# pityka/lamp

Hardware: AMD Instinct MI355X
Metric: training-step samples/sec (higher is better)
Workload: dtype bf16; 1 GPU; example-cifar100 Cnn.resnet(100) training step (fwd+backprop+AdamW), synthetic CIFAR batch; per_gpu_batch=2048, global_batch=2048, parallelism=single, optimizer=AdamW lr 1e-3 wd 0 beta2 0.95 mixedPrecision

## Files before the change

### lamp_amd/csrc/core/switches.h

```cpp
#pragma once
#include <cstdint>

namespace lamp {

constexpr int64_t SW_NO_CLAMP = INT64_MIN;

#define LAMP_SWITCHES_ONCE(X)                                                                                                             \
                                                        \
  X(conv_sibling, "LAMP_CONV_SIBLING", BOOL, 1, 0, "a residual block's 3x3 and its sibling 1x1 of the same input as one forward launch") \
  X(fuse_bn_pair, "LAMP_FUSE_BN_PAIR", BOOL, 1, 0, "relu(bn(right) + bn(left)) at a block's end as one op (0: the chain)")                \
  X(fuse_pool_logsoftmax, "LAMP_FUSE_POOL_LOGSOFTMAX", BOOL, 1, 0, "average pool -> flatten -> log-softmax tail as one node")             \
  X(fuse_block_tail, "LAMP_FUSE_BLOCK_TAIL", BOOL, 1, 0, "the last residual block and the pooled log-softmax tail as one node")          \
  X(fuse_bn_conv, "LAMP_FUSE_BN_CONV", BOOL, 1, 0, "batch norm -> relu -> convolution: the convolution applies the norm while staging")  \
  X(fuse_loss_accumulate, "LAMP_FUSE_LOSS_ACCUMULATE", BOOL, 1, 0, "acc += n * loss inside the NLL loss kernel")                          \
  X(fuse_loss_backward, "LAMP_FUSE_LOSS_BACKWARD", BOOL, 1, 0, "the NLL loss backward goes straight to the pooled log-softmax node's input in one launch")                      \
  X(fuse_loss_tail, "LAMP_FUSE_LOSS_TAIL", BOOL, 1, 0, "the loss launch also writes the pooled log-softmax's input gradient per plane")  \
  X(conv_dgrad_accumulate, "LAMP_CONV_DGRAD_ACCUMULATE", BOOL, 1, 0, "a convolution's input gradient adds into the existing one in its epilogue") \
  X(conv_dgrad_pair, "LAMP_CONV_DGRAD_PAIR", BOOL, 1, 0, "input gradients of a block's 3x3 and sibling 1x1 from one launch")             \
  X(conv_wgrad_pair, "LAMP_CONV_WGRAD_PAIR", BOOL, 1, 0, "weight gradients of a block's 3x3 and sibling 1x1 from one launch")            \
  X(linear_bias_fused, "LAMP_LINEAR_BIAS_FUSED", BOOL, 1, 0, "a linear layer's bias in the GEMM epilogue (0: mm then add)")               \
  X(mult_add_fused, "LAMP_MULT_ADD_FUSED", BOOL, 1, 0, "x * scale + residual in one pass (0: mult then add)")                             \
  X(attention_as_written_for_cuda, "LAMP_ATTENTION_AS_WRITTEN_FOR_CUDA", BOOL, 0, 0, "multi-head attention as the reference's op chain instead of the fused kernels") \
  X(recurrent_fused, "LAMP_RECURRENT_FUSED", BOOL, 1, 0, "RNN / GRU / LSTM as one node per sequence with fused cell kernels (0: the fold over time steps)") \
  X(fuse_qkv, "LAMP_FUSE_QKV", BOOL, 1, 0, "self-attention's three projections as one product (0: three)")                                \
  X(host_stream_side, "LAMP_HOST_STREAM_SIDE", BOOL, 0, 0, "batch streams gather on a side stream instead of the consumer's")             \
                                                                           \
  X(pinned_cache_mb, "LAMP_PINNED_CACHE_MB", INT, 2048, 0, "upper bound of the cache of freed pinned host buffers, MiB")                  \
  X(pinned_gather_wgs, "LAMP_PINNED_GATHER_WGS", INT, 48, 1, "workgroups of a gather that reads pinned host memory")                      \
                                                                                                    \
  X(flash_attention, "LAMP_FLASH_ATTENTION", BOOL, 1, 0, "the flash attention kernels, forward and backward")                             \
  X(small_attention, "LAMP_SMALL_ATTENTION", BOOL, 1, 0, "the short-sequence attention kernels")                                          \
  X(knn_fused, "LAMP_KNN_FUSED", BOOL, 1, 0, "the fused distance + top-k nearest-neighbour kernel")                                       \
  X(knn_split, "LAMP_KNN_SPLIT", INT, -1, SW_NO_CLAMP, "f16-plane k-NN filter: 0 off, 1 where it pays, 2 forced; negative: the mode set through the API") \
  X(knn_split_planes, "LAMP_KNN_SPLIT_PLANES", INT, 0, SW_NO_CLAMP, "f16 planes per coordinate of that filter: 3, anything else 2")      \
  X(umap_pairs2, "LAMP_UMAP_PAIRS2", BOOL, 1, 0, "the UMAP loss's two-dimensional pair kernel")                                            \
                                                                                                             \
  X(gemm_shape_tags, "LAMP_GEMM_SHAPE_TAGS", BOOL, 0, 0, "profiling aid: one kernel-timer class per GEMM shape and layout")               \
  X(gemm_splitk, "LAMP_GEMM_SPLITK", BOOL, 1, 0, "split-K for products with few output tiles (bf16 and f32 / f64)")                       \
  X(gemm_tail_split, "LAMP_GEMM_TAIL_SPLIT", BOOL, 1, 0, "an almost empty last round of 256 x 256 tiles becomes a second, split-K product") \
  X(gemm_fp_split_wgs, "LAMP_GEMM_FP_SPLIT_WGS", INT, 512, 1, "workgroups an f32 / f64 split-K product aims at")                          \
                                                                                              \
  X(bn_fused_bwd, "LAMP_BN_FUSED_BWD", BOOL, 1, 0, "one-pass batch-norm backward (workgroups exchange their sums) where no mode is set through the API") \
  X(bn_fused_fp, "LAMP_BN_FUSED_FP", BOOL, 1, 0, "... its f32 / f64 form")                                                               \
  X(bn_fused_np_mask, "LAMP_BN_FUSED_NP_MASK", INT, 24, SW_NO_CLAMP, "bit mask of packets per thread (1 .. 16) at which the one-pass form runs") \
  X(bn_fused_per_cu, "LAMP_BN_FUSED_PER_CU", INT, 1, 1, "workgroups per CU the one-pass form aims at first")                              \
  X(bn_fused_small_bytes, "LAMP_BN_FUSED_SMALL_BYTES", INT, (4 << 20) + 1, SW_NO_CLAMP, "bf16 activations below this many bytes take the one-pass form whatever the mask") \
                          \
  X(conv_small2, "LAMP_CONV_SMALL2", BOOL, 1, 0, "the small-map direct convolution kernels (second generation)")                          \
  X(conv_small2_wgrad, "LAMP_CONV_SMALL2_WGRAD", BOOL, 1, 0, "... their weight gradient")                                                 \
  X(igemm_f32, "LAMP_IGEMM_F32", BOOL, 1, 0, "implicit-GEMM convolution for f32")                                                          \
  X(igemm_f64, "LAMP_IGEMM_F64", BOOL, 1, 0, "implicit-GEMM convolution for f64")                                                          \
  X(conv_bn_stats, "LAMP_CONV_BN_STATS", BOOL, 1, 0, "forward convolutions hand per-image batch-norm statistics of their output on")     \
  X(ncv_bn_stats, "LAMP_NCV_BN_STATS", BOOL, 1, 0, "... the narrow kernels' alone (needs LAMP_CONV_BN_STATS on as well)")                 \
  X(ncv_dgrad_parity, "LAMP_NCV_DGRAD_PARITY", BOOL, 1, 0, "narrow stride-2 pair input gradient: super-tiles by row parity (0: the plain form)") \
  X(ncv_pitch, "LAMP_NCV_PITCH", BOOL, 1, 0, "narrow kernels widen the LDS row pitch to a bank-conflict-free one")                        \
  X(ncv_two_shift, "LAMP_NCV_TWO_SHIFT", BOOL, 1, 0, "narrow kernels: two output phases per MFMA where the columns allow it")             \
  X(ncv_per_cu, "LAMP_NCV_PER_CU", INT, 4, 1, "narrow kernels: most workgroups per CU")                                                   \
  X(pack_cache, "LAMP_PACK_CACHE", BOOL, 1, 0, "packed filter images are cached per parameter and storage version")                       \
  X(pack_after_step, "LAMP_PACK_AFTER_STEP", BOOL, 1, 0, "the optimiser repacks every cached filter image in one launch (0: lazily at first use)") \
                                                    \
  X(ig_small_d, "LAMP_IG_SMALL_D", BOOL, 1, 0, "the eight-image kernel for at most 64 output channels too")                               \
  X(ig_w8, "LAMP_IG_W8", BOOL, 1, 0, "two-image 128-row kernel: eight waves per image pair at one workgroup per CU or fewer (0: four)")  \
  X(ig_one_image, "LAMP_IG_ONE_IMAGE", BOOL, 1, 0, "... one image per workgroup at one image per CU or fewer (0: pairs)")                 \
                                                                                                 \
  X(wgrad_group, "LAMP_WGRAD_GROUP", BOOL, 1, 0, "two layers' eight-wave weight gradients parked and launched as one (0: every layer at once)") \
  X(wgrad_min_ips, "LAMP_WGRAD_MIN_IPS", INT, 0, 2, "fewest images per weight-gradient workgroup; unset (0): 2 up to 512 images, 8 above") \
// ... 21 lines not shown
```

### lamp_amd/csrc/kernels/conv.hip

```cpp
#include "device_utils.h"
#include "../core/strided.h"
#include "conv_geom.h"

namespace lamp {

template <class T>
__global__ __launch_bounds__(256) void conv_fwd_direct_kernel(const T* __restrict__ x, const T* __restrict__ w, const T* __restrict__ bias,
                                                              T* __restrict__ y, ConvGeom g) {
  using A = acc_t<T>;
  const int64_t total = g.N * g.Cout * g.Ho * g.Wo;
  const int cin_g = (int)(g.Cin / g.groups), cout_g = (int)(g.Cout / g.groups);
  for (int64_t e = blockIdx.x * (int64_t)blockDim.x + threadIdx.x; e < total; e += (int64_t)gridDim.x * blockDim.x) {
    const int wo = (int)(e % g.Wo);
    const int ho = (int)((e / g.Wo) % g.Ho);
    const int co = (int)((e / (g.Wo * g.Ho)) % g.Cout);
    const int64_t n = e / (g.Wo * g.Ho * g.Cout);
    const int grp = co / cout_g;
    A acc = bias ? load_as<A>(bias[co]) : A(0);
    const T* wp = w + (int64_t)co * cin_g * g.kh * g.kw;
    for (int cl = 0; cl < cin_g; cl++) {
      const T* xp = x + ((n * g.Cin + grp * cin_g + cl) * g.H) * g.W;
      for (int r = 0; r < g.kh; r++) {
        const int h = ho * g.sh - g.ph + r * g.dh;
        if (h < 0 || h >= g.H) continue;
        for (int s = 0; s < g.kw; s++) {
          const int ww = wo * g.sw - g.pw + s * g.dw;
          if (ww < 0 || ww >= g.W) continue;
          acc += load_as<A>(xp[h * g.W + ww]) * load_as<A>(wp[(cl * g.kh + r) * g.kw + s]);
        }
      }
    }
    y[e] = store_as<T>(acc);
  }
}

template <class T>
__global__ __launch_bounds__(256) void conv_dgrad_direct_kernel(const T* __restrict__ dy, const T* __restrict__ w, const T* __restrict__ bias,
                                                                T* __restrict__ dx, ConvGeom g) {
  using A = acc_t<T>;
  const int64_t total = g.N * g.Cin * g.H * g.W;
  const int cin_g = (int)(g.Cin / g.groups), cout_g = (int)(g.Cout / g.groups);
  for (int64_t e = blockIdx.x * (int64_t)blockDim.x + threadIdx.x; e < total; e += (int64_t)gridDim.x * blockDim.x) {
    const int wi = (int)(e % g.W);
    const int hi = (int)((e / g.W) % g.H);
    const int ci = (int)((e / (g.W * g.H)) % g.Cin);
    const int64_t n = e / (g.W * g.H * g.Cin);
    const int grp = ci / cin_g, cl = ci - grp * cin_g;
    A acc = bias ? load_as<A>(bias[ci]) : A(0);
    for (int r = 0; r < g.kh; r++) {
      const int hn = hi + g.ph - r * g.dh;
      if (hn < 0 || hn % g.sh != 0) continue;
      const int ho = hn / g.sh;
      if (ho >= g.Ho) continue;
      for (int s = 0; s < g.kw; s++) {
        const int wn = wi + g.pw - s * g.dw;
// ... 159 lines not shown
  hipLaunchKernelGGL((conv_fwd_direct_kernel<T>), dim3(grid_for(total, 256, 16)), dim3(256), 0, st, x->ptr<T>(), w->ptr<T>(),
                     b ? b->ptr<T>() : (const T*)nullptr, y->ptr<T>(), g);
  LAMP_LAUNCH_CHECK();
}
template <class T> static void launch_dgrad(const Tensor* dy, const Tensor* w, const Tensor* b, Tensor* dx, const ConvGeom& g, hipStream_t st) {
  const int64_t total = g.N * g.Cin * g.H * g.W;
  if (!total) return;
  KernelTimer kt("conv_dgrad_direct", conv_flops(g), conv_bytes(g, sizeof(T)), st);
  hipLaunchKernelGGL((conv_dgrad_direct_kernel<T>), dim3(grid_for(total, 256, 16)), dim3(256), 0, st, dy->ptr<T>(), w->ptr<T>(),
                     b ? b->ptr<T>() : (const T*)nullptr, dx->ptr<T>(), g);
  LAMP_LAUNCH_CHECK();
}
template <class T> static void launch_wgrad(const Tensor* dy, const Tensor* x, Tensor* dw, const ConvGeom& g, hipStream_t st) {
  const int64_t blocks = g.Cout * (g.Cin / g.groups);
  if (!blocks) return;
  const int khkw = g.kh * g.kw;
  {
    using A = acc_t<T>;
    const int64_t O = blocks * khkw;
    const size_t lds = (size_t)(g.Cin * g.H * g.W + g.Cout * g.Ho * g.Wo + O) * sizeof(A);
    if (lds <= 150 * 1024 && O <= 8192) {
      const int nb = (int)std::min<int64_t>(g.N, (int64_t)num_cus() * 2);
      const int ipb = (int)((g.N + nb - 1) / nb);
      const int nblocks = (int)((g.N + ipb - 1) / ipb);
      const int PS = O >= 256 ? 1 : (int)(256 / O);
      int64_t ps[1] = {(int64_t)nblocks * O};
      Hold partial(new_tensor(ps, 1, std::is_same<A, double>::value ? kF64 : kF32, dy->device()));
      allow_big_lds((const void*)conv_wgrad_lds_kernel<T>);
      {
        KernelTimer kt("conv_wgrad_lds", conv_flops(g), conv_bytes(g, sizeof(T)), st);
        hipLaunchKernelGGL((conv_wgrad_lds_kernel<T>), dim3(nblocks), dim3(256), lds, st, dy->ptr<T>(), x->ptr<T>(), partial->ptr<A>(), g, (int)O, PS, ipb);
        LAMP_LAUNCH_CHECK();
      }
      hipLaunchKernelGGL((conv_wgrad_reduce_kernel<T>), dim3((unsigned)((O * 64 + 255) / 256)), dim3(256), 0, st, partial->ptr<A>(), dw->ptr<T>(), (int)O, nblocks);
      LAMP_LAUNCH_CHECK();
      return;
    }
  }
  LAMP_CHECK(khkw <= MAXRS, "kernel window larger than " << MAXRS << " taps is not supported");
  KernelTimer kt("conv_wgrad_direct", conv_flops(g), conv_bytes(g, sizeof(T)), st);
  if (khkw == 1) hipLaunchKernelGGL((conv_wgrad_direct_kernel<T, 1>), dim3((unsigned)blocks), dim3(256), 0, st, dy->ptr<T>(), x->ptr<T>(), dw->ptr<T>(), g);
  else if (khkw <= 9) hipLaunchKernelGGL((conv_wgrad_direct_kernel<T, 9>), dim3((unsigned)blocks), dim3(256), 0, st, dy->ptr<T>(), x->ptr<T>(), dw->ptr<T>(), g);
  else if (khkw <= 25) hipLaunchKernelGGL((conv_wgrad_direct_kernel<T, 25>), dim3((unsigned)blocks), dim3(256), 0, st, dy->ptr<T>(), x->ptr<T>(), dw->ptr<T>(), g);
  else hipLaunchKernelGGL((conv_wgrad_direct_kernel<T, MAXRS>), dim3((unsigned)blocks), dim3(256), 0, st, dy->ptr<T>(), x->ptr<T>(), dw->ptr<T>(), g);
  LAMP_LAUNCH_CHECK();
}

bool igemm_conv_fwd(const Tensor* x, const Tensor* w, const Tensor* bias, Tensor* y, const ConvGeom& g, hipStream_t st);
bool igemm_conv_fwd_pair(const Tensor* x, const Tensor* w, const Tensor* bias, Tensor* y, const ConvGeom& g, const Tensor* w1, const Tensor* bias1,
                         Tensor* y1, const ConvGeom& g1, hipStream_t st);
bool igemm_conv_dgrad(const Tensor* dy, const Tensor* w, Tensor* dx, const ConvGeom& g, hipStream_t st, const Tensor* addend = nullptr,
                      bool* addend_fused = nullptr);
bool igemm_conv_wgrad(const Tensor* dy, const Tensor* x, Tensor* dw, const ConvGeom& g, hipStream_t st, const Tensor* affine = nullptr);
bool igemm_conv_folds_affine(const ConvGeom& g, int dtype);
bool igemm_conv_fwd_affine(const Tensor* x, const Tensor* affine, const Tensor* w, const Tensor* bias, Tensor* y, const ConvGeom& g, hipStream_t st);
bool igemm32_conv_fwd(const Tensor* x, const Tensor* w, const Tensor* bias, Tensor* y, const ConvGeom& g, hipStream_t st);
bool igemm32_conv_dgrad(const Tensor* dy, const Tensor* w, Tensor* dx, const ConvGeom& g, hipStream_t st, const Tensor* addend = nullptr,
                        bool* addend_fused = nullptr);
bool igemm32_conv_wgrad(const Tensor* dy, const Tensor* x, Tensor* dw, const ConvGeom& g, hipStream_t st);
bool narrow_conv_fwd(const Tensor* x, const Tensor* w, const Tensor* bias, Tensor* y, const ConvGeom& g, hipStream_t st);
bool narrow_conv_fwd_pair(const Tensor* x, const Tensor* w, const Tensor* bias, Tensor* y, const ConvGeom& g, const Tensor* w1, const Tensor* bias1,
                          Tensor* y1, const ConvGeom& g1, hipStream_t st);
bool narrow_conv_dgrad(const Tensor* dy, const Tensor* w, Tensor* dx, const ConvGeom& g, hipStream_t st, const Tensor* addend = nullptr,
                       bool* addend_fused = nullptr);
bool narrow_conv_dgrad_pair(const Tensor* dy, const Tensor* w, const ConvGeom& g, const Tensor* dy1, const Tensor* w1, const ConvGeom& g1, Tensor* dx,
                            hipStream_t st, const Tensor* addend, bool* addend_fused);
bool igemm_conv_dgrad_pair(const Tensor* dy, const Tensor* w, const ConvGeom& g, const Tensor* dy1, const Tensor* w1, const ConvGeom& g1, Tensor* dx,
                           hipStream_t st, const Tensor* addend, bool* addend_fused);
bool narrow_conv_wgrad(const Tensor* dy, const Tensor* x, Tensor* dw, const ConvGeom& g, hipStream_t st);
bool narrow_conv_wgrad_pair(const Tensor* dy, const Tensor* dy1, const Tensor* x, Tensor* dw, Tensor* dw1, const ConvGeom& g, const ConvGeom& g1, hipStream_t st);
bool igemm_conv_wgrad_pair(const Tensor* dy, const Tensor* dy1, const Tensor* x, Tensor* dw, Tensor* dw1, const ConvGeom& g, const ConvGeom& g1, hipStream_t st);
bool small_conv_fwd(const Tensor* x, const Tensor* w, const Tensor* bias, Tensor* y, const ConvGeom& g, hipStream_t st);
bool small_conv_dgrad(const Tensor* dy, const Tensor* w, Tensor* dx, const ConvGeom& g, hipStream_t st, const Tensor* addend = nullptr,
                      bool* addend_fused = nullptr);
bool small_conv_wgrad(const Tensor* dy, const Tensor* x, Tensor* dw, const ConvGeom& g, hipStream_t st);

Tensor* reduce_dims(const Tensor* a, const int64_t* dims, int ndims, bool keepdim, int op);

template <class T>
__global__ __launch_bounds__(256) void bn_relu_materialise_kernel(const T* __restrict__ x, T* __restrict__ y, const float4* __restrict__ affine, int64_t total,
                                                                  int64_t C, int64_t HW) {
  for (int64_t i = blockIdx.x * (int64_t)blockDim.x + threadIdx.x; i < total; i += (int64_t)gridDim.x * blockDim.x) {
    const float4 a = affine[(i / HW) % C];
    T o = store_as<T>(__builtin_fmaf(load_as<float>(x[i]) - a.x, a.y, a.z));
    if (load_as<float>(o) < 0.f) o = store_as<T>(0.f);
    y[i] = o;
  }
}
Tensor* bn_relu_materialise(const Tensor* xc, const Tensor* affine, hipStream_t st) {
  Hold y(new_like(xc));
  const int64_t total = xc->numel(), C = xc->sizes[1];
  int64_t HW = 1;
  for (int i = 2; i < xc->ndim; i++) HW *= xc->sizes[i];
  if (total > 0) {
    const float4* aff = reinterpret_cast<const float4*>(affine->ptr<float>());
    const dim3 grid(grid_for(total, 256));
    if (xc->dtype == kBF16) hipLaunchKernelGGL((bn_relu_materialise_kernel<bf16_t>), grid, dim3(256), 0, st, xc->ptr<bf16_t>(), y->ptr<bf16_t>(), aff, total, C, HW);
    else if (xc->dtype == kF16) hipLaunchKernelGGL((bn_relu_materialise_kernel<f16_t>), grid, dim3(256), 0, st, xc->ptr<f16_t>(), y->ptr<f16_t>(), aff, total, C, HW);
    else hipLaunchKernelGGL((bn_relu_materialise_kernel<float>), grid, dim3(256), 0, st, xc->ptr<float>(), y->ptr<float>(), aff, total, C, HW);
    LAMP_LAUNCH_CHECK();
  }
  return y.take();
}
static Tensor* contiguous_filter(const Tensor* w) {
  Tensor* c = contiguous(w);
  if (c->st != w->st) c->st->scratch = true;
  return c;
}
}

using namespace lamp;

extern "C" {

int lamp_convolution(lamp_tensor** out, const lamp_tensor* x, const lamp_tensor* w, const lamp_tensor* bias, const int64_t* stride,
                     const int64_t* padding, const int64_t* dilation, int nspatial, int transposed, const int64_t* output_padding,
                     int64_t groups) {
  LAMP_API_BEGIN
  check_device_tensor(x, "input"); check_device_tensor(w, "weight");
  LAMP_CHECK(x->dtype == w->dtype, "convolution: input " << x->describe() << " and weight " << w->describe() << " have different dtypes");
  ConvGeom g = make_geom(x, w, stride, padding, dilation, nspatial, transposed, output_padding, groups);
  const int64_t out_c = transposed ? g.Cin : g.Cout;
  if (bias) { check_device_tensor(bias, "bias"); LAMP_CHECK(bias->numel() == out_c && bias->dtype == x->dtype, "convolution: bias must have " << out_c << " elements"); }
  Hold xc(contiguous(x)), wc(contiguous_filter(w));
  Hold bc(bias ? contiguous(bias) : nullptr);
  std::vector<int64_t> oshape = {g.N, out_c};
  if (nspatial == 2) oshape.push_back(transposed ? g.H : g.Ho);
  oshape.push_back(transposed ? g.W : g.Wo);
  Hold y(new_tensor(oshape, x->dtype, x->device()));
  hipStream_t st = current_stream(x->device());
  if (!transposed) {
    if (!igemm_conv_fwd(xc.get(), wc.get(), bc.get(), y.get(), g, st) && !igemm32_conv_fwd(xc.get(), wc.get(), bc.get(), y.get(), g, st) &&
        !narrow_conv_fwd(xc.get(), wc.get(), bc.get(), y.get(), g, st) && !small_conv_fwd(xc.get(), wc.get(), bc.get(), y.get(), g, st)) {
      LAMP_DISPATCH_FLOAT(x->dtype, T, (launch_fwd<T>(xc.get(), wc.get(), bc.get(), y.get(), g, st)));
    }
  } else {
    LAMP_DISPATCH_FLOAT(x->dtype, T, (launch_dgrad<T>(xc.get(), wc.get(), bc.get(), y.get(), g, st)));
  }
  *out = y.take();
  LAMP_API_END
}

int lamp_convolution_pair(lamp_tensor* out2[2], const lamp_tensor* x, const lamp_tensor* w_a, const lamp_tensor* bias_a, const int64_t* stride_a,
                          const int64_t* padding_a, const int64_t* dilation_a, const lamp_tensor* w_b, const lamp_tensor* bias_b,
                          const int64_t* stride_b, const int64_t* padding_b, const int64_t* dilation_b, int nspatial, int64_t groups) {
  LAMP_API_BEGIN
  out2[0] = out2[1] = nullptr;
  check_device_tensor(x, "input"); check_device_tensor(w_a, "weight a"); check_device_tensor(w_b, "weight b");
  const int64_t zero2[2] = {0, 0};
  bool fused = false;
  if (nspatial == 2 && x->dtype == w_a->dtype && x->dtype == w_b->dtype && x->dtype == kBF16 && (!bias_a || bias_a->is_device()) && (!bias_b || bias_b->is_device())) {
    ConvGeom ga = make_geom(x, w_a, stride_a, padding_a, dilation_a, nspatial, 0, zero2, groups);
    ConvGeom gb = make_geom(x, w_b, stride_b, padding_b, dilation_b, nspatial, 0, zero2, groups);
    const bool biases_ok = (!bias_a || (bias_a->numel() == ga.Cout && bias_a->dtype == x->dtype)) && (!bias_b || (bias_b->numel() == gb.Cout && bias_b->dtype == x->dtype));
    if (biases_ok && ga.Ho == gb.Ho && ga.Wo == gb.Wo) {
// ... 22 lines not shown
int lamp_convolution_backward(lamp_tensor* out3[3], const lamp_tensor* grad_out, const lamp_tensor* x, const lamp_tensor* w,
                              const int64_t* stride, const int64_t* padding, const int64_t* dilation, int nspatial, int transposed,
                              const int64_t* output_padding, int64_t groups, const uint8_t mask[3]) {
  LAMP_API_BEGIN
  check_device_tensor(x, "input"); check_device_tensor(w, "weight"); check_device_tensor(grad_out, "grad_out");
  LAMP_CHECK(x->dtype == w->dtype && grad_out->dtype == x->dtype, "convolution_backward: dtype mismatch");
  ConvGeom g = make_geom(x, w, stride, padding, dilation, nspatial, transposed, output_padding, groups);
  {
    const int64_t oc = transposed ? g.Cin : g.Cout, oh = transposed ? g.H : g.Ho, ow = transposed ? g.W : g.Wo;
    LAMP_CHECK(grad_out->ndim == x->ndim && grad_out->sizes[0] == g.N && grad_out->sizes[1] == oc &&
               grad_out->sizes[grad_out->ndim - 1] == ow && (nspatial == 1 || grad_out->sizes[2] == oh),
               "convolution_backward: grad_out " << grad_out->describe() << " does not match the forward output shape");
  }
  Hold xc(contiguous(x)), wc(contiguous_filter(w)), gc(contiguous(grad_out));
  hipStream_t st = current_stream(x->device());
  Hold dx(mask[0] ? new_like(xc.get()) : nullptr);
  Hold dw(mask[1] ? new_like(wc.get()) : nullptr);
  Hold db;
  if (!transposed) {
    if (dx.get() && !igemm_conv_dgrad(gc.get(), wc.get(), dx.get(), g, st) && !igemm32_conv_dgrad(gc.get(), wc.get(), dx.get(), g, st) &&
        !narrow_conv_dgrad(gc.get(), wc.get(), dx.get(), g, st) && !small_conv_dgrad(gc.get(), wc.get(), dx.get(), g, st)) {
      LAMP_DISPATCH_FLOAT(x->dtype, T, (launch_dgrad<T>(gc.get(), wc.get(), nullptr, dx.get(), g, st)));
    }
    if (dw.get() && !igemm_conv_wgrad(gc.get(), xc.get(), dw.get(), g, st) && !igemm32_conv_wgrad(gc.get(), xc.get(), dw.get(), g, st) &&
        !narrow_conv_wgrad(gc.get(), xc.get(), dw.get(), g, st) && !small_conv_wgrad(gc.get(), xc.get(), dw.get(), g, st)) {
      LAMP_DISPATCH_FLOAT(x->dtype, T, (launch_wgrad<T>(gc.get(), xc.get(), dw.get(), g, st)));
    }
  } else {
    if (dx.get()) { LAMP_DISPATCH_FLOAT(x->dtype, T, (launch_fwd<T>(gc.get(), wc.get(), nullptr, dx.get(), g, st))); }
    if (dw.get()) { LAMP_DISPATCH_FLOAT(x->dtype, T, (launch_wgrad<T>(xc.get(), gc.get(), dw.get(), g, st))); }
  }
  if (mask[2]) {
    std::vector<int64_t> dims = {0};
    for (int i = 2; i < grad_out->ndim; i++) dims.push_back(i);
    db = Hold(reduce_dims(gc.get(), dims.data(), (int)dims.size(), false, 0));
  }
  out3[0] = dx.take(); out3[1] = dw.take(); out3[2] = db.take();
  LAMP_API_END
}

static void check_affine(const lamp_tensor* affine, const lamp_tensor* x) {
  check_device_tensor(affine, "affine");
  LAMP_CHECK(affine->dtype == kF32 && affine->ndim == 2 && affine->sizes[0] == x->sizes[1] && affine->sizes[1] == 4 && affine->is_contiguous(),
             "affine must be the contiguous f32 [channels, 4] table of lamp_batch_norm_affine, got " << affine->describe());
  LAMP_CHECK(x->dtype == kBF16 || x->dtype == kF16 || x->dtype == kF32, "conv(relu(bn(x))) with a folded batch norm is a reduced-precision path (f32 table): f64 runs the separate operators");
}
int lamp_convolution_bn_relu_input_folds(int* out, const lamp_tensor* x, const lamp_tensor* w, const int64_t* stride, const int64_t* padding,
                                         const int64_t* dilation, int nspatial, int64_t groups) {
  LAMP_API_BEGIN
  *out = 0;
  if (!x->is_device() || !w->is_device() || x->dtype != w->dtype) return 0;
  const int64_t zero2[2] = {0, 0};
  ConvGeom g = make_geom(x, w, stride, padding, dilation, nspatial, 0, zero2, groups);
  *out = igemm_conv_folds_affine(g, x->dtype) ? 1 : 0;
  LAMP_API_END
}
int lamp_convolution_bn_relu_input(lamp_tensor** out, const lamp_tensor* x, const lamp_tensor* affine, const lamp_tensor* w, const lamp_tensor* bias,
                                   const int64_t* stride, const int64_t* padding, const int64_t* dilation, int nspatial, int64_t groups) {
  LAMP_API_BEGIN
  check_device_tensor(x, "input"); check_device_tensor(w, "weight"); check_affine(affine, x);
  LAMP_CHECK(x->dtype == w->dtype, "convolution: input " << x->describe() << " and weight " << w->describe() << " have different dtypes");
  const int64_t zero2[2] = {0, 0};
  ConvGeom g = make_geom(x, w, stride, padding, dilation, nspatial, 0, zero2, groups);
  if (bias) { check_device_tensor(bias, "bias"); LAMP_CHECK(bias->numel() == g.Cout && bias->dtype == x->dtype, "convolution: bias must have " << g.Cout << " elements"); }
  Hold xc(contiguous(x)), wc(contiguous_filter(w));
  Hold bc(bias ? contiguous(bias) : nullptr);
  hipStream_t st = current_stream(x->device());
  std::vector<int64_t> oshape = {g.N, g.Cout};
  if (nspatial == 2) oshape.push_back(g.Ho);
  oshape.push_back(g.Wo);
  Hold y(new_tensor(oshape, x->dtype, x->device()));
  if (!igemm_conv_fwd_affine(xc.get(), affine, wc.get(), bc.get(), y.get(), g, st)) {
    Hold act(bn_relu_materialise(xc.get(), affine, st));
    lamp_tensor* o = nullptr;
    if (lamp_convolution(&o, act.get(), wc.get(), bc.get(), stride, padding, dilation, nspatial, 0, zero2, groups) != 0) throw Error(lamp_last_error());
    *out = o;
    return 0;
  }
  *out = y.take();
  LAMP_API_END
}
int lamp_convolution_bn_relu_input_backward(lamp_tensor* out3[3], const lamp_tensor* grad_out, const lamp_tensor* x, const lamp_tensor* affine,
                                            const lamp_tensor* w, const int64_t* stride, const int64_t* padding, const int64_t* dilation, int nspatial,
                                            int64_t groups, const uint8_t mask[3]) {
  LAMP_API_BEGIN
  out3[0] = out3[1] = out3[2] = nullptr;
  check_device_tensor(x, "input"); check_device_tensor(w, "weight"); check_device_tensor(grad_out, "grad_out"); check_affine(affine, x);
  const int64_t zero2[2] = {0, 0};
  ConvGeom g = make_geom(x, w, stride, padding, dilation, nspatial, 0, zero2, groups);
  Hold xc(contiguous(x)), wc(contiguous_filter(w)), gc(contiguous(grad_out));
  hipStream_t st = current_stream(x->device());
  Hold dw;
  bool dw_done = false;
  if (mask[1]) {
    dw = Hold(new_like(wc.get()));
    dw_done = igemm_conv_wgrad(gc.get(), xc.get(), dw.get(), g, st, affine);
  }
  const bool need_act = mask[1] && !dw_done;
  Hold act(need_act ? bn_relu_materialise(xc.get(), affine, st) : nullptr);
  const uint8_t m3[3] = {mask[0], (uint8_t)(mask[1] && !dw_done), mask[2]};
  lamp_tensor* r3[3] = {nullptr, nullptr, nullptr};
  if (m3[0] || m3[1] || m3[2]) {
    if (lamp_convolution_backward(r3, gc.get(), need_act ? act.get() : xc.get(), wc.get(), stride, padding, dilation, nspatial, 0, zero2, groups, m3) != 0)
      throw Error(lamp_last_error());
  }
  out3[0] = r3[0]; out3[1] = dw_done ? dw.take() : r3[1]; out3[2] = r3[2];
  LAMP_API_END
}

int lamp_convolution_backward_input_add(lamp_tensor** out, const lamp_tensor* grad_out, const lamp_tensor* x, const lamp_tensor* w,
                                        const int64_t* stride, const int64_t* padding, const int64_t* dilation, int nspatial,
                                        const int64_t* output_padding, int64_t groups, const lamp_tensor* addend) {
  LAMP_API_BEGIN
  check_device_tensor(x, "input"); check_device_tensor(w, "weight"); check_device_tensor(grad_out, "grad_out"); check_device_tensor(addend, "addend");
  LAMP_CHECK(x->dtype == w->dtype && grad_out->dtype == x->dtype && addend->dtype == x->dtype, "convolution_backward_input_add: dtype mismatch");
  LAMP_CHECK(addend->ndim == x->ndim, "convolution_backward_input_add: addend " << addend->describe() << " does not have the input's shape " << x->describe());
  for (int i = 0; i < x->ndim; i++)
    LAMP_CHECK(addend->sizes[i] == x->sizes[i], "convolution_backward_input_add: addend " << addend->describe() << " does not have the input's shape " << x->describe());
  ConvGeom g = make_geom(x, w, stride, padding, dilation, nspatial, 0, output_padding, groups);
  LAMP_CHECK(grad_out->ndim == x->ndim && grad_out->sizes[0] == g.N && grad_out->sizes[1] == g.Cout &&
             grad_out->sizes[grad_out->ndim - 1] == g.Wo && (nspatial == 1 || grad_out->sizes[2] == g.Ho),
             "convolution_backward_input_add: grad_out " << grad_out->describe() << " does not match the forward output shape");
  Hold wc(contiguous_filter(w)), gc(contiguous(grad_out)), ac(contiguous(addend));
  hipStream_t st = current_stream(x->device());
  Hold dx(new_tensor(std::vector<int64_t>(x->sizes, x->sizes + x->ndim), x->dtype, x->device()));
  bool fused = false;
  if (!igemm_conv_dgrad(gc.get(), wc.get(), dx.get(), g, st, ac.get(), &fused) && !igemm32_conv_dgrad(gc.get(), wc.get(), dx.get(), g, st, ac.get(), &fused) &&
      !narrow_conv_dgrad(gc.get(), wc.get(), dx.get(), g, st, ac.get(), &fused) && !small_conv_dgrad(gc.get(), wc.get(), dx.get(), g, st, ac.get(), &fused)) {
    LAMP_DISPATCH_FLOAT(x->dtype, T, (launch_dgrad<T>(gc.get(), wc.get(), nullptr, dx.get(), g, st)));
  }
  if (fused) { *out = dx.take(); }
  else {
    lamp_tensor* sum = nullptr;
    if (lamp_add(&sum, ac.get(), dx.get(), 1.0) != 0) throw Error(lamp_last_error());
    *out = sum;
  }
  LAMP_API_END
}

int lamp_convolution_backward_input_pair(lamp_tensor** out, const lamp_tensor* x, const lamp_tensor* grad_out_a, const lamp_tensor* w_a,
                                         const int64_t* stride_a, const int64_t* padding_a, const int64_t* dilation_a,
                                         const lamp_tensor* grad_out_b, const lamp_tensor* w_b, const int64_t* stride_b,
                                         const int64_t* padding_b, const int64_t* dilation_b, int nspatial, int64_t groups,
                                         const lamp_tensor* addend) {
  LAMP_API_BEGIN
  check_device_tensor(x, "input"); check_device_tensor(w_a, "first weight"); check_device_tensor(grad_out_a, "first grad_out");
  check_device_tensor(w_b, "second weight"); check_device_tensor(grad_out_b, "second grad_out");
  LAMP_CHECK(x->dtype == w_a->dtype && x->dtype == w_b->dtype && grad_out_a->dtype == x->dtype && grad_out_b->dtype == x->dtype,
             "convolution_backward_input_pair: dtype mismatch");
// ... 83 lines not shown
```

### lamp_amd/csrc/kernels/conv_igemm.hip

```cpp
#include <map>
#include <mutex>
#include <tuple>
#include "device_utils.h"
#include "conv_geom.h"
#include "wgrad_reduce.h"
#include <thread>
#include "conv_narrow_pack.h"
#include "../core/switches.h"

namespace lamp {

typedef short s8v __attribute__((ext_vector_type(8)));
typedef __bf16 bf8v __attribute__((ext_vector_type(8)));
typedef float f4v __attribute__((ext_vector_type(4)));

constexpr int IG_M = 128;
constexpr int IG_WTILE = 128 * 64 * 2;

__device__ __forceinline__ int ig_kc_off(int row, int chunk) { return row * 128 + ((chunk ^ (row & 7)) << 4); }

__device__ __forceinline__ void ig_stage_load_rows(uint4 (&r)[4], const bf16_t* __restrict__ base, int64_t ld, int64_t k0, int64_t rows,
                                                   int64_t K, int tid) {
#pragma unroll
  for (int i = 0; i < 4; i++) {
// ... 260 lines not shown
        for (int j = 0; j < 4; j++) acc[i][j] = __builtin_amdgcn_mfma_f32_16x16x32_bf16(fb1[j], fa1[i], acc[i][j], 0, 0, 0);
      __builtin_amdgcn_s_setprio(0);
      stage_wait(cc);
      __builtin_amdgcn_s_barrier();
    }
    if constexpr (SIBM == 1) {
      epilogue(sib.y, sib.bias, sib.stats, nullptr);
#pragma unroll
      for (int i = 0; i < NTI; i++)
#pragma unroll
        for (int j = 0; j < 4; j++) acc[i][j] = f4v{0.f, 0.f, 0.f, 0.f};
    } else {
      load_images(x);
      asm volatile("s_waitcnt vmcnt(0) lgkmcnt(0)" ::: "memory");
      __builtin_amdgcn_s_barrier();
    }
  }
  int t = 0;
#pragma unroll
  for (int rs = 0; rs < RS; rs++) {
    for (int cc = 0; cc < CC; cc++, t++) {
      const char* wl = Wl + ((CS + t) & (NSLOT - 1)) * IG_WTILE + a_row;
      if (CS + t + NSLOT - 1 < TT) stage_dma(CS + t + NSLOT - 1);
      const int u = ((cc * (KW >> 3)) & cmask) << 4;
#pragma unroll
      for (int i = 0; i < NTI; i++) {
        fa0[i] = __builtin_bit_cast(bf8v, *reinterpret_cast<const s8v*>(wl + i * 16 * 128 + a_ch0));
        fa1[i] = __builtin_bit_cast(bf8v, *reinterpret_cast<const s8v*>(wl + i * 16 * 128 + a_ch1));
      }
#pragma unroll
      for (int j = 0; j < 4; j++) {
        fb0[j] = __builtin_bit_cast(bf8v, *reinterpret_cast<const s8v*>(Xl + (pre[rs][j] ^ u)));
        fb1[j] = __builtin_bit_cast(bf8v, *reinterpret_cast<const s8v*>(Xl + (pre[rs][j] ^ u ^ (4 << 4))));
      }
      asm volatile("s_waitcnt lgkmcnt(0)" ::: "memory");
      __builtin_amdgcn_s_setprio(1);
#pragma unroll
      for (int i = 0; i < NTI; i++)
#pragma unroll
        for (int j = 0; j < 4; j++) acc[i][j] = __builtin_amdgcn_mfma_f32_16x16x32_bf16(fb0[j], fa0[i], acc[i][j], 0, 0, 0);
#pragma unroll
      for (int i = 0; i < NTI; i++)
#pragma unroll
        for (int j = 0; j < 4; j++) acc[i][j] = __builtin_amdgcn_mfma_f32_16x16x32_bf16(fb1[j], fa1[i], acc[i][j], 0, 0, 0);
      __builtin_amdgcn_s_setprio(0);
      stage_wait(CS + t);
      __builtin_amdgcn_s_barrier();
    }
  }

  epilogue(y, bias, stats, addend);
}

template <int KS, int SIBM = 0>
__global__ __launch_bounds__(256) void ig_conv8c_kernel(const bf16_t* __restrict__ x, const bf16_t* __restrict__ wp, const bf16_t* __restrict__ bias,
                                                        bf16_t* __restrict__ y, int N, int CI, int KP, int CO, float* __restrict__ stats,
                                                        const bf16_t* addend, const IgSibling sib) {
  static_assert(SIBM == 0 || (SIBM == 2 && KS == 3), "second-source input gradients of a 3x3 only");
  extern __shared__ __attribute__((aligned(16))) char smem[];
  constexpr int RS = KS * KS;
  constexpr int PAD = (KS - 1) / 2;
  constexpr int NW = 2, NT = 256, LPT = 2;
  constexpr int WT = 64 * 64 * 2, NSLOT = 4;
  const int RB = KP * 2;
  const int XIMG = 64 * RB;
  char* Xl = smem;
  const int ZOFF = NW * XIMG;
  char* Wl = smem + NW * XIMG + RB;
  const int tid = threadIdx.x, lane = tid & 63;
  const int wid = __builtin_amdgcn_readfirstlane(tid >> 6);
  const int wr = wid >> 1, wc = wid & 1;
  const int n0 = blockIdx.x * NW;
  const int cmask = (KP >> 3) - 1;

  constexpr int KW = 64;
  const int CC = KP / KW;
  const int T = RS * CC;
  typedef __attribute__((address_space(3))) char lds_char_t;
  typedef const __attribute__((address_space(1))) char glb_char_t;
  const int CS = SIBM ? CC : 0, TT = CS + T;
  auto stage_dma = [&](int g) {
    const bf16_t* wimg = (SIBM && g < CS) ? sib.wp : wp;
    const int t = (SIBM && g < CS) ? g : g - CS;
    const int rs1 = t / CC, cc1 = t - rs1 * CC;
    const bf16_t* base = wimg + (int64_t)rs1 * IG_M * KP + cc1 * KW;
#pragma unroll
    for (int i = 0; i < LPT; i++) {
      const int piece = wid * LPT + i;
      const int p = piece * 64 + lane;
      const int row = p >> 3, chunk = (p & 7) ^ (row & 7);
      __builtin_amdgcn_global_load_lds((glb_char_t*)(base + row * KP + chunk * 8), (lds_char_t*)(Wl + (g & 3) * WT + piece * 1024), 16, 0, 0);
    }
  };
  stage_dma(0);
  if (1 < TT) stage_dma(1);
  if (2 < TT) stage_dma(2);
  if (tid * 16 < RB) *reinterpret_cast<uint4*>(Xl + ZOFF + tid * 16) = make_uint4(0, 0, 0, 0);
  auto load_images = [&](const bf16_t* __restrict__ x) {
    const int ncgp = KP >> 3;
    for (int e = tid; e < NW * 8 * ncgp; e += NT) {
      const int cg = e % ncgp, h = (e / ncgp) & 7, img = e / (ncgp * 8);
      const int n = n0 + img;
      unsigned int w[8][4];
#pragma unroll
      for (int k = 0; k < 8; k++) {
        const int c = cg * 8 + k;
        uint4 v = make_uint4(0, 0, 0, 0);
        if (c < CI && n < N) v = *reinterpret_cast<const uint4*>(x + ((int64_t)n * CI + c) * 64 + h * 8);
        w[k][0] = v.x; w[k][1] = v.y; w[k][2] = v.z; w[k][3] = v.w;
      }
      char* xi = Xl + img * XIMG;
#pragma unroll
      for (int p = 0; p < 8; p++) {
        unsigned int d[4];
#pragma unroll
        for (int j = 0; j < 4; j++) {
          const unsigned int lo = w[2 * j][p >> 1], hi = w[2 * j + 1][p >> 1];
          d[j] = (p & 1) ? ((lo >> 16) | (hi & 0xffff0000u)) : ((lo & 0xffffu) | (hi << 16));
        }
        *reinterpret_cast<uint4*>(xi + (h * 8 + p) * RB + ((cg ^ x_swz(h + 1, p + 1, cmask)) << 4)) = make_uint4(d[0], d[1], d[2], d[3]);
      }
    }
  };
  load_images(SIBM == 2 ? sib.x2 : x);

  f4v acc[2][4];
#pragma unroll
  for (int i = 0; i < 2; i++)
#pragma unroll
    for (int j = 0; j < 4; j++) acc[i][j] = f4v{0.f, 0.f, 0.f, 0.f};


  int rowsel, wpix;
  px_of_col(lane & 15, rowsel, wpix);
  int pre[RS][4];
#pragma unroll
  for (int rs = 0; rs < RS; rs++) {
    const int r = rs / KS, s = rs - r * KS;
#pragma unroll
    for (int j = 0; j < 4; j++) {
      const int h = 2 * j + rowsel + r - PAD, w = wpix + s - PAD;
      const bool inside = h >= 0 && h < 8 && w >= 0 && w < 8;
      pre[rs][j] = inside ? wc * XIMG + (h * 8 + w) * RB + ((((lane >> 4) & cmask) ^ x_swz(h + 1, w + 1, cmask)) << 4)
                          : ZOFF + (((lane >> 4) & cmask) << 4);
    }
  }
  const int a_row = (wr * 32 + (lane & 15)) * 128;
  const int a_ch0 = ((lane >> 4) ^ (lane & 7)) << 4, a_ch1 = ((4 + (lane >> 4)) ^ (lane & 7)) << 4;

  asm volatile("s_waitcnt vmcnt(0) lgkmcnt(0)" ::: "memory");
  __builtin_amdgcn_s_barrier();

  bf8v fa0[2], fb0[4], fa1[2], fb1[4];
  if constexpr (SIBM == 2) {
    for (int g = 0; g < CS; g++) {
      const char* wl = Wl + (g & 3) * WT + a_row;
      if (g + 3 < TT) stage_dma(g + 3);
      const int u = ((g * (KW >> 3)) & cmask) << 4;
#pragma unroll
      for (int i = 0; i < 2; i++) {
        fa0[i] = __builtin_bit_cast(bf8v, *reinterpret_cast<const s8v*>(wl + i * 16 * 128 + a_ch0));
// ... 45 lines not shown
      asm volatile("s_waitcnt lgkmcnt(0)" ::: "memory");
      __builtin_amdgcn_s_setprio(1);
#pragma unroll
      for (int i = 0; i < 2; i++)
#pragma unroll
        for (int j = 0; j < 4; j++) acc[i][j] = __builtin_amdgcn_mfma_f32_16x16x32_bf16(fb0[j], fa0[i], acc[i][j], 0, 0, 0);
#pragma unroll
      for (int i = 0; i < 2; i++)
#pragma unroll
        for (int j = 0; j < 4; j++) acc[i][j] = __builtin_amdgcn_mfma_f32_16x16x32_bf16(fb1[j], fa1[i], acc[i][j], 0, 0, 0);
      __builtin_amdgcn_s_setprio(0);
      if (g + 3 < TT) asm volatile("s_waitcnt vmcnt(4)" ::: "memory");
      else if (g + 2 < TT) asm volatile("s_waitcnt vmcnt(2)" ::: "memory");
      else asm volatile("s_waitcnt vmcnt(0)" ::: "memory");
      __builtin_amdgcn_s_barrier();
    }
  }

  const int n = n0 + wc;
  if (n < N) {
    bf16_t* yp = y + (int64_t)n * CO * 64;
    const int q = lane >> 4;
    const int qrow = (q == 1 || q == 2) ? 1 : 0, qw = (q >= 2) ? 4 : 0;
#pragma unroll
    for (int i = 0; i < 2; i++) {
      const int co = wr * 32 + i * 16 + (lane & 15);
      const float b = (bias && co < CO) ? (float)bias[co] : 0.f;
      float vals[16];
#pragma unroll
      for (int j = 0; j < 4; j++) {
        const bf16_t o0(acc[i][j][0] + b), o1(acc[i][j][1] + b), o2(acc[i][j][2] + b), o3(acc[i][j][3] + b);
        if (co < CO) {
          uint2 pk;
          pk.x = (unsigned)o0.bits | ((unsigned)o1.bits << 16);
          pk.y = (unsigned)o2.bits | ((unsigned)o3.bits << 16);
          if (addend) {
            const uint2 av = *reinterpret_cast<const uint2*>(addend + (int64_t)n * CO * 64 + co * 64 + (2 * j + qrow) * 8 + qw);
            pk.x = add_bf16x2(pk.x, av.x); pk.y = add_bf16x2(pk.y, av.y);
          }
          *reinterpret_cast<uint2*>(yp + co * 64 + (2 * j + qrow) * 8 + qw) = pk;
        }
        vals[4 * j + 0] = __uint_as_float((unsigned)o0.bits << 16); vals[4 * j + 1] = __uint_as_float((unsigned)o1.bits << 16);
        vals[4 * j + 2] = __uint_as_float((unsigned)o2.bits << 16); vals[4 * j + 3] = __uint_as_float((unsigned)o3.bits << 16);
      }
      if (stats) {
        float wn, wm, w2;
        ig_stats_wave(vals, wn, wm, w2);
        if (q == 0 && co < CO) { float* sp = stats + ((int64_t)co * N + n) * 3;  sp[0] = wn; sp[1] = wm; sp[2] = w2; }
      }
    }
  }
}

__device__ __forceinline__ uint4 ig_bn_relu_x8(uint4 v, float mu, float scale, float bb) {
  unsigned* w = &v.x;
#pragma unroll
  for (int q = 0; q < 4; q++) {
    const float x0 = __uint_as_float(w[q] << 16), x1 = __uint_as_float(w[q] & 0xffff0000u);
    bf16_t o0(__builtin_fmaf(x0 - mu, scale, bb)), o1(__builtin_fmaf(x1 - mu, scale, bb));
    if ((float)o0 < 0.f) o0 = bf16_t(0.f);
    if ((float)o1 < 0.f) o1 = bf16_t(0.f);
    w[q] = (unsigned)o0.bits | ((unsigned)o1.bits << 16);
  }
  return v;
}

#ifdef IG8D_STAMP
__device__ unsigned long long ig8d_stamps[8 * 512];
__device__ unsigned long long ig8d_rt_stamps[8 * 512];
#define IG_STAMP(k) do { if (threadIdx.x == 0 && blockIdx.x < 512) { ig8d_stamps[blockIdx.x * 8 + (k)] = __builtin_amdgcn_s_memtime(); \
                                                                     ig8d_rt_stamps[blockIdx.x * 8 + (k)] = __builtin_amdgcn_s_memrealtime(); } } while (0)
#else
#define IG_STAMP(k) do { } while (0)
#endif
__device__ __forceinline__ int ig8d_swz(int h, int w) { return ((h & 1) << 1) | ((w >> 2) & 1); }

__device__ __forceinline__ void ig8d_tile_stats(const uint2 (&pk)[4], float& mean, float& m2) {
  typedef float f2v __attribute__((ext_vector_type(2)));
  const float sh = __uint_as_float(pk[0].x << 16);
  const f2v sh2 = {sh, sh};
  f2v s1 = {0.f, 0.f}, s2 = {0.f, 0.f};
#pragma unroll
  for (int j = 0; j < 4; j++) {
    const f2v va = {__uint_as_float(pk[j].x << 16), __uint_as_float(pk[j].x & 0xffff0000u)};
    const f2v vb = {__uint_as_float(pk[j].y << 16), __uint_as_float(pk[j].y & 0xffff0000u)};
    const f2v da = va - sh2, db = vb - sh2;
    s1 += da; s2 = __builtin_elementwise_fma(da, da, s2);
    s1 += db; s2 = __builtin_elementwise_fma(db, db, s2);
  }
  const float t1 = s1[0] + s1[1], t2 = s2[0] + s2[1];
  mean = sh + t1 * (1.f / 16.f); m2 = t2 - t1 * t1 * (1.f / 16.f);
  {
    float ma = mean, mb = mean, qa = m2, qb = m2;
    asm("s_nop 1\n\tv_permlane16_swap_b32 %0, %1" : "+v"(ma), "+v"(mb));
    asm("s_nop 1\n\tv_permlane16_swap_b32 %0, %1" : "+v"(qa), "+v"(qb));
    const float d = mb - ma; mean = ma + d * 0.5f; m2 = qa + qb + d * d * 8.f;
  }
  {
    float ma = mean, mb = mean, qa = m2, qb = m2;
    asm("s_nop 1\n\tv_permlane32_swap_b32 %0, %1" : "+v"(ma), "+v"(mb));
    asm("s_nop 1\n\tv_permlane32_swap_b32 %0, %1" : "+v"(qa), "+v"(qb));
    const float d = mb - ma; mean = ma + d * 0.5f; m2 = qa + qb + d * d * 16.f;
  }
}

template <int KS, int NCT, int SIBM>
__global__ __launch_bounds__(512) void ig_conv8d_kernel(const bf16_t* __restrict__ x, const bf16_t* __restrict__ wp, const bf16_t* __restrict__ bias,
                                                        bf16_t* y, int N, int CI, int KP, int CO, float* __restrict__ stats, int stats_per_wg,
                                                        const bf16_t* addend, const float4* __restrict__ affine, const IgSibling sib) {
  constexpr bool SIB = SIBM == 1, DG2 = SIBM == 2;
  static_assert(SIBM == 0 || KS == 3, "the sibling product is the centre tap of a 3x3 staging");
  extern __shared__ __attribute__((aligned(16))) char smem[];
  constexpr int RS = KS * KS;
  constexpr int PAD = (KS - 1) / 2;
  constexpr int NI = 8, NT = 512;
  constexpr int WT = 128 * 32 * 2, NSLOT = 3;
  constexpr int RB = 64;
  constexpr int XIMG = 64 * RB;
// ... 40 lines not shown
  const unsigned d_srcw = (unsigned)((lane >> 2) * KP + wid * 32 + (((lane & 3) ^ ((4 - ((lane >> 4) & 3)) & 3)) << 3)) * 2u;
  auto stage_dma_w = [&](const bf16_t* wimg, int rs1, int slot) {
    if (wid < KC)
      __builtin_amdgcn_global_load_lds((glb_char_t*)(reinterpret_cast<const char*>(wimg + (int64_t)rs1 * IG_M * KP) + d_srcw),
                                       (lds_char_t*)(Wl + slot * WT + wid * 1024), 16, 0, 0);
  };
  const bool taps4 = WIDE && !DG2 && KC == 1 && RS > 1;
  auto stage_dma_t = [&](int g, int slot) {
    const int tap = 4 * g + wid;
    if (wid < 4 && tap < RS)
      __builtin_amdgcn_global_load_lds((glb_char_t*)(reinterpret_cast<const char*>(wp + (int64_t)tap * IG_M * KP) + (d_srcw - (unsigned)(wid * 32) * 2u)),
                                       (lds_char_t*)(Wl + slot * WT + wid * 1024), 16, 0, 0);
  };
  IG_STAMP(0);
  if constexpr (WIDE) {
    if (taps4) { stage_dma_t(0, 0); stage_dma_t(1, 1); }
    else if (DG2) { stage_dma_w(sib.wp, 0, 0); stage_dma_w(wp, 0, 1); }
    else { stage_dma_w(wp, 0, 0); if (RS > 1) stage_dma_w(wp, 1, 1); }
  } else if (SIB || DG2) {
    stage_dma_of(sib.wp, 0, 0, 0);
    if (KC > 1) stage_dma_of(sib.wp, 1, 0, 1);
  } else {
    stage_dma(0, 0, 0);
    if (T > 1) stage_dma(1 / RS, 1 % RS, 1);
  }
  IG_STAMP(1);
  unsigned bpair[SIB ? (NCT + 1) / 2 : 1];
  if constexpr (SIB) {
#pragma unroll
    for (int k = 0; k < (NCT + 1) / 2; k++) {
      const int c0 = 2 * k * 16 + (lane & 15), c1 = c0 + 16;
      const unsigned b0 = (sib.bias && c0 < CO) ? sib.bias[c0].bits : 0u, b1 = (sib.bias && 2 * k + 1 < NCT && c1 < CO) ? sib.bias[c1].bits : 0u;
      bpair[k] = b0 | (b1 << 16);
    }
  }
  auto load_images = [&](const bf16_t* __restrict__ x) {
    for (int e = tid; e < NI * 8 * 4 * KC; e += NT) {
      const int cg = e & 3, h = (e >> 2) & 7, img = (e >> 5) & 7, ch = e >> 8;
      const int n = n0 + img;
      uint4 rw[8];
#pragma unroll
      for (int k = 0; k < 8; k++) {
        const int c = ch * 32 + cg * 8 + k;
        rw[k] = make_uint4(0, 0, 0, 0);
        if (c < CI && n < N) {
          const uint4* src = reinterpret_cast<const uint4*>(x + ((int64_t)n * CI + c) * 64 + h * 8);
          rw[k] = stats ? nt_load16(src) : *src;
        }
      }
      if (affine) {
#pragma unroll
        for (int k = 0; k < 8; k++) {
          const int c = ch * 32 + cg * 8 + k;
          if (c < CI && n < N) { const float4 a = affine[c]; rw[k] = ig_bn_relu_x8(rw[k], a.x, a.y, a.z); }
        }
      }
      char* xi = Xl + ch * XBUF + img * XIMG;
#pragma unroll
      for (int p = 0; p < 8; p++) {
        unsigned int d[4];
#pragma unroll
        for (int j = 0; j < 4; j++) {
          const unsigned int lo = (&rw[2 * j].x)[p >> 1], hi = (&rw[2 * j + 1].x)[p >> 1];
          d[j] = (p & 1) ? ((lo >> 16) | (hi & 0xffff0000u)) : ((lo & 0xffffu) | (hi << 16));
        }
        *reinterpret_cast<uint4*>(xi + (h * 8 + p) * RB + ((cg ^ ig8d_swz(h, p)) << 4)) = make_uint4(d[0], d[1], d[2], d[3]);
      }
    }
  };
  load_images(DG2 ? sib.x2 : x);
  f4v acc[NCT][4];
#pragma unroll
  for (int i = 0; i < NCT; i++)
#pragma unroll
    for (int j = 0; j < 4; j++) acc[i][j] = f4v{0.f, 0.f, 0.f, 0.f};

  int rowsel, wpix;
  px_of_col(lane & 15, rowsel, wpix);
  const int p0 = wid * XIMG + ((rowsel - PAD) * 8 + (wpix - PAD)) * RB;
  int va[2][KS];
#pragma unroll
  for (int par = 0; par < 2; par++)
#pragma unroll
    for (int s = 0; s < KS; s++)
      va[par][s] = p0 + (((lane >> 4) ^ ig8d_swz(rowsel + par - PAD, wpix + s - PAD)) << 4);
  const bool col_lo = wpix == 0, col_hi = wpix == 7, row_lo = rowsel == 0, row_hi = rowsel == 1;
  const int a_off = (lane & 15) * 64 + ((((lane >> 4) ^ ((4 - ((lane >> 2) & 3)) & 3)) & 3) << 4);

  asm volatile("s_waitcnt vmcnt(0) lgkmcnt(0)" ::: "memory");
  __builtin_amdgcn_s_barrier();
  if constexpr (SIB) {
#pragma unroll
    for (int k = 0; k < (NCT + 1) / 2; k++) asm volatile("" : "+v"(bpair[k]));
  }
  IG_STAMP(2);

  bf8v fa[NCT], fb[4];
  const bf8v zero8 = __builtin_bit_cast(bf8v, s8v{0, 0, 0, 0, 0, 0, 0, 0});
  if constexpr (WIDE) {
    bf8v fw[4], fx[4][4];
    auto read_stage = [&](int slot, int r, int s) {
      const char* wl = Wl + slot * WT + a_off;
#pragma unroll
      for (int kc = 0; kc < 4; kc++)
        if (kc < KC) {
          fw[kc] = __builtin_bit_cast(bf8v, *reinterpret_cast<const s8v*>(wl + kc * 1024));
          const char* xb = Xl + kc * XBUF + va[r & 1][s];
// ... 366 lines not shown
      float s1 = 0.f, s2 = 0.f, sm = 0.f;
#pragma unroll
      for (int w = 0; w < 8; w++) { const float2 v = sl[w * 128]; const float d = v.x - shift; s1 += d; s2 += d * d; sm += v.y; }
      float* sp = stats + ((int64_t)tid * gridDim.x + blockIdx.x) * 3;
      sp[0] = 512.f; sp[1] = shift + s1 * 0.125f; sp[2] = sm + 64.f * (s2 - s1 * s1 * 0.125f);
    }
  }
  asm volatile("s_waitcnt lgkmcnt(0)" ::: "memory");
  IG_STAMP(4);
  if (n < N) {
    bf16_t* yp = y + (int64_t)n * CO * 64;
    if (addend) {
      const bf16_t* ap = addend + (int64_t)n * CO * 64;
      uint4 av[NCT * 2];
#pragma unroll
      for (int it = 0; it < NCT * 2; it++) {
        const int idx = it * 64 + lane;
        const int co = idx >> 3, c = idx & 7;
        av[it] = make_uint4(0, 0, 0, 0);
        if (co < CO) av[it] = *reinterpret_cast<const uint4*>(ap + co * 64 + c * 8);
      }
#pragma unroll
      for (int it = 0; it < NCT * 2; it++) {
        const int idx = it * 64 + lane;
        const int co = idx >> 3, c = idx & 7;
        const uint4 v = *reinterpret_cast<const uint4*>(El + co * 128 + ((c ^ (co & 7)) << 4));
        if (co < CO) *reinterpret_cast<uint4*>(yp + co * 64 + c * 8) = add_bf16x8(v, av[it]);
      }
    } else {
#pragma unroll
      for (int it = 0; it < NCT * 2; it++) {
        const int idx = it * 64 + lane;
        const int co = idx >> 3, c = idx & 7;
        const uint4 v = *reinterpret_cast<const uint4*>(El + co * 128 + ((c ^ (co & 7)) << 4));
        if (co < CO) *reinterpret_cast<uint4*>(yp + co * 64 + c * 8) = v;
      }
    }
  }
  IG_STAMP(5);
#ifdef IG8D_STAMP
  asm volatile("s_waitcnt vmcnt(0)" ::: "memory");
  IG_STAMP(6);
#endif
}
#ifdef IG8D_STAMP
extern "C" int lamp_debug_ig8d_stamps(unsigned long long* out) { return hipMemcpyFromSymbol(out, HIP_SYMBOL(ig8d_stamps), sizeof(ig8d_stamps)) == hipSuccess ? 0 : 1; }
extern "C" int lamp_debug_ig8d_rt_stamps(unsigned long long* out) { return hipMemcpyFromSymbol(out, HIP_SYMBOL(ig8d_rt_stamps), sizeof(ig8d_rt_stamps)) == hipSuccess ? 0 : 1; }
#endif

constexpr int WG_CI = 32;
constexpr int WG_XCH = 176;
constexpr int WG_XCOPY = WG_CI * WG_XCH;
constexpr int WG_STAGE = IG_WTILE + 3 * WG_XCOPY + 512;
template <int KS, bool NARROW, int CIT, bool PAIR = false, bool CI16 = false>
__global__ __launch_bounds__(256) void ig_wgrad8v2_kernel(const bf16_t* __restrict__ dy, const bf16_t* __restrict__ x, float* __restrict__ partial,
                                                          int N, int CO, int CI, int CIP, int images_per_split, int COP, int ntile,
                                                          const bf16_t* __restrict__ dy2, float* __restrict__ partial2, int CO2, int COP2) {
  static_assert(!PAIR || (KS == 3 && CIT == 1), "the pair rides on the 3x3 kernel with one slice of Cin");
  extern __shared__ __attribute__((aligned(16))) char smem[];
  constexpr int RS = KS * KS;
  constexpr int PAD = (KS - 1) / 2;
  const int nsplit = gridDim.x / ntile;
  int tile, split;
  {
    const int b = blockIdx.x;
    if ((nsplit & 7) == 0) { const int xcd = b & 7, slot = b >> 3; tile = slot % ntile; split = xcd + 8 * (slot / ntile); }
    else { tile = b % ntile; split = b / ntile; }
  }
  const int ci0 = tile * WG_CI * CIT;
  constexpr int STAGE1 = IG_WTILE + (CIT > 1 ? CIT * WG_XCOPY : 3 * WG_XCOPY) + 512;
  constexpr int STAGE = STAGE1 + (PAIR ? IG_WTILE : 0);
  const int tid = threadIdx.x, lane = tid & 63, wid = tid >> 6;
  constexpr int NI = CI16 ? 2 : 4;
  const int wr = CI16 ? wid : wid >> 1, wc = CI16 ? 0 : wid & 1;
  const int co_w = wr * (NI * 16);
  const int nbeg = split * images_per_split, nend = min(nbeg + images_per_split, N);
  for (int o = tid * 16; o < 2 * STAGE; o += 256 * 16) *reinterpret_cast<uint4*>(smem + o) = make_uint4(0, 0, 0, 0);
  __syncthreads();

  const int xci = tid >> 3, xh = tid & 7;
  auto load_x = [&](int n, int ct) -> uint4 {
    const int c = ci0 + ct * WG_CI + xci;
    if (c < CI) return *reinterpret_cast<const uint4*>(x + ((int64_t)n * CI + c) * 64 + xh * 8);
    return make_uint4(0, 0, 0, 0);
  };
  auto store_x = [&](char* stage, uint4 v, int ct) {
    char* xb = stage + IG_WTILE + (ct * WG_CI + xci) * WG_XCH + (xh + 1) * 16;
    if (KS == 1) { *reinterpret_cast<uint4*>(xb) = v; return; }
    *reinterpret_cast<uint4*>(xb + WG_XCOPY) = v;
  };

  f4v acc[CIT][RS][NI];
#pragma unroll
  for (int ct = 0; ct < CIT; ct++)
#pragma unroll
    for (int t = 0; t < RS; t++)
#pragma unroll
      for (int i = 0; i < NI; i++) acc[ct][t][i] = f4v{0.f, 0.f, 0.f, 0.f};
  const bool col_active = ci0 + wc * 16 < CIP;
  bool tile_active[NI];
#pragma unroll
  for (int i = 0; i < NI; i++) tile_active[i] = col_active && (co_w + i * 16 < COP);

  uint4 ra[4], rx[CIT], rb[PAIR ? 4 : 1];
  f4v acc2[PAIR ? NI : 1];
  if constexpr (PAIR) {
#pragma unroll
    for (int i = 0; i < NI; i++) acc2[i] = f4v{0.f, 0.f, 0.f, 0.f};
  }
  if (nbeg < nend) {
    ig_stage_load_rows(ra, dy + (int64_t)nbeg * CO * 64, 64, 0, CO, 64, tid);
    if constexpr (PAIR) ig_stage_load_rows(rb, dy2 + (int64_t)nbeg * CO2 * 64, 64, 0, CO2, 64, tid);
#pragma unroll
    for (int ct = 0; ct < CIT; ct++) rx[ct] = load_x(nbeg, ct);
    ig_stage_store_rows(ra, smem, tid);
    if constexpr (PAIR) ig_stage_store_rows(rb, smem + STAGE1, tid);
#pragma unroll
    for (int ct = 0; ct < CIT; ct++) store_x(smem, rx[ct], ct);
  }
  __syncthreads();
  for (int n = nbeg; n < nend; n++) {
    const int cur = (n - nbeg) & 1;
    if (n + 1 < nend) {
      ig_stage_load_rows(ra, dy + (int64_t)(n + 1) * CO * 64, 64, 0, CO, 64, tid);
      if constexpr (PAIR) ig_stage_load_rows(rb, dy2 + (int64_t)(n + 1) * CO2 * 64, 64, 0, CO2, 64, tid);
#pragma unroll
      for (int ct = 0; ct < CIT; ct++) rx[ct] = load_x(n + 1, ct);
    }
    const char* st = smem + cur * STAGE;
    const char* xl = st + IG_WTILE + (wc * 16 + (lane & 15)) * WG_XCH;
#pragma unroll
    for (int ks = 0; ks < 2; ks++) {
      bf8v fa[NI];
#pragma unroll
      for (int i = 0; i < NI; i++) fa[i] = ig_frag_rows(st, co_w + i * 16, ks, lane);
      const int h = 4 * ks + (lane >> 4);
#pragma unroll
      for (int ct = 0; ct < CIT; ct++) {
        if constexpr (KS == 3) {
// ... 59 lines not shown
#pragma unroll
      for (int i = 0; i < NI; i++)
        if (!NARROW || tile_active[i]) {
#pragma unroll
          for (int rr = 0; rr < 4; rr++) {
            const int co = co_w + i * 16 + (lane >> 4) * 4 + rr, ci = ci0 + ct * WG_CI + wc * 16 + (lane & 15);
            if (co < CO && ci < CI) out[co * CIP + ci] = acc[ct][t][i][rr];
          }
        }
  }
}
#ifdef LAMP_WG8H_STAMPS
__device__ unsigned int g_wg8h_stamps[1024 * 8 * 8];
#endif
struct WgSecondProblem { const bf16_t* dy; const bf16_t* x; float* partial; int CO, CI, CIP, images_per_split, ntile; const float4* affine; int wgs0; };
template <bool PAIR, bool DMA>
__global__ __launch_bounds__(512) void ig_wgrad8h_kernel(const bf16_t* __restrict__ dy_, const bf16_t* __restrict__ x_, float* __restrict__ partial_,
                                                         int N, int CO_, int CI_, int CIP_, int images_per_split_, int ntile_, const float4* __restrict__ affine_,
                                                         const bf16_t* __restrict__ dy2, float* __restrict__ partial2, int CO2,
                                                         const WgSecondProblem sp) {
  const bool second_problem = !PAIR && sp.wgs0 > 0 && (int)blockIdx.x >= sp.wgs0;
  const bf16_t* __restrict__ dy = second_problem ? sp.dy : dy_;
  const bf16_t* __restrict__ x = second_problem ? sp.x : x_;
  float* __restrict__ partial = second_problem ? sp.partial : partial_;
  const int CO = second_problem ? sp.CO : CO_, CI = second_problem ? sp.CI : CI_, CIP = second_problem ? sp.CIP : CIP_;
  const int images_per_split = second_problem ? sp.images_per_split : images_per_split_, ntile = second_problem ? sp.ntile : ntile_;
  const float4* __restrict__ affine = second_problem ? sp.affine : affine_;
  const int wg_index = second_problem ? (int)blockIdx.x - sp.wgs0 : (int)blockIdx.x;
  const int wg_count = second_problem ? (int)gridDim.x - sp.wgs0 : ((!PAIR && sp.wgs0 > 0) ? sp.wgs0 : (int)gridDim.x);
  constexpr int XC = PAIR ? 2 * IG_WTILE : IG_WTILE + WG_XCOPY;
  constexpr int STG = PAIR ? 2 * IG_WTILE + WG_XCOPY + 512 : WG_STAGE;
  constexpr int ZSLOT = STG - 512;
  extern __shared__ __attribute__((aligned(16))) char smem[];
  constexpr int KS = 3, RS = 9, PAD = 1;
  const int nsplit = wg_count / ntile;
  int tile, split;
  {
    const int b = wg_index;
    if ((nsplit & 7) == 0) { const int xcd = b & 7, slot = b >> 3; tile = slot % ntile; split = xcd + 8 * (slot / ntile); }
    else { tile = b % ntile; split = b / ntile; }
  }
  const int ci0 = tile * WG_CI;
  const int tid = threadIdx.x, lane = tid & 63;
  const int wid = __builtin_amdgcn_readfirstlane(tid >> 6);
  const int nbeg = split * images_per_split, nend = min(nbeg + images_per_split, N);
  if (tid < 4) *reinterpret_cast<uint4*>(smem + tid * STG + ZSLOT) = make_uint4(0, 0, 0, 0);

  const int xci = (tid & 255) >> 3, xh = tid & 7, xim = tid >> 8, xcc = min(ci0 + xci, CI - 1);
  const float4 aff = affine ? affine[xcc] : make_float4(0.f, 0.f, 0.f, 0.f);
  auto load_x = [&](int n) -> uint4 {
    return *reinterpret_cast<const uint4*>(x + ((int64_t)min(n + xim, nend - 1) * CI + xcc) * 64 + xh * 8);
  };
  auto store_x = [&](char* stage, uint4 v) {
    if (affine) v = ig_bn_relu_x8(v, aff.x, aff.y, aff.z);
    *reinterpret_cast<uint4*>(stage + xim * STG + XC + xci * WG_XCH + (xh + 1) * 16) = v;
  };
  auto load_dy = [&](uint4 (&r)[2], int n) {
    const bf16_t* base = dy + (int64_t)n * CO * 64;
#pragma unroll
    for (int i = 0; i < 2; i++) {
      const int c = tid + i * 512, gr = c >> 3;
      r[i] = nt_load16(reinterpret_cast<const uint4*>(base + min(gr, CO - 1) * 64 + ((c & 7) << 3)));
    }
  };
  auto store_dy = [&](const uint4 (&r)[2], char* stage) {
#pragma unroll
    for (int i = 0; i < 2; i++) { const int c = tid + i * 512; *reinterpret_cast<uint4*>(stage + ig_kc_off(c >> 3, c & 7)) = r[i]; }
  };
  auto load_dy2 = [&](uint4 (&r)[2], int n) {
    const bf16_t* base = dy2 + (int64_t)n * CO2 * 64;
#pragma unroll
    for (int i = 0; i < 2; i++) {
      const int c = tid + i * 512, gr = c >> 3;
      r[i] = nt_load16(reinterpret_cast<const uint4*>(base + min(gr, CO2 - 1) * 64 + ((c & 7) << 3)));
    }
  };

  f4v acc[RS][2];
#pragma unroll
  for (int t = 0; t < RS; t++)
#pragma unroll
    for (int i = 0; i < 2; i++) acc[t][i] = f4v{0.f, 0.f, 0.f, 0.f};
  f4v acc2[2] = {f4v{0.f, 0.f, 0.f, 0.f}, f4v{0.f, 0.f, 0.f, 0.f}};

  auto lds_barrier = [] { asm volatile("s_waitcnt lgkmcnt(0)" ::: "memory"); __builtin_amdgcn_s_barrier(); };
  uint4 rb[PAIR ? 2 : 1][2];
  typedef __attribute__((address_space(3))) char lds_char_t;
  auto dma_tile = [&](const bf16_t* src, int rows, char* tile) {
#pragma unroll
    for (int i = 0; i < 2; i++) {
      const int piece = wid * 2 + i, pos = piece * 64 + lane, row = pos >> 3, chunk = (pos & 7) ^ (row & 7);
      const bf16_t* gsrc = src + min(row, rows - 1) * 64 + chunk * 8;
      const unsigned lds_dst = __builtin_amdgcn_readfirstlane((unsigned)(unsigned long long)(lds_char_t*)(tile + piece * 1024));
      unsigned keep;
      asm volatile("s_mov_b32 %0, m0\n\ts_mov_b32 m0, %2\n\ts_nop 0\n\tglobal_load_lds_dwordx4 %1, off\n\ts_mov_b32 m0, %0"
                   : "=&s"(keep) : "v"(gsrc), "s"(lds_dst) : "memory");
    }
  };
  auto zero_tile = [&](char* tile) {
#pragma unroll
    for (int i = 0; i < 2; i++) *reinterpret_cast<uint4*>(tile + (tid + i * 512) * 16) = make_uint4(0, 0, 0, 0);
  };
  auto dma_pair = [&](char* stage, int n) {
#pragma unroll
    for (int im = 0; im < 2; im++) {
      if (n + im < nend) {
        dma_tile(dy + (int64_t)(n + im) * CO * 64, CO, stage + im * STG);
// ... 246 lines not shown
      a.w[cnt] = w->ptr<bf16_t>(); a.Cout[cnt] = kv.first.Cout; a.Cin[cnt] = kv.first.Cin; a.KS[cnt] = KS; a.KPf[cnt] = KPf; a.KPd[cnt] = KPd;
      a.wp[cnt] = static_cast<bf16_t*>(kv.second.packed->raw());
      done.push_back({kv.first, w->st->version.load(std::memory_order_relaxed)});
      maxtotal = std::max(maxtotal, total);
      cnt++;
      break;
    }
  }
  static_assert(NCV_NKMAX * 64 <= 4 * 256, "a narrow image is four blocks of the pack kernel");
  if (cnt > 0 && ncnt > 0 && 4 * ncnt <= std::min(512, (maxtotal + 255) / 256)) {
    hipLaunchKernelGGL(ig_ncv_pack_many_kernel, dim3((unsigned)std::min(512, (maxtotal + 255) / 256), (unsigned)(cnt + 1)), dim3(256), 0, st, a, nb, cnt, ncnt);
    LAMP_LAUNCH_CHECK();
    cnt = 0; ncnt = 0;
  }
  flush();
  for (auto& d : done) {
    auto it = g_pack_cache.find(d.first);
    if (it != g_pack_cache.end()) { it->second.version = d.second; it->second.tick = ++g_pack_tick; }
  }
}

enum class IgForm { Eight, Two64, Two128 };
static IgForm ig_form(const ConvGeom& g, bool dgrad) {
  const char variant = sw_now().ig_variant;
  const int64_t CO = dgrad ? g.Cin : g.Cout;
  if ((CO > 64 || sw().ig_small_d) && variant != 'b' && (variant == 'd' || g.N >= 4 * (int64_t)num_cus())) return IgForm::Eight;
  return (CO <= 64 && variant != 'b') ? IgForm::Two64 : IgForm::Two128;
}

struct SiblingConv { const Tensor* w; const Tensor* bias; Tensor* out; const ConvGeom* g; };
struct SecondGradConv { const Tensor* dy; const Tensor* w; const ConvGeom* g; };
struct IgRequest {
  const Tensor* addend = nullptr;
  const Tensor* affine = nullptr;
  const SiblingConv* sibling = nullptr;
  const SecondGradConv* second = nullptr;
};
struct IgPlan {
  IgForm form;
  bool folds_addend, folds_affine;
  bool sibling, second;
  bool stats, per_wg;
  bool w8, one;
  int blocks;
  size_t lds;
};
static IgPlan ig_plan(const ConvGeom& g, bool dgrad, const IgRequest& rq) {
  IgPlan p{};
  p.form = ig_form(g, dgrad);
  const int KS = g.kh, CI = (int)(dgrad ? g.Cout : g.Cin), KP = pad_k(CI);
  const bool eight = p.form == IgForm::Eight;
  auto beside = [&](const ConvGeom* o) { return KS == 3 && o->kh == 1 && o->Cout == g.Cout && o->Cin == g.Cin && o->N == g.N; };
  p.folds_addend = eight || dgrad;
  p.folds_affine = eight;
  p.sibling = sw().conv_sibling && rq.sibling && !dgrad && !rq.addend && p.form != IgForm::Two64 && beside(rq.sibling->g);
  p.second = sw().conv_dgrad_pair && rq.second && dgrad && beside(rq.second->g);
  p.stats = sw().conv_bn_stats && !dgrad && g.N >= 2;
  const int pairs = (int)((g.N + 1) / 2);
  if (eight) {
    p.blocks = (int)((g.N + 7) / 8);
    p.per_wg = p.stats && g.N % 8 == 0;
    p.lds = std::max<size_t>((size_t)3 * (128 * 32 * 2) + (size_t)((CI + 31) / 32) * 8 * 4096 + (KS == 3 ? 9 * 64 : 0), (size_t)8 * 16384 + 8 * 128 * 8);
  } else if (p.form == IgForm::Two64) {
    p.blocks = pairs;
    p.lds = (size_t)2 * 64 * KP * 2 + KP * 2 + 4 * (64 * 64 * 2);
  } else {
    p.w8 = sw().ig_w8 && pairs <= num_cus();
    p.one = sw().ig_one_image && p.w8 && g.N <= num_cus();
    p.blocks = p.one ? (int)g.N : pairs;
    p.lds = (size_t)(p.one ? 1 : 2) * 64 * KP * 2 + KP * 2 + (p.one ? 4 : 2) * IG_WTILE;
  }
  return p;
}

struct StatsPublish { Hold& t; const Tensor* y; int P; ~StatsPublish() { if (t.get()) conv_stats_publish(y, t.get(), P); } };

static IgSibling ig_second_product(const IgRequest& rq, const IgPlan& pl, int64_t stat_elems, hipStream_t st, Hold* wpk, Hold* statt) {
  IgSibling s{nullptr, nullptr, nullptr, nullptr, nullptr, nullptr};
  if (!pl.sibling && !pl.second) return s;
  int64_t dgrad_off = 0;
  *wpk = Hold(pl.second ? packed_weights(rq.second->w, *rq.second->g, 1, st, &dgrad_off) : packed_weights(rq.sibling->w, *rq.sibling->g, 1, st, &dgrad_off));
  s.wp = static_cast<const Tensor*>(wpk->get())->ptr<bf16_t>() + (pl.second ? dgrad_off : 0);
  if (pl.second) { s.x2 = rq.second->dy->ptr<bf16_t>(); return s; }
  s.bias = rq.sibling->bias ? rq.sibling->bias->ptr<bf16_t>() : (const bf16_t*)nullptr;
  s.y = rq.sibling->out->ptr<bf16_t>();
  if (stat_elems) {
    int64_t ps[1] = {stat_elems};
    *statt = Hold(new_tensor(ps, 1, kF32, rq.sibling->out->device()));
    s.stats = (*statt)->ptr<float>();
  }
  return s;
}

static void run_conv8(const Tensor* in, const Tensor* w, const Tensor* bias, Tensor* out, const ConvGeom& g, bool dgrad, hipStream_t st,
                      const IgRequest& rq, const IgPlan& pl) {
  const int KS = g.kh;
  const int CI = (int)(dgrad ? g.Cout : g.Cin), CO = (int)(dgrad ? g.Cin : g.Cout);
  const int KP = pad_k(CI);
  int64_t dgrad_off = 0;
  int64_t tail_off[2] = {-1, -1};
  Hold wpk(packed_weights(w, g, KS, st, &dgrad_off, tail_off));
  const bf16_t* wpp = static_cast<const Tensor*>(wpk.get())->ptr<bf16_t>() + (dgrad ? dgrad_off : 0);
  const bool ktail_on = sw_now().ig_ktail;
  const bf16_t* wtailp = (ktail_on && tail_off[dgrad ? 1 : 0] >= 0) ? static_cast<const Tensor*>(wpk.get())->ptr<bf16_t>() + tail_off[dgrad ? 1 : 0] : (const bf16_t*)nullptr;
  const int64_t stat_elems = pl.stats ? (int64_t)g.N * CO * 3 : 0;
  Hold statt;
  float* statp = nullptr;
  if (stat_elems) {
    int64_t ps[1] = {stat_elems};
    statt = Hold(new_tensor(ps, 1, kF32, in->device()));
    statp = statt->ptr<float>();
  }
  const int per_wg = pl.per_wg ? 1 : 0;
  StatsPublish publish{statt, out, per_wg ? pl.blocks : (int)g.N};
  const ConvGeom* g2 = pl.sibling ? rq.sibling->g : pl.second ? rq.second->g : nullptr;
  const double fl2 = g2 ? conv_flops(*g2) : 0.0, by2 = g2 ? conv_bytes(*g2, 2) - (double)g.N * g.Cin * 64 * 2 : 0.0;
  KernelTimer kt("conv_igemm_fprop_dgrad", conv_flops(g) + fl2, conv_bytes(g, 2) + by2, st);
  const bf16_t* bp = bias ? bias->ptr<bf16_t>() : (const bf16_t*)nullptr;
  const bf16_t* addp = (rq.addend && pl.folds_addend) ? rq.addend->ptr<bf16_t>() : (const bf16_t*)nullptr;
  const float4* affp = (rq.affine && pl.folds_affine) ? reinterpret_cast<const float4*>(rq.affine->ptr<float>()) : (const float4*)nullptr;
  Hold sib_wpk, sib_statt;
  StatsPublish publish_sib{sib_statt, pl.sibling ? rq.sibling->out : nullptr, publish.P};
  IgSibling sib = ig_second_product(rq, pl, stat_elems, st, &sib_wpk, &sib_statt);
  const int sibm = pl.second ? 2 : pl.sibling ? 1 : 0;
  const int N = (int)g.N;
  const bf16_t* inp = in->ptr<bf16_t>();
  bf16_t* outp = out->ptr<bf16_t>();
#define IG_FOR_KS_SIBM(L_)                                                                                                                     \
  do { if (KS == 1) L_(1, 0); else if (sibm == 2) L_(3, 2); else if (sibm == 1) L_(3, 1); else L_(3, 0); } while (0)
  if (pl.form == IgForm::Eight) {
    if (KS == 3 && CO > 16 && !pl.sibling) sib.wtail = wtailp;
#define IG_LAUNCH_D(KS_, NCT_, SIBM_)                                                                                                          \
  do {                                                                                                                                         \
    allow_big_lds((const void*)ig_conv8d_kernel<KS_, NCT_, SIBM_>);                                                                            \
    hipLaunchKernelGGL((ig_conv8d_kernel<KS_, NCT_, SIBM_>), dim3(pl.blocks), dim3(512), pl.lds, st, inp, wpp, bp, outp, N, CI, KP, CO, statp, \
                       per_wg, addp, affp, sib);                                                                                               \
  } while (0)
#define IG_LAUNCH_D_CO(KS_, SIBM_)                                                                                                             \
  do { if (CO <= 16) IG_LAUNCH_D(KS_, 1, SIBM_); else if (CO <= 64) IG_LAUNCH_D(KS_, 4, SIBM_); else if (CO <= 112) IG_LAUNCH_D(KS_, 7, SIBM_); \
       else IG_LAUNCH_D(KS_, 8, SIBM_); } while (0)
    IG_FOR_KS_SIBM(IG_LAUNCH_D_CO);
#undef IG_LAUNCH_D_CO
#undef IG_LAUNCH_D
  } else {
#define IG_LAUNCH_TWO(K_, NT_)                                                                                                                 \
  do {                                                                                                                                         \
    allow_big_lds((const void*)K_);                                                                                                            \
    hipLaunchKernelGGL(K_, dim3(pl.blocks), dim3(NT_), pl.lds, st, inp, wpp, bp, outp, N, CI, KP, CO, statp, addp, sib);                       \
  } while (0)
#define IG_LAUNCH_B(KS_, SIBM_)                                                                                                                \
  do { if (pl.one) IG_LAUNCH_TWO((ig_conv8b_kernel<KS_, 8, SIBM_, 1>), 512); else if (pl.w8) IG_LAUNCH_TWO((ig_conv8b_kernel<KS_, 8, SIBM_, 2>), 512); \
       else IG_LAUNCH_TWO((ig_conv8b_kernel<KS_, 4, SIBM_, 2>), 256); } while (0)
    if (pl.form == IgForm::Two128) IG_FOR_KS_SIBM(IG_LAUNCH_B);
    else if (KS == 1) IG_LAUNCH_TWO((ig_conv8c_kernel<1>), 256);
    else if (sibm == 2) IG_LAUNCH_TWO((ig_conv8c_kernel<3, 2>), 256);
    else IG_LAUNCH_TWO((ig_conv8c_kernel<3>), 256);
#undef IG_LAUNCH_B
#undef IG_LAUNCH_TWO
  }
#undef IG_FOR_KS_SIBM
  LAMP_LAUNCH_CHECK();
}

bool igemm_conv_fwd(const Tensor* x, const Tensor* w, const Tensor* bias, Tensor* y, const ConvGeom& g, hipStream_t st) {
  if (!ig_qualifies(g, x->dtype)) return false;
  const IgRequest rq;
  run_conv8(x, w, bias, y, g, false, st, rq, ig_plan(g, false, rq));
  return true;
}
bool igemm_conv_fwd_pair(const Tensor* x, const Tensor* w, const Tensor* bias, Tensor* y, const ConvGeom& g, const Tensor* w1, const Tensor* bias1,
                         Tensor* y1, const ConvGeom& g1, hipStream_t st) {
  if (!ig_qualifies(g, x->dtype) || !ig_qualifies(g1, x->dtype)) return false;
  const SiblingConv sc{w1, bias1, y1, &g1};
  IgRequest rq;
  rq.sibling = &sc;
  const IgPlan pl = ig_plan(g, false, rq);
  if (!pl.sibling) return false;
  run_conv8(x, w, bias, y, g, false, st, rq, pl);
  return true;
}
bool igemm_conv_dgrad_pair(const Tensor* dy, const Tensor* w, const ConvGeom& g, const Tensor* dy1, const Tensor* w1, const ConvGeom& g1, Tensor* dx,
                           hipStream_t st, const Tensor* addend, bool* addend_fused) {
  if (addend_fused) *addend_fused = false;
  if (!ig_qualifies(g, dy->dtype) || !ig_qualifies(g1, dy1->dtype)) return false;
  const SecondGradConv sg{dy1, w1, &g1};
  IgRequest rq;
  rq.addend = addend;
  rq.second = &sg;
  const IgPlan pl = ig_plan(g, true, rq);
  if (!pl.second) return false;
  run_conv8(dy, w, nullptr, dx, g, true, st, rq, pl);
  if (addend_fused) *addend_fused = addend && pl.folds_addend;
  return true;
}
static bool ig_fwd_folds_affine(const ConvGeom& g, int dtype) { return ig_qualifies(g, dtype) && ig_plan(g, false, IgRequest{}).folds_affine; }
static bool wgrad_takes_eight_wave(const ConvGeom& g) { return g.kh == 3 && g.Cin > WG_CI && g.Cout > 64; }
static bool ig_wgrad_folds_affine(const ConvGeom& g, int dtype) { return ig_qualifies(g, dtype) && wgrad_takes_eight_wave(g); }
bool igemm_conv_folds_affine(const ConvGeom& g, int dtype) { return ig_fwd_folds_affine(g, dtype) && ig_wgrad_folds_affine(g, dtype); }
bool igemm_conv_fwd_affine(const Tensor* x, const Tensor* affine, const Tensor* w, const Tensor* bias, Tensor* y, const ConvGeom& g, hipStream_t st) {
  if (!ig_qualifies(g, x->dtype)) return false;
  IgRequest rq;
  rq.affine = affine;
  const IgPlan pl = ig_plan(g, false, rq);
  if (!pl.folds_affine) return false;
  run_conv8(x, w, bias, y, g, false, st, rq, pl);
  return true;
}
bool igemm_conv_dgrad(const Tensor* dy, const Tensor* w, Tensor* dx, const ConvGeom& g, hipStream_t st, const Tensor* addend, bool* addend_fused) {
  if (addend_fused) *addend_fused = false;
  if (!ig_qualifies(g, dy->dtype)) return false;
  IgRequest rq;
  rq.addend = addend;
  const IgPlan pl = ig_plan(g, true, rq);
  run_conv8(dy, w, nullptr, dx, g, true, st, rq, pl);
  if (addend_fused) *addend_fused = addend && pl.folds_addend;
  return true;
}
static int wgrad_min_ips(int64_t N) {
  const int v = (int)sw().wgrad_min_ips;
  return v ? v : (N <= 512 ? 2 : 8);
}
struct WgradSplit { int ips, nsplit; };
static WgradSplit wgrad_split(int64_t N, int wg_budget, int ntile) {
  const int target = std::max(1, wg_budget / ntile);
  int ips = (int)std::max<int64_t>(1, (N + target - 1) / target);
  if (ips < wgrad_min_ips(N) && N >= wgrad_min_ips(N)) ips = wgrad_min_ips(N);
  return {ips, (int)((N + ips - 1) / ips)};
}
static WgradReduceArgs wgrad_reduce_args(int CO, int CI, int CIP, int COP, int RS, int nsplit) {
  WgradReduceArgs ra{};
  ra.kind = 0; ra.CO = CO; ra.CI = CI; ra.CIP = CIP; ra.COP = COP; ra.RS = RS; ra.nsplit = nsplit;
  ra.blocks = (int)(((int64_t)RS * COP * CIP / 4 + 31) / 32);
  return ra;
}
static bool wg8h_group_defer(const Tensor* dy, const Tensor* x, Tensor* dw, const ConvGeom& g, hipStream_t st, const Tensor* affine) {
  const bool on = sw().wgrad_group;
  if (!on || !wgrad_reduce_deferred() || g.N < 8 * (int64_t)num_cus()) return false;
  if (!dy->st->owned || !x->st->owned || !dw->st->owned || (affine && !affine->st->owned)) return false;
  wgrad_park(Wg8hProblem{dy, x, dw, g, affine}, st);
  return true;
}
struct SecondWgradConv { const Tensor* dy; Tensor* dw; const ConvGeom* g; };
void wg8h_launch(const Wg8hProblem& pa, const Wg8hProblem* pb, hipStream_t st, const SecondWgradConv* second, std::vector<WgradReduction>* out) {
  const bool pair = second != nullptr;
  LAMP_CHECK(!(pair && pb), "internal: the sibling pair and the two-layer group do not combine");
  const int RS = 9;
  const int cus = num_cus();
  struct Plan { int ntile, CIP, ips, nsplit, wgs; Hold partial; };
  auto plan = [&](const Wg8hProblem& p, int wg_budget) {
    Plan q;
    q.ntile = (int)((p.g.Cin + WG_CI - 1) / WG_CI);
// ... 5 lines not shown
    q.partial = Hold(new_tensor(ps, 1, kF32, p.x->device()));
    return q;
  };
  Plan A = plan(pa, pb ? cus / 2 : cus), B;
  if (pb) {
    B = plan(*pb, cus / 2);
    if (A.wgs % 8 != 0) {
      Wg8hProblem a1 = pa, b1 = *pb;
      wg8h_launch(a1, nullptr, st, nullptr, out);
      wg8h_launch(b1, nullptr, st, nullptr, out);
      return;
    }
  }
  Hold partial2;
  if (pair) { int64_t ps2[1] = {(int64_t)A.nsplit * IG_M * A.CIP}; partial2 = Hold(new_tensor(ps2, 1, kF32, pa.x->device())); }
  const size_t lds = pair ? 4 * (size_t)(2 * IG_WTILE + WG_XCOPY + 512) : 4 * (size_t)WG_STAGE;
  {
    const double sec_fl = pair ? conv_flops(*second->g) : pb ? conv_flops(pb->g) : 0.0;
    const double sec_by = pair ? conv_bytes(*second->g, 2) - (double)pa.g.N * pa.g.Cin * 64 * 2 : pb ? conv_bytes(pb->g, 2) : 0.0;
    KernelTimer kt("conv_wgrad_igemm", conv_flops(pa.g) + sec_fl, conv_bytes(pa.g, 2) + sec_by, st);
    const bf16_t* dy2p = pair ? second->dy->ptr<bf16_t>() : (const bf16_t*)nullptr;
    float* p2p = pair ? partial2->ptr<float>() : (float*)nullptr;
    const int co2 = pair ? (int)second->g->Cout : 0;
    const float4* affp = pa.affine ? reinterpret_cast<const float4*>(pa.affine->ptr<float>()) : (const float4*)nullptr;
    WgSecondProblem sp{};
    if (pb) {
      sp.dy = pb->dy->ptr<bf16_t>(); sp.x = pb->x->ptr<bf16_t>(); sp.partial = B.partial->ptr<float>();
      sp.CO = (int)pb->g.Cout; sp.CI = (int)pb->g.Cin; sp.CIP = B.CIP; sp.images_per_split = B.ips; sp.ntile = B.ntile;
      sp.affine = pb->affine ? reinterpret_cast<const float4*>(pb->affine->ptr<float>()) : (const float4*)nullptr;
      sp.wgs0 = A.wgs;
    }
    const bool dma = sw().wg8h_dma;
    const auto kfn = pair ? (dma ? ig_wgrad8h_kernel<true, true> : ig_wgrad8h_kernel<true, false>)
                          : (dma ? ig_wgrad8h_kernel<false, true> : ig_wgrad8h_kernel<false, false>);
    allow_big_lds((const void*)kfn);
    hipLaunchKernelGGL(kfn, dim3(A.wgs + (pb ? B.wgs : 0)), dim3(512), lds, st, pa.dy->ptr<bf16_t>(), pa.x->ptr<bf16_t>(), A.partial->ptr<float>(),
                       (int)pa.g.N, (int)pa.g.Cout, (int)pa.g.Cin, A.CIP, A.ips, A.ntile, affp, dy2p, p2p, co2, sp);
    LAMP_LAUNCH_CHECK();
  }
  auto enqueue = [&](const Wg8hProblem& p, Plan& q) {
    const WgradReduceArgs ra = wgrad_reduce_args((int)p.g.Cout, (int)p.g.Cin, q.CIP, IG_M, RS, q.nsplit);
    if (!out) { wgrad_reduce_enqueue(ra, q.partial.get(), p.dw, st); return; }
    out->push_back(WgradReduction{ra, std::move(q.partial), Hold(retain(p.dw))});
  };
  enqueue(pa, A);
  if (pb) enqueue(*pb, B);
  if (pair) wgrad_reduce_enqueue(wgrad_reduce_args((int)second->g->Cout, (int)pa.g.Cin, A.CIP, IG_M, 1, A.nsplit), partial2.get(), second->dw, st);
}
static bool igemm_conv_wgrad_impl(const Tensor* dy, const Tensor* x, Tensor* dw, const ConvGeom& g, hipStream_t st, const Tensor* affine,
                                  const SecondWgradConv* second) {
  if (!ig_qualifies(g, x->dtype)) return false;
  const int KS = g.kh, RS = KS * KS;
  const float4* affp = affine ? reinterpret_cast<const float4*>(affine->ptr<float>()) : (const float4*)nullptr;
  if (affine && !ig_wgrad_folds_affine(g, x->dtype)) return false;
  if (wgrad_takes_eight_wave(g)) {
    if (!second && wg8h_group_defer(dy, x, dw, g, st, affine)) return true;
    Wg8hProblem a{dy, x, dw, g, affine};
    wg8h_launch(a, nullptr, st, second, nullptr);
    return true;
  }
  {
    const bool all_ci = KS == 1 && g.Cin > WG_CI;
    const int ntile = all_ci ? 1 : (int)((g.Cin + WG_CI - 1) / WG_CI);
    const int CIP = g.Cin <= 16 ? 16 : (all_ci ? 4 : ntile) * WG_CI;
    const bool narrow = g.Cout <= 64 || g.Cin <= 16;
    const int COP = narrow ? (int)((g.Cout + 15) / 16) * 16 : IG_M;
    const WgradSplit split = wgrad_split(g.N, num_cus(), ntile);
    const int ips = split.ips, nsplit = split.nsplit;
    int64_t ps[1] = {(int64_t)nsplit * RS * COP * CIP};
    Hold partial(new_tensor(ps, 1, kF32, x->device()));
    const bool pair = second != nullptr;
    if (pair && (KS != 3 || all_ci)) return false;
    const int COP2 = pair ? (int)((second->g->Cout + 15) / 16) * 16 : 0;
    Hold partial2;
    if (pair) { int64_t ps2[1] = {(int64_t)nsplit * COP2 * CIP}; partial2 = Hold(new_tensor(ps2, 1, kF32, x->device())); }
    const size_t lds = all_ci ? 2 * (size_t)(IG_WTILE + 4 * WG_XCOPY + 512) : 2 * (size_t)(WG_STAGE + (pair ? IG_WTILE : 0));
    {
      const double sec_fl = pair ? conv_flops(*second->g) : 0.0;
      const double sec_by = pair ? conv_bytes(*second->g, 2) - (double)g.N * g.Cin * 64 * 2 : 0.0;
      KernelTimer kt("conv_wgrad_igemm", conv_flops(g) + sec_fl, conv_bytes(g, 2) + sec_by, st);
      const bool ci16 = KS == 3 && CIP == 16;
      const void* kfn = ci16    ? (pair ? (const void*)ig_wgrad8v2_kernel<3, true, 1, true, true> : (const void*)ig_wgrad8v2_kernel<3, true, 1, false, true>)
                      : pair    ? (narrow ? (const void*)ig_wgrad8v2_kernel<3, true, 1, true> : (const void*)ig_wgrad8v2_kernel<3, false, 1, true>)
                      : KS == 3 ? (narrow ? (const void*)ig_wgrad8v2_kernel<3, true, 1> : (const void*)ig_wgrad8v2_kernel<3, false, 1>)
                      : all_ci  ? (narrow ? (const void*)ig_wgrad8v2_kernel<1, true, 4> : (const void*)ig_wgrad8v2_kernel<1, false, 4>)
                                : (narrow ? (const void*)ig_wgrad8v2_kernel<1, true, 1> : (const void*)ig_wgrad8v2_kernel<1, false, 1>);
      allow_big_lds(kfn);
      const bf16_t* dyp = dy->ptr<bf16_t>(); const bf16_t* xp = x->ptr<bf16_t>(); float* pp = partial->ptr<float>();
      const bf16_t* dy2p = pair ? second->dy->ptr<bf16_t>() : (const bf16_t*)nullptr;
      float* p2p = pair ? partial2->ptr<float>() : (float*)nullptr;
      int a_N = (int)g.N, a_CO = (int)g.Cout, a_CI = (int)g.Cin, a_CIP = CIP, a_ips = ips, a_COP = COP, a_ntile = ntile;
      int a_CO2 = pair ? (int)second->g->Cout : 0, a_COP2 = COP2;
      void* args[] = {(void*)&dyp, (void*)&xp, (void*)&pp, (void*)&a_N, (void*)&a_CO, (void*)&a_CI, (void*)&a_CIP, (void*)&a_ips, (void*)&a_COP, (void*)&a_ntile,
                      (void*)&dy2p, (void*)&p2p, (void*)&a_CO2, (void*)&a_COP2};
      HIP_CHECK(hipLaunchKernel(kfn, dim3(ntile * nsplit), dim3(256), args, lds, st));
      LAMP_LAUNCH_CHECK();
    }
    wgrad_reduce_enqueue(wgrad_reduce_args((int)g.Cout, (int)g.Cin, CIP, COP, RS, nsplit), partial.get(), dw, st);
    if (pair) wgrad_reduce_enqueue(wgrad_reduce_args((int)second->g->Cout, (int)g.Cin, CIP, COP2, 1, nsplit), partial2.get(), second->dw, st);
    return true;
  }
}
bool igemm_conv_wgrad(const Tensor* dy, const Tensor* x, Tensor* dw, const ConvGeom& g, hipStream_t st, const Tensor* affine) {
  return igemm_conv_wgrad_impl(dy, x, dw, g, st, affine, nullptr);
}
bool igemm_conv_wgrad_pair(const Tensor* dy, const Tensor* dy1, const Tensor* x, Tensor* dw, Tensor* dw1, const ConvGeom& g, const ConvGeom& g1, hipStream_t st) {
  if (!sw().conv_wgrad_pair) return false;
  if (!ig_qualifies(g, x->dtype) || !ig_qualifies(g1, x->dtype) || g.kh != 3 || g1.kh != 1) return false;
  if (g.Cin != g1.Cin || g.N != g1.N) return false;
  const SecondWgradConv sw{dy1, dw1, &g1};
  return igemm_conv_wgrad_impl(dy, x, dw, g, st, nullptr, &sw);
}

}

#ifdef LAMP_WG8H_STAMPS
extern "C" int lamp_debug_wg8h_stamps(unsigned int* out, int n) {
  (void)hipDeviceSynchronize();
  return (int)hipMemcpyFromSymbol(out, HIP_SYMBOL(lamp::g_wg8h_stamps), (size_t)n * 4);
}
#endif
```

### lamp_amd/csrc/kernels/conv_narrow.hip

```cpp
#include "device_utils.h"
#include "conv_geom.h"
#include "wgrad_reduce.h"
#include <map>
#include <type_traits>
#include <mutex>
#include <tuple>
#include <vector>
#include "conv_narrow_pack.h"
#include "../core/switches.h"

namespace lamp {

typedef nv_s8 __attribute__((aligned(2))) nv_s8_u;
typedef float nv_f4 __attribute__((ext_vector_type(4)));

struct NcvGeom {
  int N, C, CO;
  int H, W;
  int Hs, Ws;
  int top, left, dil;
  int Ho, Wo;
  int sh, sw, wx;
  int kh;
  int kh_inv;
// ... 83 lines not shown
    ncv_stage(xs, src + (int64_t)n * q.C * q.H * q.W, q, tid, 256);
    __syncthreads();
    first = false;
    bf16_t* yp = dst + (int64_t)n * q.CO * HoWo;
    for (int tile = wid; tile < ntiles; tile += 4) {
      const int p = min(tile * 16 + (lane & 15), HoWo - 1);
      const int ho = p / q.Wo, wo = p - ho * q.Wo;
      const char* base = smem + ((ho * q.sh) * q.Ws + wo * q.sw + q.wx) * 2;
      nv_f4 acc = {0.f, 0.f, 0.f, 0.f};
#pragma unroll
      for (int ks = 0; ks < NK; ks++) {
        const nv_s8 a = *reinterpret_cast<const nv_s8_u*>(base + koff[ks]);
        acc = __builtin_amdgcn_mfma_f32_16x16x32_bf16(__builtin_bit_cast(nv_bf8, a), wfr[ks], acc, 0, 0, 0);
      }
      const int p4 = tile * 16 + (lane >> 4) * 4;
      if (co < q.CO && p4 < HoWo) {
        const bf16_t o0(acc[0] + bv), o1(acc[1] + bv), o2(acc[2] + bv), o3(acc[3] + bv);
        uint2 pk;
        pk.x = (unsigned)o0.bits | ((unsigned)o1.bits << 16);
        pk.y = (unsigned)o2.bits | ((unsigned)o3.bits << 16);
        *reinterpret_cast<uint2*>(yp + co * HoWo + p4) = pk;
      }
    }
  }
  (void)first;
}

#if defined(NCV_SKIP) && (NCV_SKIP & 2)
#define NCV_STORE_COND && pk[0] == 0x12345678u
#else
#define NCV_STORE_COND
#endif
#ifdef NCV_STAMP
__device__ unsigned long long ncv_stamps[1024 * 8];
#define NCV_STAMP_AT(k) do { if (threadIdx.x == 0 && blockIdx.x < 1024) ncv_stamps[blockIdx.x * 8 + (k)] = __builtin_amdgcn_s_memtime(); } while (0)
#define NCV_STAMP_ONCE(k) do { if (n == (int)blockIdx.x) NCV_STAMP_AT(k); } while (0)
#else
#define NCV_STAMP_AT(k) do { } while (0)
#define NCV_STAMP_ONCE(k) do { } while (0)
#endif
template <int I0, int I1, class F> __device__ __forceinline__ void ncv_static_for(F&& f) {
  if constexpr (I0 < I1) { f(std::integral_constant<int, I0>{}); ncv_static_for<I0 + 1, I1>(f); }
}
struct NcvWf { float n, mean, m2; };
__device__ __forceinline__ NcvWf ncv_wf_merge(const NcvWf& a, const NcvWf& b) {
  NcvWf r;
  r.n = a.n + b.n;
  if (r.n == 0.f) { r.mean = 0.f; r.m2 = 0.f; return r; }
  const float d = b.mean - a.mean, f = b.n / r.n;
  r.mean = a.mean + d * f;
  r.m2 = a.m2 + b.m2 + d * d * a.n * f;
  return r;
}
template <int NK, int SW, int PH0, int NS, bool ADD, bool STATS, bool PAR = false>
__global__ __launch_bounds__(256, (STATS && NK <= 5) ? 3 : 1) void ncv_fwd2_kernel(const bf16_t* __restrict__ src, const nv_bf8* __restrict__ wpk, const bf16_t* __restrict__ bias,
                                                       bf16_t* dst, NcvGeom q, const bf16_t* add, bf16_t* dst2, const bf16_t* __restrict__ bias2, int co_a,
                                                       float* __restrict__ stats, float* __restrict__ stats2, int stats_per_wg,
                                                       const bf16_t* __restrict__ src2) {
  __shared__ float sst[STATS ? 2 : 1][4][16][3];
  extern __shared__ __attribute__((aligned(16))) char smem[];
  unsigned short* xs = reinterpret_cast<unsigned short*>(smem);
  NCV_STAMP_AT(0);
  constexpr int P = 8 / SW;
  constexpr int ND = P / NS;
  constexpr int NSEG = (PH0 + (ND - 1) * NS * SW + 7) < 16 ? 2 : 3;
  const int tid = threadIdx.x, lane = tid & 63, wid = tid >> 6, nthreads = blockDim.x, nwaves = nthreads >> 6;
  const int co = NS == 2 ? (lane & 7) : (lane & 15);
  const int ncg = q.Wo / P, TR = 16 / ncg;
  const int64_t img_in = (int64_t)q.C1 * q.H * q.W, img_in2 = (int64_t)(q.C - q.C1) * q.H * q.W;
  NcvPre pre;
  const NcvPlan plan = ncv_stage_plan(q, tid, nthreads);
  if (q.pf && (int)blockIdx.x < q.N) ncv_stage_load(pre, plan, src + blockIdx.x * img_in, src2 + blockIdx.x * img_in2);
  nv_bf8 wfr[NK];
  int koff[NK];
#pragma unroll
  for (int ks = 0; ks < NK; ks++) {
    wfr[ks] = wpk[ks * 64 + lane];
    int pair = ks * 4 + (lane >> 4);
    const int pairs1 = q.C1 * q.kh;
    if (pair >= pairs1 + (q.C - q.C1)) pair = 0;
    int c = (pair * q.kh_inv) >> 16, r = pair - c * q.kh;
    if (pair >= pairs1) { c = q.C1 + (pair - pairs1); r = q.kh >> 1; }
    if constexpr (PAR) {
      const int pr = ks * 4 + (lane >> 4);
      if (ks < NK / 2) { c = pr >> 1; r = 2 * (pr & 1); if (c >= q.C1) { c = 0; r = 0; } }
      else {
        const int p2 = pr - (NK / 2) * 4;
        if (p2 < q.C1) { c = p2; r = 1; }
        else if (p2 < q.C) { c = p2; r = 1; }
        else { c = 0; r = 0; }
      }
    }
    koff[ks] = (c * q.Hs + r) * q.Ws * 2;
  }
  const float bv = co < co_a ? (bias ? (float)bias[co] : 0.f) : ((bias2 && co < q.CO) ? (float)bias2[co - co_a] : 0.f);
#ifdef NCV_STAMP
  __builtin_amdgcn_s_waitcnt(0);
  NCV_STAMP_AT(1);
#endif
  const int HoWo = q.Ho * q.Wo, nsuper = q.Ho / TR;
  const int img_elems = q.C * q.Hs * q.Ws;
  for (int o = tid * 8; o < img_elems; o += nthreads * 8) *reinterpret_cast<uint4*>(xs + o) = make_uint4(0, 0, 0, 0);
  const int a_tr = (lane & 15) / ncg, a_cg = (lane & 15) - a_tr * ncg;
  const int a_off = ((PAR ? 2 : 1) * a_tr * q.sh * q.Ws + a_cg * 8 + (q.wx - PH0)) * 2;
  auto stats_flush = [&](int part, int nparts, int par) {
    if (wid == 0 && lane < (NS == 2 ? 8 : 16) && lane < q.CO) {
      float cnt = 0.f, sy = 0.f, sq = 0.f;
      for (int h = 0; h < NS; h++)
        for (int k = 0; k < nwaves; k++) { cnt += sst[par][k][lane + 8 * h][0]; sy += sst[par][k][lane + 8 * h][1]; sq += sst[par][k][lane + 8 * h][2]; }
      const float mean = sy / cnt;
      float* o = lane < co_a ? stats + ((int64_t)lane * nparts + part) * 3 : stats2 + ((int64_t)(lane - co_a) * nparts + part) * 3;
      o[0] = cnt; o[1] = mean; o[2] = fmaxf(sq - sy * mean, 0.f);
    }
  };
  nv_f4 st1 = nv_f4{0.f, 0.f, 0.f, 0.f}, st2 = nv_f4{0.f, 0.f, 0.f, 0.f};
  int tiles = 0;
  auto stats_leave = [&](int par) {
    const int j = lane & 15, r = j & 3;
    const float sq = r == 0 ? st2[0] : r == 1 ? st2[1] : r == 2 ? st2[2] : st2[3];
    if ((lane >> 4) == (j >> 2)) { sst[par][wid][j][0] = (float)(tiles * (16 * P / NS)); sst[par][wid][j][1] = st1[0]; sst[par][wid][j][2] = sq; }
    st1 = nv_f4{0.f, 0.f, 0.f, 0.f}; st2 = nv_f4{0.f, 0.f, 0.f, 0.f}; tiles = 0;
  };
  const unsigned ones2 = 0x3f803f80u;
  typedef unsigned int nv_u4 __attribute__((ext_vector_type(4)));
  const nv_bf8 ones = __builtin_bit_cast(nv_bf8, nv_u4{ones2, ones2, ones2, ones2});
  auto stats_take = [&](unsigned a, unsigned b, unsigned c, unsigned d) {
    const nv_bf8 y = __builtin_bit_cast(nv_bf8, nv_u4{a, b, c, d});
    st1 = __builtin_amdgcn_mfma_f32_16x16x32_bf16(ones, y, st1, 0, 0, 0);
    st2 = __builtin_amdgcn_mfma_f32_16x16x32_bf16(y, y, st2, 0, 0, 0);
  };
  int it = 0;
  for (int n = blockIdx.x; n < q.N; n += gridDim.x, it++) {
    __syncthreads();
    NCV_STAMP_ONCE(2);
    if (STATS && !stats_per_wg && it > 0) stats_flush(n - (int)gridDim.x, q.N, (it - 1) & 1);
#if defined(NCV_SKIP) && (NCV_SKIP & 4)
    if (n < 0)
#endif
    {
    if (q.pf) ncv_stage_store(xs, pre, plan, q.dil);
    else ncv_stage(xs, src + n * img_in, q, tid, nthreads);
    }
    __syncthreads();
    NCV_STAMP_ONCE(3);
#if defined(NCV_SKIP) && (NCV_SKIP & 4)
    if (n < 0)
#endif
    if (q.pf && n + (int)gridDim.x < q.N)
      ncv_stage_load(pre, plan, src + (n + (int)gridDim.x) * img_in, src2 + (n + (int)gridDim.x) * img_in2);
    bf16_t* yc = co < co_a ? dst + ((int64_t)n * co_a + co) * HoWo : dst2 + ((int64_t)n * (q.CO - co_a) + (co - co_a)) * HoWo;
    for (int st = wid; st < nsuper; st += nwaves) {
      constexpr int RS = PAR ? 2 : 1;
      const int h0 = PAR ? (st >> 1) * (2 * TR) + (st & 1) : st * TR;
      const char* base = smem + a_off + h0 * q.sh * q.Ws * 2;
      nv_f4 acc[ND];
#pragma unroll
      for (int d = 0; d < ND; d++) acc[d] = nv_f4{0.f, 0.f, 0.f, 0.f};
#ifdef NCV_SKIP
      if (NCV_SKIP & 1) { acc[0][0] = (float)lane; }
      else
#endif
      {
      auto kstep = [&](auto ksc) {
        constexpr int ks = decltype(ksc)::value;
        unsigned int sg[NSEG * 4 + 1];
#pragma unroll
        for (int e = 0; e < NSEG; e++) {
          const uint4 v = *reinterpret_cast<const uint4*>(base + koff[ks] + e * 16);
          sg[e * 4 + 0] = v.x; sg[e * 4 + 1] = v.y; sg[e * 4 + 2] = v.z; sg[e * 4 + 3] = v.w;
        }
        sg[NSEG * 4] = 0;
#pragma unroll
        for (int d = 0; d < ND; d++) {
          const int o = PH0 + d * NS * SW;
          const int dq = o >> 1;
          unsigned int f[4];
#pragma unroll
          for (int j = 0; j < 4; j++) f[j] = (o & 1) ? __builtin_amdgcn_alignbit(sg[dq + j + 1], sg[dq + j], 16) : sg[dq + j];
          typedef unsigned int u4v __attribute__((ext_vector_type(4)));
          const u4v fv = {f[0], f[1], f[2], f[3]};
          acc[d] = __builtin_amdgcn_mfma_f32_16x16x32_bf16(__builtin_bit_cast(nv_bf8, fv), wfr[ks], acc[d], 0, 0, 0);
        }
      };
      if constexpr (PAR) {
        if (((h0 + q.top) & 1) == 0) ncv_static_for<0, NK / 2>(kstep);
        else ncv_static_for<NK / 2, NK>(kstep);
      } else ncv_static_for<0, NK>(kstep);
      }
      constexpr int NROW = NS == 1 ? 4 : 2;
      const int row0 = (lane >> 4) * 4 + (NS == 1 ? 0 : ((lane >> 3) & 1) * 2);
      uint4 addv[NROW];
      if (ADD && co < q.CO) {
// ... 143 lines not shown
      const int rc = q.W >> 3, total = q.Cin * q.H * rc;
      for (int i = tid; i < total; i += 256) {
        const int b = i % rc, a = (i / rc) % q.H, c = i / (rc * q.H);
        const uint4 v = *reinterpret_cast<const uint4*>(xp + (c * q.H + a) * q.W + b * 8);
        if (SW == 1) {
          *reinterpret_cast<uint4*>(xi + (c * q.Hs + q.ph + a) * q.Ws + NCV_LEFT + b * 8) = v;
        } else {
          uint2 ev, od;
          ev.x = (v.x & 0xffffu) | (v.y << 16); ev.y = (v.z & 0xffffu) | (v.w << 16);
          od.x = (v.x >> 16) | (v.y & 0xffff0000u); od.y = (v.z >> 16) | (v.w & 0xffff0000u);
          unsigned short* row = xi + ((c * q.Hs + q.ph + a) * 2) * q.Ws + NCV_OFF2 + b * 4;
          *reinterpret_cast<uint2*>(row) = ev;
          *reinterpret_cast<uint2*>(row + q.Ws) = od;
        }
      }
      const bf16_t* dp = dy + (nb + im) * q.Cout * HoWo;
      unsigned short* di = ds + im * 16 * HoWo;
      const int dtot = q.Cout * HoWo >> 3;
      for (int i = tid; i < dtot; i += 256) *reinterpret_cast<uint4*>(di + i * 8) = *reinterpret_cast<const uint4*>(dp + i * 8);
    }
    __syncthreads();
    const int nchunks = ig * chunks_per_img;
    for (int ch = wid; ch < nchunks; ch += 4) {
      const int pg = ch * 32 + (lane >> 4) * 8;
      const int im = pg / HoWo, pp = pg - im * HoWo;
      const int ho = pp / q.Wo, wo0 = pp - ho * q.Wo;
      const nv_s8 a = *reinterpret_cast<const nv_s8*>(ds + (im * 16 + (lane & 15)) * HoWo + pp);
      const char* xb = reinterpret_cast<const char*>(xs + im * ximg) +
                       (SW == 1 ? (ho * q.Ws + wo0) * 2 : ((ho * 2) * 2 * q.Ws + wo0) * 2);
#pragma unroll
      for (int nt = 0; nt < NT; nt++) {
        const nv_s8 b = *reinterpret_cast<const nv_s8_u*>(xb + coff[nt]);
        acc[nt] = __builtin_amdgcn_mfma_f32_16x16x32_bf16(__builtin_bit_cast(nv_bf8, a), __builtin_bit_cast(nv_bf8, b), acc[nt], 0, 0, 0);
      }
    }
  }
#pragma unroll
  for (int nt = 0; nt < NT; nt++)
#pragma unroll
    for (int rr = 0; rr < 4; rr++) red[(wid * 16 + (lane >> 4) * 4 + rr) * (NT * 16) + nt * 16 + (lane & 15)] = acc[nt][rr];
  __syncthreads();
  const int O = q.Cout * q.ncol;
  for (int i = tid; i < O; i += 256) {
    const int co = i / q.ncol, cidx = i - co * q.ncol;
    float a = 0.f;
#pragma unroll
    for (int w = 0; w < 4; w++) a += red[(w * 16 + co) * (NT * 16) + cidx];
    partial[(int64_t)blockIdx.x * O + i] = a;
  }
}

constexpr int NCV_OFFA = 8;
constexpr int NCV_WPF = 6;
template <int KW, int PW, int SW, int NPT>
__global__ __launch_bounds__(256) void ncv_wgrad2_kernel(const bf16_t* __restrict__ dy, const bf16_t* __restrict__ x, float* __restrict__ partial, NcvWGeom q,
                                                         int images_per_block, const bf16_t* __restrict__ dy2, float* __restrict__ partial2) {
  extern __shared__ __attribute__((aligned(16))) char smem[];
  const int tid = threadIdx.x, lane = tid & 63, wid = tid >> 6;
  const int HoWo = q.Ho * q.Wo;
  const int ximg = q.Cin * q.Hs * q.Ws * (SW == 2 ? 2 : 1);
  unsigned short* xs = reinterpret_cast<unsigned short*>(smem);
  unsigned short* ds = xs + q.IG * ximg;
  constexpr int NCOLT = NPT * KW * 16;
  float* red = reinterpret_cast<float*>(ds + q.IG * 16 * HoWo);
  {
    const int tot = q.IG * (ximg + 16 * HoWo);
    for (int o = tid * 8; o < tot; o += 256 * 8) *reinterpret_cast<uint4*>(xs + o) = make_uint4(0, 0, 0, 0);
  }
  const int npairs = q.Cin * q.kh;
  int poff[NPT];
#pragma unroll
  for (int pt = 0; pt < NPT; pt++) {
    int pair = pt * 16 + (lane & 15);
    if (pair >= npairs) pair = 0;
    const int ci = pair / q.kh, r = pair - ci * q.kh;
    poff[pt] = (SW == 1 ? (ci * q.Hs + r) * q.Ws : (ci * q.Hs + r) * 2 * q.Ws) * 2;
  }
  nv_f4 acc[NPT][KW];
#pragma unroll
  for (int pt = 0; pt < NPT; pt++)
#pragma unroll
    for (int s = 0; s < KW; s++) acc[pt][s] = nv_f4{0.f, 0.f, 0.f, 0.f};

  const int64_t n0 = (int64_t)blockIdx.x * images_per_block, n1 = min<int64_t>(n0 + images_per_block, q.N);
  const int chunks_per_img = HoWo >> 5;
  const int xpk = (q.Cin * q.H * q.W) >> 3, dpk = (q.Cout * HoWo) >> 3, dpk2 = (q.Cout2 * HoWo) >> 3, per = xpk + dpk + dpk2;
  const int rc = q.W >> 3;
  const bool pf = q.IG * per <= NCV_WPF * 256;
  uint4 pre[NCV_WPF];
  int p_src[NCV_WPF], p_dst[NCV_WPF], p_im[NCV_WPF];
#pragma unroll
  for (int k = 0; k < NCV_WPF; k++) {
    const int idx = tid + k * 256;
    const int im = idx / per, j = idx - im * per;
    p_im[k] = (pf && im < q.IG) ? im : -1;
    if (j < xpk) {
      const int b = j % rc, a = (j / rc) % q.H, c = j / (rc * q.H);
      p_src[k] = im * q.Cin * q.H * q.W + j * 8;
      p_dst[k] = im * ximg + (SW == 1 ? (c * q.Hs + q.ph + a) * q.Ws + NCV_OFFA + b * 8 : ((c * q.Hs + q.ph + a) * 2) * q.Ws + NCV_OFFA + b * 4);
    } else if (j < xpk + dpk) {
      p_src[k] = -(im * q.Cout * HoWo + (j - xpk) * 8) - 1;
      p_dst[k] = q.IG * ximg + im * 16 * HoWo + (j - xpk) * 8;
    } else {
      p_src[k] = -(im * q.Cout2 * HoWo + (j - xpk - dpk) * 8) - 1 - (1 << 30);
      p_dst[k] = q.IG * ximg + im * 16 * HoWo + q.Cout * HoWo + (j - xpk - dpk) * 8;
    }
  }
  auto pre_load = [&](int64_t nb, int ig) {
    const bf16_t* xg = x + nb * q.Cin * q.H * q.W;
    const bf16_t* dg = dy + nb * q.Cout * HoWo;
    const bf16_t* dg2 = dy2 + nb * q.Cout2 * HoWo;
#pragma unroll
    for (int k = 0; k < NCV_WPF; k++)
      if (p_im[k] >= 0 && p_im[k] < ig) {
        const bf16_t* sp = p_src[k] >= 0 ? xg + p_src[k] : p_src[k] >= -(1 << 30) ? dg + (-p_src[k] - 1) : dg2 + (-p_src[k] - 1 - (1 << 30));
        pre[k] = *reinterpret_cast<const uint4*>(sp);
      }
  };
  auto stage_x = [&](unsigned short* dst, const uint4 v) {
    if (SW == 1) {
      *reinterpret_cast<uint4*>(dst) = v;
    } else {
      uint2 ev, od;
      ev.x = (v.x & 0xffffu) | (v.y << 16); ev.y = (v.z & 0xffffu) | (v.w << 16);
      od.x = (v.x >> 16) | (v.y & 0xffff0000u); od.y = (v.z >> 16) | (v.w & 0xffff0000u);
      *reinterpret_cast<uint2*>(dst) = ev;
      *reinterpret_cast<uint2*>(dst + q.Ws) = od;
    }
  };
  auto pre_store = [&](int ig) {
#pragma unroll
    for (int k = 0; k < NCV_WPF; k++) {
      if (p_im[k] < 0 || p_im[k] >= ig) continue;
      const uint4 v = pre[k];
      if (SW == 1 || p_src[k] < 0) *reinterpret_cast<uint4*>(xs + p_dst[k]) = v;
      else stage_x(xs + p_dst[k], v);
    }
  };
  auto x_dst = [&](unsigned short* xi, int j) {
    const int b = j % rc, a = (j / rc) % q.H, c = j / (rc * q.H);
    return xi + (SW == 1 ? (c * q.Hs + q.ph + a) * q.Ws + NCV_OFFA + b * 8 : ((c * q.Hs + q.ph + a) * 2) * q.Ws + NCV_OFFA + b * 4);
  };

  if (pf && n0 < n1) pre_load(n0, (int)min<int64_t>(q.IG, n1 - n0));
  for (int64_t nb = n0; nb < n1; nb += q.IG) {
    const int ig = (int)min<int64_t>(q.IG, n1 - nb);
    __syncthreads();
#if defined(NCV_WSKIP) && (NCV_WSKIP & 4)
    if (nb < 0)
#endif
    if (pf) pre_store(ig);
    else for (int im = 0; im < ig; im++) {
      const bf16_t* xp = x + (nb + im) * q.Cin * q.H * q.W;
      unsigned short* xi = xs + im * ximg;
      for (int i = tid; i < xpk; i += 256) stage_x(x_dst(xi, i), *reinterpret_cast<const uint4*>(xp + i * 8));
      const bf16_t* dp = dy + (nb + im) * q.Cout * HoWo;
      unsigned short* di = ds + im * 16 * HoWo;
      for (int i = tid; i < dpk; i += 256) *reinterpret_cast<uint4*>(di + i * 8) = *reinterpret_cast<const uint4*>(dp + i * 8);
      const bf16_t* dp2 = dy2 + (nb + im) * q.Cout2 * HoWo;
      for (int i = tid; i < dpk2; i += 256) *reinterpret_cast<uint4*>(di + q.Cout * HoWo + i * 8) = *reinterpret_cast<const uint4*>(dp2 + i * 8);
    }
    __syncthreads();
#if defined(NCV_WSKIP) && (NCV_WSKIP & 4)
    if (nb < 0)
#endif
    if (pf && nb + q.IG < n1) pre_load(nb + q.IG, (int)min<int64_t>(q.IG, n1 - nb - q.IG));
    const int nchunks = ig * chunks_per_img;
#if defined(NCV_WSKIP) && (NCV_WSKIP & 1)
    if (nb < 0)
#endif
    for (int ch = wid; ch < nchunks; ch += 4) {
      const int pg = ch * 32 + (lane >> 4) * 8;
      const int im = pg / HoWo, pp = pg - im * HoWo;
      const int ho = pp / q.Wo, wo0 = pp - ho * q.Wo;
      const nv_s8 a = *reinterpret_cast<const nv_s8*>(ds + (im * 16 + (lane & 15)) * HoWo + pp);
      const nv_bf8 af = __builtin_bit_cast(nv_bf8, a);
      const char* xb = reinterpret_cast<const char*>(xs + im * ximg) +
                       (SW == 1 ? (ho * q.Ws + wo0 + NCV_OFFA - 8) * 2 : ((ho * 2) * 2 * q.Ws + wo0 + NCV_OFFA - 8) * 2);
#pragma unroll
      for (int pt = 0; pt < NPT; pt++) {
        const char* rowp = xb + poff[pt];
        if (SW == 1) {
          constexpr bool need_m = PW > 0, need_p = (KW - 1 - PW) > 0;
          unsigned int sg[13];
          const uint4 z = make_uint4(0, 0, 0, 0);
          const uint4 v0 = need_m ? *reinterpret_cast<const uint4*>(rowp) : z;
          const uint4 v1 = *reinterpret_cast<const uint4*>(rowp + 16);
          const uint4 v2 = need_p ? *reinterpret_cast<const uint4*>(rowp + 32) : z;
          sg[0] = v0.x; sg[1] = v0.y; sg[2] = v0.z; sg[3] = v0.w; sg[4] = v1.x; sg[5] = v1.y; sg[6] = v1.z; sg[7] = v1.w;
          sg[8] = v2.x; sg[9] = v2.y; sg[10] = v2.z; sg[11] = v2.w; sg[12] = 0;
#pragma unroll
          for (int s = 0; s < KW; s++) {
            const int o = 8 + s - PW;
            const int dq = o >> 1;
            typedef unsigned int u4v __attribute__((ext_vector_type(4)));
            u4v f;
#pragma unroll
            for (int j = 0; j < 4; j++) f[j] = (o & 1) ? __builtin_amdgcn_alignbit(sg[dq + j + 1], sg[dq + j], 16) : sg[dq + j];
            acc[pt][s] = __builtin_amdgcn_mfma_f32_16x16x32_bf16(af, __builtin_bit_cast(nv_bf8, f), acc[pt][s], 0, 0, 0);
          }
        } else {
          unsigned int sg[2][9];
#pragma unroll
          for (int par = 0; par < 2; par++) {
            const uint4 v0 = *reinterpret_cast<const uint4*>(rowp + par * q.Ws * 2);
            const uint4 v1 = *reinterpret_cast<const uint4*>(rowp + par * q.Ws * 2 + 16);
            sg[par][0] = v0.x; sg[par][1] = v0.y; sg[par][2] = v0.z; sg[par][3] = v0.w;
            sg[par][4] = v1.x; sg[par][5] = v1.y; sg[par][6] = v1.z; sg[par][7] = v1.w; sg[par][8] = 0;
// ... 120 lines not shown
  const bool on = sw().pack_after_step;
  if (!on) return;
  std::lock_guard<std::mutex> lk(g_ncv_mu);
  if (g_ncv_cache.empty()) return;
  std::vector<const Tensor*> cand;
  for (int i = 0; i < n; i++) {
    const Tensor* w = params[i];
    if (!w || !w->is_device() || w->dtype != kBF16 || w->ndim != 4 || !w->st->owned || !w->is_contiguous()) continue;
    if (w->sizes[0] > 16 || w->sizes[1] > 16) continue;
    cand.push_back(w);
  }
  if (cand.empty()) return;
  auto find = [&](uint64_t uid, int64_t offset, int co, int ci, int kh, int kw) -> const Tensor* {
    for (const Tensor* w : cand)
      if (w->st->uid == uid && w->offset == offset && (int)w->sizes[0] == co && (int)w->sizes[1] == ci && (int)w->sizes[2] == kh && (int)w->sizes[3] == kw)
        return w;
    return nullptr;
  };
  NcvPackMany a;
  int cnt = 0;
  auto flush = [&] {
    if (cnt == 0) return;
    ncv_pack_launch(a, cnt, st);
    cnt = 0;
  };
  for (auto it = g_ncv_cache.begin(); it != g_ncv_cache.end();) {
    const NcvPackKey& k = it->first;
    NcvPackVal& v = it->second;
    if (k.st != st) { ++it; continue; }
    const Tensor* w1 = find(k.uid, k.offset, k.Cout, k.Cin, k.kh, k.kw);
    const Tensor* w2 = k.Cout2 > 0 ? find(k.uid2, k.offset2, k.Cout2, k.Cin, 1, 1) : nullptr;
    if (!w1 && !w2) { ++it; continue; }
    if (!w1 || (k.Cout2 > 0 && !w2)) {
      if (!v.pinned) { release(v.packed); it = g_ncv_cache.erase(it); }
      else ++it;
      continue;
    }
    if (cnt == NCV_PACK_MAX) flush();
    a.w[cnt] = NcvW{w1->ptr<bf16_t>(), k.Cout, k.Cin, k.kh, k.kw, k.dgrad, k.ns & 15, k.sw, w2 ? w2->ptr<bf16_t>() : nullptr, k.Cout2, k.ns >> 4};
    a.dst[cnt] = static_cast<nv_bf8*>(v.packed->raw());
    v.version = w1->st->version.load(std::memory_order_relaxed);
    v.version2 = w2 ? w2->st->version.load(std::memory_order_relaxed) : 0;
    v.tick = ++g_ncv_tick;
    cnt++;
    ++it;
  }
  if (fill && cnt > 0) { *fill = a; *fill_cnt = cnt; }
  else flush();
}
void narrow_pack_launch(const NcvPackMany& a, int cnt, hipStream_t st) { ncv_pack_launch(a, cnt, st); }

struct NcvSibling { const Tensor* w; const Tensor* bias; Tensor* out; };
struct NcvSecondGrad { const Tensor* dy; const Tensor* w; };
static bool ncv_run(const Tensor* in, const Tensor* w, const Tensor* bias, Tensor* out, const ConvGeom& g, bool dgrad, hipStream_t st,
                    const Tensor* addend = nullptr, bool* addend_fused = nullptr, const NcvSibling* sib = nullptr,
                    const NcvSecondGrad* second = nullptr) {
  if (addend_fused) *addend_fused = false;
  if (!ncv_common(g, in->dtype)) return false;
  const int cout2 = sib ? (int)sib->w->sizes[0] : second ? (int)second->w->sizes[0] : 0;
  if (sib && (dgrad || g.Cout + cout2 > 16)) return false;
  if (second && (!dgrad || sib || cout2 > 16)) return false;
  NcvGeom q;
  q.N = (int)g.N; q.kh = g.kh; q.pf = 0; q.kh_inv = 65536 / g.kh + 1;
  if (!dgrad) {
    if (g.W % 8 != 0) return false;
    q.C = (int)g.Cin; q.C1 = q.C; q.CO = (int)g.Cout + cout2; q.H = (int)g.H; q.W = (int)g.W; q.dil = 1;
    q.top = g.ph; q.left = NCV_LEFT;
    q.Ho = (int)g.Ho; q.Wo = (int)g.Wo; q.sh = g.sh; q.sw = g.sw; q.wx = NCV_LEFT - g.pw;
    q.Hs = std::max((int)g.H + 2 * g.ph, (q.Ho - 1) * g.sh + g.kh);
    q.Ws = round_up(std::max(NCV_LEFT + (int)g.W, (q.Wo - 1) * g.sw + q.wx + 8), 8);
  } else {
    const int pt = g.kh - 1 - g.ph, pl = g.kw - 1 - g.pw;
    q.C1 = (int)g.Cout; q.C = q.C1 + (second ? cout2 : 0); q.CO = (int)g.Cin; q.H = (int)g.Ho; q.W = (int)g.Wo; q.dil = g.sh;
    if (q.dil == 1 && q.W % 8 != 0) return false;
    q.top = pt; q.left = NCV_LEFT;
    q.Ho = (int)g.H; q.Wo = (int)g.W; q.sh = 1; q.sw = 1; q.wx = NCV_LEFT - pl;
    q.Hs = std::max(pt + ((int)g.Ho - 1) * g.sh + 1, (int)g.H + g.kh - 1);
    q.Ws = round_up(std::max(NCV_LEFT + ((int)g.Wo - 1) * g.sw + 1, (int)g.W - 1 + q.wx + 8), 8);
  }
  if ((q.Ho * q.Wo) % 4 != 0) return false;
  const int P = 8 / q.sw, ph0 = q.wx & 7;
  bool aligned = q.Wo % P == 0 && (ph0 == 0 || ph0 == 6 || ph0 == 7);
  int ncg = aligned ? q.Wo / P : 0;
  if (aligned && !(ncg == 2 || ncg == 4 || ncg == 8 || ncg == 16)) aligned = false;
  if (aligned && q.Ho % (16 / ncg) != 0) aligned = false;
  if (aligned) q.Ws = round_up(std::max(q.Ws, q.Wo * q.sw + (q.wx - ph0) + 16), 8);
  if ((sib || second) && !aligned) return false;
  const int pairs = q.C1 * q.kh + (q.C - q.C1);
  const int nk_real = (pairs + 3) / 4;
  static const int nk_opts[] = {1, 2, 4, 5, 6, 8, 12, 16};
  int NK = 0;
  for (int o : nk_opts) if (o >= nk_real) { NK = o; break; }
  if (!NK) return false;
  int nke = 0;
  const bool par_on = sw().ncv_dgrad_parity;
  if (par_on && aligned && dgrad && second && q.dil == 2 && g.kh == 3 && NK > 5) {
    const int nk2 = NK <= 6 ? 6 : NK <= 8 ? 8 : 16;
    const int need_e = (q.C1 * 2 + 3) / 4, need_o = (q.C + 3) / 4;
    if (need_e <= nk2 / 2 && need_o <= nk2 / 2 && q.Ho % (2 * (16 / ncg)) == 0) nke = nk2 / 2;
  }
  const bool pitch_on = sw().ncv_pitch;
  if (pitch_on && aligned) {
    const int rs = (nke > 0 ? 2 : 1) * q.sh;
    for (int k = 0; k < 16; k++) {
      const int step = (rs * ((q.Ws >> 3) + k)) & 15;
      if (step % ncg == 0 && ((step / ncg) & 1) == 1 && (size_t)q.C * q.Hs * (q.Ws + 8 * k) * 2 <= 64 * 1024) { q.Ws += 8 * k; break; }
    }
  }
  const size_t lds = (size_t)q.C * q.Hs * q.Ws * 2;
  if (lds > 64 * 1024) return false;
  const bool two_shift_on = sw().ncv_two_shift;
  const int NS = (two_shift_on && aligned && q.CO <= 8 && g.kw + q.sw <= 8) ? 2 : 1;
  const Tensor* wsecond = sib ? sib->w : second ? second->w : nullptr;
  const NcvW wq{w->ptr<bf16_t>(), (int)g.Cout, (int)g.Cin, g.kh, g.kw, dgrad ? 1 : 0, NS, q.sw, wsecond ? wsecond->ptr<bf16_t>() : (const bf16_t*)nullptr, cout2, nke};
  Hold wpk_h(ncv_packed_weights(w, wq, st, wsecond));
  const nv_bf8* wpk = reinterpret_cast<const nv_bf8*>(static_cast<const Tensor*>(wpk_h.get())->ptr<bf16_t>());
  const int max_per_cu = (int)sw().ncv_per_cu;
  const int lds_per_cu = (int)std::max<size_t>(1, std::min<size_t>(max_per_cu, (size_t)(150 * 1024) / std::max<size_t>(lds, 1)));
  const bf16_t* bp = bias ? bias->ptr<bf16_t>() : (const bf16_t*)nullptr;
  if (aligned) {
    const int nsuper = q.Ho / (16 / ncg);
    const int threads = 64 * std::min(4, nsuper);
    q.pf = (q.W % 8 == 0 && (int64_t)q.C * q.H * q.W <= (int64_t)NCV_PF * threads * 8) ? 1 : 0;
    if (second && !q.pf) return false;
    if (NK > 12 && !second) return false;
    const int NK2 = nke > 0 ? 2 * nke : NK <= 2 ? 2 : (NK <= 4 ? 4 : (NK <= 5 ? 5 : (NK <= 6 && second ? 6 : (NK <= 8 && second ? 8 : (NK <= 12 ? 12 : 16)))));
    const void* kfn = nullptr;
    const bool with_add = addend != nullptr && q.sw == 1;
    const bool bn_stats = sw().conv_bn_stats && sw().ncv_bn_stats;
    const bool with_stats = bn_stats && !dgrad && !addend && g.N >= 2 && (int64_t)q.Ho * q.Wo >= 64 && (sib || conv_stats_wanted(w->st->uid));
#define NCV_F2(NKv, SWv, PHv, ADDv, STv) kfn = NS == 2 ? (const void*)ncv_fwd2_kernel<NKv, SWv, PHv, 2, ADDv, STv> : (const void*)ncv_fwd2_kernel<NKv, SWv, PHv, 1, ADDv, STv>
#define NCV_F2_PH(NKv, SWv, ADDv, STv) do { if (ph0 == 0) NCV_F2(NKv, SWv, 0, ADDv, STv); else if (ph0 == 6) NCV_F2(NKv, SWv, 6, ADDv, STv); else NCV_F2(NKv, SWv, 7, ADDv, STv); } while (0)
#define NCV_F2_SW(NKv) do { if (with_stats) { if (q.sw == 1) NCV_F2_PH(NKv, 1, false, true); else NCV_F2_PH(NKv, 2, false, true); }                \
                            else if (q.sw == 1) { if (with_add) NCV_F2_PH(NKv, 1, true, false); else NCV_F2_PH(NKv, 1, false, false); }                \
                            else NCV_F2_PH(NKv, 2, false, false); } while (0)
#define NCV_F2P(NKv, PHv, ADDv) kfn = NS == 2 ? (const void*)ncv_fwd2_kernel<NKv, 1, PHv, 2, ADDv, false, true> : (const void*)ncv_fwd2_kernel<NKv, 1, PHv, 1, ADDv, false, true>
#define NCV_F2P_PH(NKv, ADDv) do { if (ph0 == 0) NCV_F2P(NKv, 0, ADDv); else if (ph0 == 6) NCV_F2P(NKv, 6, ADDv); else NCV_F2P(NKv, 7, ADDv); } while (0)
#define NCV_F2_PAIR(NKv) do { if (nke > 0) { if (with_add) NCV_F2P_PH(NKv, true); else NCV_F2P_PH(NKv, false); }                                   \
                              else if (with_add) NCV_F2_PH(NKv, 1, true, false); else NCV_F2_PH(NKv, 1, false, false); } while (0)
    switch (NK2) {
      case 2: NCV_F2_SW(2); break;
      case 4: NCV_F2_SW(4); break;
      case 5: NCV_F2_SW(5); break;
      case 6: NCV_F2_PAIR(6); break;
      case 8: NCV_F2_PAIR(8); break;
      case 16: NCV_F2_PAIR(16); break;
      default: NCV_F2_SW(12); break;
    }
#undef NCV_F2_PAIR
#undef NCV_F2P_PH
#undef NCV_F2P
#undef NCV_F2_SW
#undef NCV_F2_PH
#undef NCV_F2
    const int per_cu = std::min(lds_per_cu, kernel_occupancy(kfn, threads, lds));
    const int blocks = (int)std::min<int64_t>(g.N, (int64_t)num_cus() * per_cu);
    const double sib_fl = sib ? 2.0 * (double)g.N * cout2 * (double)g.Ho * g.Wo * (double)g.Cin : 0.0;
    const double sib_by = sib ? ((double)g.N * cout2 * g.Ho * g.Wo + (double)cout2 * g.Cin) * 2.0 : 0.0;
    const double sec_fl = second ? 2.0 * (double)g.N * cout2 * (double)g.Ho * g.Wo * (double)g.Cin : 0.0;
    const double sec_by = second ? ((double)g.N * cout2 * g.Ho * g.Wo + (double)cout2 * g.Cin) * 2.0 : 0.0;
    KernelTimer kt(dgrad ? "conv_dgrad_narrow" : "conv_fwd_narrow", conv_flops(g) + sib_fl + sec_fl, conv_bytes(g, 2) + sib_by + sec_by, st);
    const bf16_t* srcp = in->ptr<bf16_t>();
    const bf16_t* src2p = second ? second->dy->ptr<bf16_t>() : (const bf16_t*)nullptr;
    bf16_t* dstp = out->ptr<bf16_t>();
    const bf16_t* addp = with_add ? addend->ptr<bf16_t>() : (const bf16_t*)nullptr;
    if (addend_fused) *addend_fused = with_add;
    bf16_t* dst2p = sib ? sib->out->ptr<bf16_t>() : (bf16_t*)nullptr;
    const bf16_t* bias2p = (sib && sib->bias) ? sib->bias->ptr<bf16_t>() : (const bf16_t*)nullptr;
    int co_a = sib ? (int)g.Cout : q.CO;
    Hold statt, statt2;
    float* statp = nullptr;
    float* stat2p = nullptr;
    int stats_per_wg = g.N % blocks == 0 ? 1 : 0;
    const int parts = stats_per_wg ? blocks : (int)g.N;
    if (with_stats) {
      int64_t ps[1] = {(int64_t)parts * g.Cout * 3};
      statt = Hold(new_tensor(ps, 1, kF32, in->device()));
      statp = statt->ptr<float>();
      if (sib) {
        int64_t ps2[1] = {(int64_t)parts * cout2 * 3};
        statt2 = Hold(new_tensor(ps2, 1, kF32, in->device()));
        stat2p = statt2->ptr<float>();
      }
    }
    void* args[] = {(void*)&srcp, (void*)&wpk, (void*)&bp, (void*)&dstp, (void*)&q, (void*)&addp, (void*)&dst2p, (void*)&bias2p, (void*)&co_a,
                    (void*)&statp, (void*)&stat2p, (void*)&stats_per_wg, (void*)&src2p};
    HIP_CHECK(hipLaunchKernel(kfn, dim3(blocks), dim3(threads), args, lds, st));
    LAMP_LAUNCH_CHECK();
    if (statt.get()) conv_stats_publish(out, statt.get(), parts, sib ? 0 : w->st->uid);
    if (statt2.get()) conv_stats_publish(sib->out, statt2.get(), parts);
    return true;
  }
  if (NK > 12) return false;
  const int blocks = (int)std::min<int64_t>(g.N, (int64_t)num_cus() * lds_per_cu);
  KernelTimer kt(dgrad ? "conv_dgrad_narrow" : "conv_fwd_narrow", conv_flops(g), conv_bytes(g, 2), st);
  switch (NK) {
    case 1: ncv_launch<1>(in->ptr<bf16_t>(), wpk, bp, out->ptr<bf16_t>(), q, blocks, lds, st); break;
    case 2: ncv_launch<2>(in->ptr<bf16_t>(), wpk, bp, out->ptr<bf16_t>(), q, blocks, lds, st); break;
    case 4: ncv_launch<4>(in->ptr<bf16_t>(), wpk, bp, out->ptr<bf16_t>(), q, blocks, lds, st); break;
    case 5: ncv_launch<5>(in->ptr<bf16_t>(), wpk, bp, out->ptr<bf16_t>(), q, blocks, lds, st); break;
    case 6: case 8: ncv_launch<8>(in->ptr<bf16_t>(), wpk, bp, out->ptr<bf16_t>(), q, blocks, lds, st); break;
    default: ncv_launch<12>(in->ptr<bf16_t>(), wpk, bp, out->ptr<bf16_t>(), q, blocks, lds, st); break;
  }
  LAMP_LAUNCH_CHECK();
  return true;
}

bool narrow_conv_fwd(const Tensor* x, const Tensor* w, const Tensor* bias, Tensor* y, const ConvGeom& g, hipStream_t st) {
  return ncv_run(x, w, bias, y, g, false, st);
}
bool narrow_conv_fwd_pair(const Tensor* x, const Tensor* w, const Tensor* bias, Tensor* y, const ConvGeom& g, const Tensor* w1, const Tensor* bias1,
                          Tensor* y1, const ConvGeom& g1, hipStream_t st) {
  const bool on = sw().conv_sibling;
  if (!on || x->dtype != kBF16) return false;
  if (g.kh != 3 || g.kw != 3 || g.ph != 1 || g.pw != 1 || g1.kh != 1 || g1.kw != 1 || g1.ph != 0 || g1.pw != 0) return false;
  if (g.sh != g1.sh || g.sw != g1.sw || g.Ho != g1.Ho || g.Wo != g1.Wo || g.Cin != g1.Cin || g.N != g1.N || g.groups != 1 || g1.groups != 1) return false;
  if (g.dh != 1 || g.dw != 1 || g1.dh != 1 || g1.dw != 1) return false;
  const NcvSibling sb{w1, bias1, y1};
  return ncv_run(x, w, bias, y, g, false, st, nullptr, nullptr, &sb);
}
bool narrow_conv_dgrad(const Tensor* dy, const Tensor* w, Tensor* dx, const ConvGeom& g, hipStream_t st, const Tensor* addend, bool* addend_fused) {
  return ncv_run(dy, w, nullptr, dx, g, true, st, addend, addend_fused);
}
bool narrow_conv_dgrad_pair(const Tensor* dy, const Tensor* w, const ConvGeom& g, const Tensor* dy1, const Tensor* w1, const ConvGeom& g1, Tensor* dx,
                            hipStream_t st, const Tensor* addend, bool* addend_fused) {
  if (addend_fused) *addend_fused = false;
  const bool on = sw().conv_dgrad_pair;
  if (!on || dy->dtype != kBF16 || dy1->dtype != kBF16) return false;
  if (g.kh != 3 || g.kw != 3 || g.ph != 1 || g.pw != 1 || g1.kh != 1 || g1.kw != 1 || g1.ph != 0 || g1.pw != 0) return false;
  if (g.sh != g1.sh || g.sw != g1.sw || g.Ho != g1.Ho || g.Wo != g1.Wo || g.H != g1.H || g.W != g1.W || g.Cin != g1.Cin || g.N != g1.N) return false;
  if (g.groups != 1 || g1.groups != 1 || g.dh != 1 || g.dw != 1 || g1.dh != 1 || g1.dw != 1 || g1.Cout > 16) return false;
  const NcvSecondGrad sg{dy1, w1};
  return ncv_run(dy, w, nullptr, dx, g, true, st, addend, addend_fused, nullptr, &sg);
}

template <int NT, int SW>
static void ncv_wg_launch(const bf16_t* dy, const bf16_t* x, float* partial, const NcvWGeom& q, int ipb, int blocks, size_t lds, hipStream_t st) {
  static bool attr = false;
  allow_big_lds((const void*)ncv_wgrad_kernel<NT, SW>);
  hipLaunchKernelGGL((ncv_wgrad_kernel<NT, SW>), dim3(blocks), dim3(256), lds, st, dy, x, partial, q, ipb);
}

struct NcvSecondWgrad { const Tensor* dy; Tensor* dw; };
static bool ncv_wgrad_run(const Tensor* dy, const Tensor* x, Tensor* dw, const ConvGeom& g, hipStream_t st, const NcvSecondWgrad* second) {
  if (!ncv_common(g, x->dtype)) return false;
  if (g.W % 8 != 0 || g.Wo % 8 != 0 || (g.Ho * g.Wo) % 32 != 0) return false;
  const int cout2 = second ? (int)second->dy->sizes[1] : 0;
  if (second && (g.Cout + cout2 > 16 || g.kh != 3 || g.kw != 3 || g.ph != 1 || g.pw != 1)) return false;
  NcvWGeom q;
  q.N = (int)g.N; q.Cin = (int)g.Cin; q.Cout = (int)g.Cout; q.H = (int)g.H; q.W = (int)g.W; q.Ho = (int)g.Ho; q.Wo = (int)g.Wo;
  q.kh = g.kh; q.kw = g.kw; q.ph = g.ph; q.pw = g.pw; q.Cout2 = cout2;
  q.ncol = (int)g.Cin * g.kh * g.kw;
  const int SW = g.sh;
  q.Hs = std::max((int)g.H + 2 * g.ph, ((int)g.Ho - 1) * g.sh + g.kh);
  if (SW == 1) q.Ws = round_up(std::max(NCV_LEFT + (int)g.W, (int)g.Wo - 1 + g.kw - 1 - g.pw + NCV_LEFT + 1), 8);
  else {
    const int half_max = (g.kw - 1 - g.pw) >> 1;
    q.Ws = round_up(std::max((int)g.W / 2, (int)g.Wo + half_max) + NCV_OFF2 + 1, 8);
  }
  const int HoWo = (int)(g.Ho * g.Wo);
  q.IG = std::max(1, 256 / HoWo);
  const int npt = (int)((g.Cin * g.kh + 15) / 16);
  const bool aligned = g.kh == g.kw && npt <= 3 &&
                       ((g.kw == 5 && g.pw == 2 && SW == 1) || (g.kw == 3 && g.pw == 1) || (g.kw == 1 && g.pw == 0));
  if (aligned) {
    if (SW == 1) q.Ws = round_up(NCV_OFFA + std::max((int)g.W, (int)g.Wo + 8) + 8, 8);
    else q.Ws = round_up(NCV_OFFA + std::max((int)g.W / 2, (int)g.Wo) + 8, 8);
    const int ximg2 = q.Cin * q.Hs * q.Ws * (SW == 2 ? 2 : 1);
    const int ncolt = npt * g.kw * 16;
    const size_t lds2 = (size_t)q.IG * (ximg2 + 16 * HoWo) * 2 + (size_t)4 * 16 * ncolt * 4;
    if (lds2 <= 150 * 1024) {
      const int O = q.Cout * q.ncol;
      const void* kfn = nullptr;
#define NCV_WG2(KWv, PWv, SWv, NPTv) kfn = (const void*)ncv_wgrad2_kernel<KWv, PWv, SWv, NPTv>
#define NCV_WG2_NPT(KWv, PWv, SWv) do { if (npt == 1) NCV_WG2(KWv, PWv, SWv, 1); else if (npt == 2) NCV_WG2(KWv, PWv, SWv, 2); else NCV_WG2(KWv, PWv, SWv, 3); } while (0)
      if (g.kw == 5) NCV_WG2_NPT(5, 2, 1);
      else if (g.kw == 3 && SW == 1) NCV_WG2_NPT(3, 1, 1);
      else if (g.kw == 3) NCV_WG2_NPT(3, 1, 2);
      else if (SW == 1) NCV_WG2_NPT(1, 0, 1);
      else NCV_WG2_NPT(1, 0, 2);
#undef NCV_WG2_NPT
#undef NCV_WG2
      allow_big_lds(kfn);
      const int per_cu = std::min((int)std::max<size_t>(1, std::min<size_t>(4, (size_t)(150 * 1024) / lds2)), kernel_occupancy(kfn, 256, lds2));
      const int64_t rounds = (g.N + q.IG - 1) / q.IG;
      const int nb = (int)std::min<int64_t>(rounds, (int64_t)num_cus() * per_cu);
      const int ipb = (int)((rounds + nb - 1) / nb) * q.IG;
      const int nblocks = (int)((g.N + ipb - 1) / ipb);
      int64_t ps[1] = {(int64_t)nblocks * O};
      Hold partial(new_tensor(ps, 1, kF32, dy->device()));
      const int O2 = cout2 * q.Cin;
      Hold partial2;
      if (second) { int64_t ps2[1] = {(int64_t)nblocks * O2}; partial2 = Hold(new_tensor(ps2, 1, kF32, dy->device())); }
      {
        const double sec_fl = second ? 2.0 * (double)g.N * cout2 * (double)g.Ho * g.Wo * (double)g.Cin : 0.0;
        const double sec_by = second ? ((double)g.N * cout2 * g.Ho * g.Wo + (double)cout2 * g.Cin) * 2.0 : 0.0;
        KernelTimer kt("conv_wgrad_narrow", conv_flops(g) + sec_fl, conv_bytes(g, 2) + sec_by, st);
        const bf16_t* dp = dy->ptr<bf16_t>(); const bf16_t* xp = x->ptr<bf16_t>(); float* pp = partial->ptr<float>();
        const bf16_t* dp2 = second ? second->dy->ptr<bf16_t>() : (const bf16_t*)nullptr;
        float* pp2 = second ? partial2->ptr<float>() : (float*)nullptr;
        int ipb_arg = ipb;
        void* args[] = {(void*)&dp, (void*)&xp, (void*)&pp, (void*)&q, (void*)&ipb_arg, (void*)&dp2, (void*)&pp2};
        HIP_CHECK(hipLaunchKernel(kfn, dim3(nblocks), dim3(256), args, lds2, st));
        LAMP_LAUNCH_CHECK();
      }
      WgradReduceArgs ra{};
      ra.kind = 1; ra.O = O; ra.nsplit = nblocks; ra.blocks = (int)(((int64_t)O * 64 + 255) / 256);
      wgrad_reduce_enqueue(ra, partial.get(), dw, st);
      if (second) {
        WgradReduceArgs rb{};
        rb.kind = 1; rb.O = O2; rb.nsplit = nblocks; rb.blocks = (int)(((int64_t)O2 * 64 + 255) / 256);
        wgrad_reduce_enqueue(rb, partial2.get(), second->dw, st);
      }
      return true;
    }
    if (second) return false;
    if (SW == 1) q.Ws = round_up(std::max(NCV_LEFT + (int)g.W, (int)g.Wo - 1 + g.kw - 1 - g.pw + NCV_LEFT + 1), 8);
    else { const int half_max = (g.kw - 1 - g.pw) >> 1; q.Ws = round_up(std::max((int)g.W / 2, (int)g.Wo + half_max) + NCV_OFF2 + 1, 8); }
  }
  if (second) return false;
  const int nt_real = (q.ncol + 15) / 16;
  static const int nt_opts[] = {1, 2, 4, 5, 9};
  int NT = 0;
  for (int o : nt_opts) if (o >= nt_real) { NT = o; break; }
  if (!NT) return false;
  const int ximg = q.Cin * q.Hs * q.Ws * (SW == 2 ? 2 : 1);
  if ((q.IG * (ximg + 16 * HoWo)) % 8 != 0) return false;
  const size_t lds = (size_t)q.IG * (ximg + 16 * HoWo) * 2 + (size_t)4 * 16 * NT * 16 * 4;
  if (lds > 150 * 1024) return false;
  const int O = q.Cout * q.ncol;
  const int per_cu = (int)std::max<size_t>(1, std::min<size_t>(4, (size_t)(150 * 1024) / lds));
  const int64_t rounds = (g.N + q.IG - 1) / q.IG;
  const int nb = (int)std::min<int64_t>(rounds, (int64_t)num_cus() * per_cu);
  const int ipb = (int)((rounds + nb - 1) / nb) * q.IG;
  const int nblocks = (int)((g.N + ipb - 1) / ipb);
  int64_t ps[1] = {(int64_t)nblocks * O};
  Hold partial(new_tensor(ps, 1, kF32, dy->device()));
  {
    KernelTimer kt("conv_wgrad_narrow", conv_flops(g), conv_bytes(g, 2), st);
    const bf16_t* dp = dy->ptr<bf16_t>(); const bf16_t* xp = x->ptr<bf16_t>(); float* pp = partial->ptr<float>();
#define NCV_WG(NTv)                                                                                          \
  do {                                                                                                       \
    if (SW == 1) ncv_wg_launch<NTv, 1>(dp, xp, pp, q, ipb, nblocks, lds, st);                                \
    else ncv_wg_launch<NTv, 2>(dp, xp, pp, q, ipb, nblocks, lds, st);                                        \
  } while (0)
    switch (NT) {
      case 1: NCV_WG(1); break;
      case 2: NCV_WG(2); break;
      case 4: NCV_WG(4); break;
      case 5: NCV_WG(5); break;
      default: NCV_WG(9); break;
    }
#undef NCV_WG
    LAMP_LAUNCH_CHECK();
  }
  WgradReduceArgs ra{};
  ra.kind = 1; ra.O = O; ra.nsplit = nblocks; ra.blocks = (int)(((int64_t)O * 64 + 255) / 256);
  wgrad_reduce_enqueue(ra, partial.get(), dw, st);
  return true;
}

bool narrow_conv_wgrad(const Tensor* dy, const Tensor* x, Tensor* dw, const ConvGeom& g, hipStream_t st) { return ncv_wgrad_run(dy, x, dw, g, st, nullptr); }
bool narrow_conv_wgrad_pair(const Tensor* dy, const Tensor* dy1, const Tensor* x, Tensor* dw, Tensor* dw1, const ConvGeom& g, const ConvGeom& g1, hipStream_t st) {
  const bool on = sw().conv_wgrad_pair;
  if (!on || x->dtype != kBF16 || dy->dtype != kBF16 || dy1->dtype != kBF16) return false;
  if (g1.kh != 1 || g1.kw != 1 || g1.ph != 0 || g1.pw != 0) return false;
  if (g.sh != g1.sh || g.sw != g1.sw || g.Ho != g1.Ho || g.Wo != g1.Wo || g.H != g1.H || g.W != g1.W || g.Cin != g1.Cin || g.N != g1.N) return false;
  if (g.groups != 1 || g1.groups != 1 || g.dh != 1 || g.dw != 1 || g1.dh != 1 || g1.dw != 1) return false;
  const NcvSecondWgrad sw{dy1, dw1};
  return ncv_wgrad_run(dy, x, dw, g, st, &sw);
}

}
```

### lamp_amd/csrc/kernels/device_utils.h

```cpp
#pragma once
#include <hip/hip_runtime.h>
#include <cstdint>
#include <type_traits>
#include "../core/tensor.h"

namespace lamp {

struct alignas(2) bf16_t {
  uint16_t bits;
  bf16_t() = default;
  __host__ __device__ explicit bf16_t(float f) {
#if defined(__HIP_DEVICE_COMPILE__)
    __bf16 h = (__bf16)f;
    bits = __builtin_bit_cast(uint16_t, h);
#else
    uint32_t u;
    memcpy(&u, &f, 4);
    if ((u & 0x7fffffffu) > 0x7f800000u) { bits = (uint16_t)((u >> 16) | 0x40); }
    else { bits = (uint16_t)((u + 0x7fffu + ((u >> 16) & 1u)) >> 16); }
#endif
  }
  __host__ __device__ explicit operator float() const {
    uint32_t u = ((uint32_t)bits) << 16;
#if defined(__HIP_DEVICE_COMPILE__)
    return __builtin_bit_cast(float, u);
#else
    float f;
    memcpy(&f, &u, 4);
    return f;
#endif
  }
};

__device__ __forceinline__ unsigned add_bf16x2(unsigned a, unsigned b) {
  const float lo = __uint_as_float(a << 16) + __uint_as_float(b << 16);
  const float hi = __uint_as_float(a & 0xffff0000u) + __uint_as_float(b & 0xffff0000u);
  return (unsigned)bf16_t(lo).bits | ((unsigned)bf16_t(hi).bits << 16);
}
__device__ __forceinline__ uint4 add_bf16x8(const uint4& a, const uint4& b) {
  return make_uint4(add_bf16x2(a.x, b.x), add_bf16x2(a.y, b.y), add_bf16x2(a.z, b.z), add_bf16x2(a.w, b.w));
}

__device__ __forceinline__ uint4 nt_load16(const uint4* p) {
  typedef unsigned int nt_u4 __attribute__((ext_vector_type(4)));
  const nt_u4 v = __builtin_nontemporal_load(reinterpret_cast<const nt_u4*>(p));
  return make_uint4(v[0], v[1], v[2], v[3]);
}
__device__ __forceinline__ void nt_store16(uint4* p, const uint4& v) {
  typedef unsigned int nt_u4 __attribute__((ext_vector_type(4)));
  const nt_u4 t = {v.x, v.y, v.z, v.w};
  __builtin_nontemporal_store(t, reinterpret_cast<nt_u4*>(p));
}

struct alignas(2) f16_t {
  uint16_t bits;
  f16_t() = default;
  __host__ __device__ explicit f16_t(float f) { _Float16 h = (_Float16)f; bits = __builtin_bit_cast(uint16_t, h); }
  __host__ __device__ explicit operator float() const { return (float)__builtin_bit_cast(_Float16, bits); }
};

template <class T> struct acc_type { using type = T; };
template <> struct acc_type<f16_t> { using type = float; };
template <> struct acc_type<bf16_t> { using type = float; };
template <> struct acc_type<float> { using type = float; };
template <> struct acc_type<double> { using type = double; };
template <> struct acc_type<int64_t> { using type = int64_t; };
template <> struct acc_type<int32_t> { using type = int64_t; };
template <> struct acc_type<uint8_t> { using type = int64_t; };
template <class T> using acc_t = typename acc_type<T>::type;

template <class A, class T> __host__ __device__ inline A load_as(const T& v) { return (A)v; }
template <> __host__ __device__ inline float load_as<float, bf16_t>(const bf16_t& v) { return (float)v; }
template <> __host__ __device__ inline double load_as<double, bf16_t>(const bf16_t& v) { return (double)(float)v; }
template <> __host__ __device__ inline int64_t load_as<int64_t, bf16_t>(const bf16_t& v) { return (int64_t)(float)v; }

template <> __host__ __device__ inline float load_as<float, f16_t>(const f16_t& v) { return (float)v; }
template <> __host__ __device__ inline double load_as<double, f16_t>(const f16_t& v) { return (double)(float)v; }
template <> __host__ __device__ inline int64_t load_as<int64_t, f16_t>(const f16_t& v) { return (int64_t)(float)v; }

template <class T, class A> __host__ __device__ inline T store_as(A v) { return (T)v; }
template <> __host__ __device__ inline f16_t store_as<f16_t, float>(float v) { return f16_t(v); }
template <> __host__ __device__ inline f16_t store_as<f16_t, double>(double v) { return f16_t((float)v); }
template <> __host__ __device__ inline f16_t store_as<f16_t, int64_t>(int64_t v) { return f16_t((float)v); }
template <> __host__ __device__ inline bf16_t store_as<bf16_t, float>(float v) { return bf16_t(v); }
template <> __host__ __device__ inline bf16_t store_as<bf16_t, double>(double v) { return bf16_t((float)v); }
template <> __host__ __device__ inline bf16_t store_as<bf16_t, int64_t>(int64_t v) { return bf16_t((float)v); }

template <class T, int N> struct alignas(sizeof(T) * N) Vec {
  T v[N];
};
template <class T> constexpr int vec_width() { return 16 / sizeof(T); }

#define LAMP_DISPATCH_FLOAT(DT, T, ...)                                                           \
// ... 69 lines not shown
```

Measured before the change: 2.219 million samples/s.

## Fold batch-norm+relu into narrow 6/16-channel convolution forward and weight-gradient kernels

```diff
diff --git a/lamp_amd/csrc/core/switches.h b/lamp_amd/csrc/core/switches.h
--- a/lamp_amd/csrc/core/switches.h
+++ b/lamp_amd/csrc/core/switches.h
@@ -12,6 +12,7 @@
   X(fuse_pool_logsoftmax, "LAMP_FUSE_POOL_LOGSOFTMAX", BOOL, 1, 0, "average pool -> flatten -> log-softmax tail as one node")             \
   X(fuse_block_tail, "LAMP_FUSE_BLOCK_TAIL", BOOL, 1, 0, "the last residual block and the pooled log-softmax tail as one node")          \
   X(fuse_bn_conv, "LAMP_FUSE_BN_CONV", BOOL, 1, 0, "batch norm -> relu -> convolution: the convolution applies the norm while staging")  \
+  X(fuse_bn_conv_narrow, "LAMP_FUSE_BN_CONV_NARROW", BOOL, 1, 0, "... also in the kernels of the 6- and 16-channel layers: narrow forward / weight gradient, igemm 64-row forward and four-wave weight gradient") \
   X(fuse_loss_accumulate, "LAMP_FUSE_LOSS_ACCUMULATE", BOOL, 1, 0, "acc += n * loss inside the NLL loss kernel")                          \
   X(fuse_loss_backward, "LAMP_FUSE_LOSS_BACKWARD", BOOL, 1, 0, "the NLL loss backward goes straight to the pooled log-softmax node's input in one launch")                      \
   X(fuse_loss_tail, "LAMP_FUSE_LOSS_TAIL", BOOL, 1, 0, "the loss launch also writes the pooled log-softmax's input gradient per plane")  \
diff --git a/lamp_amd/csrc/kernels/conv.hip b/lamp_amd/csrc/kernels/conv.hip
--- a/lamp_amd/csrc/kernels/conv.hip
+++ b/lamp_amd/csrc/kernels/conv.hip
@@ -1,6 +1,7 @@
 #include "device_utils.h"
 #include "../core/strided.h"
 #include "conv_geom.h"
+#include "../core/switches.h"
 
 namespace lamp {
 
@@ -266,7 +267,8 @@
 bool igemm_conv_dgrad(const Tensor* dy, const Tensor* w, Tensor* dx, const ConvGeom& g, hipStream_t st, const Tensor* addend = nullptr,
                       bool* addend_fused = nullptr);
 bool igemm_conv_wgrad(const Tensor* dy, const Tensor* x, Tensor* dw, const ConvGeom& g, hipStream_t st, const Tensor* affine = nullptr);
-bool igemm_conv_folds_affine(const ConvGeom& g, int dtype);
+bool igemm_conv_fwd_folds_affine(const ConvGeom& g, int dtype);
+bool igemm_conv_wgrad_folds_affine(const ConvGeom& g, int dtype);
 bool igemm_conv_fwd_affine(const Tensor* x, const Tensor* affine, const Tensor* w, const Tensor* bias, Tensor* y, const ConvGeom& g, hipStream_t st);
 bool igemm32_conv_fwd(const Tensor* x, const Tensor* w, const Tensor* bias, Tensor* y, const ConvGeom& g, hipStream_t st);
 bool igemm32_conv_dgrad(const Tensor* dy, const Tensor* w, Tensor* dx, const ConvGeom& g, hipStream_t st, const Tensor* addend = nullptr,
@@ -281,7 +283,10 @@
                             hipStream_t st, const Tensor* addend, bool* addend_fused);
 bool igemm_conv_dgrad_pair(const Tensor* dy, const Tensor* w, const ConvGeom& g, const Tensor* dy1, const Tensor* w1, const ConvGeom& g1, Tensor* dx,
                            hipStream_t st, const Tensor* addend, bool* addend_fused);
-bool narrow_conv_wgrad(const Tensor* dy, const Tensor* x, Tensor* dw, const ConvGeom& g, hipStream_t st);
+bool narrow_conv_wgrad(const Tensor* dy, const Tensor* x, Tensor* dw, const ConvGeom& g, hipStream_t st, const Tensor* affine = nullptr);
+bool narrow_conv_fwd_affine(const Tensor* x, const Tensor* affine, const Tensor* w, const Tensor* bias, Tensor* y, const ConvGeom& g, hipStream_t st);
+bool narrow_conv_fwd_folds_affine(const ConvGeom& g, int dtype);
+bool narrow_conv_wgrad_folds_affine(const ConvGeom& g, int dtype);
 bool narrow_conv_wgrad_pair(const Tensor* dy, const Tensor* dy1, const Tensor* x, Tensor* dw, Tensor* dw1, const ConvGeom& g, const ConvGeom& g1, hipStream_t st);
 bool igemm_conv_wgrad_pair(const Tensor* dy, const Tensor* dy1, const Tensor* x, Tensor* dw, Tensor* dw1, const ConvGeom& g, const ConvGeom& g1, hipStream_t st);
 bool small_conv_fwd(const Tensor* x, const Tensor* w, const Tensor* bias, Tensor* y, const ConvGeom& g, hipStream_t st);
@@ -315,6 +320,17 @@
     LAMP_LAUNCH_CHECK();
   }
   return y.take();
+}
+struct BnConvFold {
+  enum Arm { None, Igemm, Narrow } fwd, wgrad;
+  bool both() const { return fwd != None && wgrad != None; }
+};
+static BnConvFold bn_conv_fold(const ConvGeom& g, int dtype) {
+  const bool narrow_on = sw().fuse_bn_conv_narrow;
+  BnConvFold f;
+  f.fwd = igemm_conv_fwd_folds_affine(g, dtype) ? BnConvFold::Igemm : (narrow_on && narrow_conv_fwd_folds_affine(g, dtype)) ? BnConvFold::Narrow : BnConvFold::None;
+  f.wgrad = igemm_conv_wgrad_folds_affine(g, dtype) ? BnConvFold::Igemm : (narrow_on && narrow_conv_wgrad_folds_affine(g, dtype)) ? BnConvFold::Narrow : BnConvFold::None;
+  return f;
 }
 static Tensor* contiguous_filter(const Tensor* w) {
   Tensor* c = contiguous(w);
@@ -443,7 +459,7 @@
   if (!x->is_device() || !w->is_device() || x->dtype != w->dtype) return 0;
   const int64_t zero2[2] = {0, 0};
   ConvGeom g = make_geom(x, w, stride, padding, dilation, nspatial, 0, zero2, groups);
-  *out = igemm_conv_folds_affine(g, x->dtype) ? 1 : 0;
+  *out = bn_conv_fold(g, x->dtype).both() ? 1 : 0;
   LAMP_API_END
 }
 int lamp_convolution_bn_relu_input(lamp_tensor** out, const lamp_tensor* x, const lamp_tensor* affine, const lamp_tensor* w, const lamp_tensor* bias,
@@ -461,7 +477,11 @@
   if (nspatial == 2) oshape.push_back(g.Ho);
   oshape.push_back(g.Wo);
   Hold y(new_tensor(oshape, x->dtype, x->device()));
-  if (!igemm_conv_fwd_affine(xc.get(), affine, wc.get(), bc.get(), y.get(), g, st)) {
+  const BnConvFold::Arm arm = bn_conv_fold(g, x->dtype).fwd;
+  const bool folded = arm == BnConvFold::Igemm    ? igemm_conv_fwd_affine(xc.get(), affine, wc.get(), bc.get(), y.get(), g, st)
+                      : arm == BnConvFold::Narrow ? narrow_conv_fwd_affine(xc.get(), affine, wc.get(), bc.get(), y.get(), g, st) : false;
+  LAMP_CHECK(folded || arm == BnConvFold::None, "internal: the kernel chosen to fold the batch norm into this convolution refused it");
+  if (!folded) {
     Hold act(bn_relu_materialise(xc.get(), affine, st));
     lamp_tensor* o = nullptr;
     if (lamp_convolution(&o, act.get(), wc.get(), bc.get(), stride, padding, dilation, nspatial, 0, zero2, groups) != 0) throw Error(lamp_last_error());
@@ -485,7 +505,10 @@
   bool dw_done = false;
   if (mask[1]) {
     dw = Hold(new_like(wc.get()));
-    dw_done = igemm_conv_wgrad(gc.get(), xc.get(), dw.get(), g, st, affine);
+    const BnConvFold::Arm arm = bn_conv_fold(g, x->dtype).wgrad;
+    dw_done = arm == BnConvFold::Igemm    ? igemm_conv_wgrad(gc.get(), xc.get(), dw.get(), g, st, affine)
+              : arm == BnConvFold::Narrow ? narrow_conv_wgrad(gc.get(), xc.get(), dw.get(), g, st, affine) : false;
+    LAMP_CHECK(dw_done || arm == BnConvFold::None, "internal: the kernel chosen to rebuild relu(bn(x)) for this weight gradient refused it");
   }
   const bool need_act = mask[1] && !dw_done;
   Hold act(need_act ? bn_relu_materialise(xc.get(), affine, st) : nullptr);
diff --git a/lamp_amd/csrc/kernels/conv_igemm.hip b/lamp_amd/csrc/kernels/conv_igemm.hip
--- a/lamp_amd/csrc/kernels/conv_igemm.hip
+++ b/lamp_amd/csrc/kernels/conv_igemm.hip
@@ -336,11 +336,12 @@
   epilogue(y, bias, stats, addend);
 }
 
-template <int KS, int SIBM = 0>
+template <int KS, int SIBM = 0, bool AFF = false>
 __global__ __launch_bounds__(256) void ig_conv8c_kernel(const bf16_t* __restrict__ x, const bf16_t* __restrict__ wp, const bf16_t* __restrict__ bias,
                                                         bf16_t* __restrict__ y, int N, int CI, int KP, int CO, float* __restrict__ stats,
-                                                        const bf16_t* addend, const IgSibling sib) {
+                                                        const bf16_t* addend, const IgSibling sib, const float4* __restrict__ affine) {
   static_assert(SIBM == 0 || (SIBM == 2 && KS == 3), "second-source input gradients of a 3x3 only");
+  static_assert(!AFF || (SIBM == 0 && KS == 3), "the batch-norm table goes with a plain 3x3 forward");
   extern __shared__ __attribute__((aligned(16))) char smem[];
   constexpr int RS = KS * KS;
   constexpr int PAD = (KS - 1) / 2;
@@ -390,7 +391,10 @@
       for (int k = 0; k < 8; k++) {
         const int c = cg * 8 + k;
         uint4 v = make_uint4(0, 0, 0, 0);
-        if (c < CI && n < N) v = *reinterpret_cast<const uint4*>(x + ((int64_t)n * CI + c) * 64 + h * 8);
+        if (c < CI && n < N) {
+          v = *reinterpret_cast<const uint4*>(x + ((int64_t)n * CI + c) * 64 + h * 8);
+          if constexpr (AFF) { const float4 a = affine[c]; v = bn_relu_bf16x8(v, a.x, a.y, a.z); }
+        }
         w[k][0] = v.x; w[k][1] = v.y; w[k][2] = v.z; w[k][3] = v.w;
       }
       char* xi = Xl + img * XIMG;
@@ -542,18 +546,6 @@
   }
 }
 
-__device__ __forceinline__ uint4 ig_bn_relu_x8(uint4 v, float mu, float scale, float bb) {
-  unsigned* w = &v.x;
-#pragma unroll
-  for (int q = 0; q < 4; q++) {
-    const float x0 = __uint_as_float(w[q] << 16), x1 = __uint_as_float(w[q] & 0xffff0000u);
-    bf16_t o0(__builtin_fmaf(x0 - mu, scale, bb)), o1(__builtin_fmaf(x1 - mu, scale, bb));
-    if ((float)o0 < 0.f) o0 = bf16_t(0.f);
-    if ((float)o1 < 0.f) o1 = bf16_t(0.f);
-    w[q] = (unsigned)o0.bits | ((unsigned)o1.bits << 16);
-  }
-  return v;
-}
 
 #ifdef IG8D_STAMP
 __device__ unsigned long long ig8d_stamps[8 * 512];
@@ -700,7 +692,7 @@
 #pragma unroll
         for (int k = 0; k < 8; k++) {
           const int c = ch * 32 + cg * 8 + k;
-          if (c < CI && n < N) { const float4 a = affine[c]; rw[k] = ig_bn_relu_x8(rw[k], a.x, a.y, a.z); }
+          if (c < CI && n < N) { const float4 a = affine[c]; rw[k] = bn_relu_bf16x8(rw[k], a.x, a.y, a.z); }
         }
       }
       char* xi = Xl + ch * XBUF + img * XIMG;
@@ -1173,11 +1165,13 @@
 constexpr int WG_XCH = 176;
 constexpr int WG_XCOPY = WG_CI * WG_XCH;
 constexpr int WG_STAGE = IG_WTILE + 3 * WG_XCOPY + 512;
-template <int KS, bool NARROW, int CIT, bool PAIR = false, bool CI16 = false>
+template <int KS, bool NARROW, int CIT, bool PAIR = false, bool CI16 = false, bool AFF = false>
 __global__ __launch_bounds__(256) void ig_wgrad8v2_kernel(const bf16_t* __restrict__ dy, const bf16_t* __restrict__ x, float* __restrict__ partial,
                                                           int N, int CO, int CI, int CIP, int images_per_split, int COP, int ntile,
-                                                          const bf16_t* __restrict__ dy2, float* __restrict__ partial2, int CO2, int COP2) {
+                                                          const bf16_t* __restrict__ dy2, float* __restrict__ partial2, int CO2, int COP2,
+                                                          const float4* __restrict__ affine) {
   static_assert(!PAIR || (KS == 3 && CIT == 1), "the pair rides on the 3x3 kernel with one slice of Cin");
+  static_assert(!AFF || (KS == 3 && CIT == 1), "the batch-norm table goes with a 3x3 and one slice of Cin");
   extern __shared__ __attribute__((aligned(16))) char smem[];
   constexpr int RS = KS * KS;
   constexpr int PAD = (KS - 1) / 2;
@@ -1205,7 +1199,10 @@
     if (c < CI) return *reinterpret_cast<const uint4*>(x + ((int64_t)n * CI + c) * 64 + xh * 8);
     return make_uint4(0, 0, 0, 0);
   };
+  float4 aff = make_float4(0.f, 0.f, 0.f, 0.f);
+  if constexpr (AFF) { if (ci0 + xci < CI) aff = affine[ci0 + xci]; }
   auto store_x = [&](char* stage, uint4 v, int ct) {
+    if constexpr (AFF) { if (ci0 + xci < CI) v = bn_relu_bf16x8(v, aff.x, aff.y, aff.z); }
     char* xb = stage + IG_WTILE + (ct * WG_CI + xci) * WG_XCH + (xh + 1) * 16;
     if (KS == 1) { *reinterpret_cast<uint4*>(xb) = v; return; }
     *reinterpret_cast<uint4*>(xb + WG_XCOPY) = v;
@@ -1371,7 +1368,7 @@
     return *reinterpret_cast<const uint4*>(x + ((int64_t)min(n + xim, nend - 1) * CI + xcc) * 64 + xh * 8);
   };
   auto store_x = [&](char* stage, uint4 v) {
-    if (affine) v = ig_bn_relu_x8(v, aff.x, aff.y, aff.z);
+    if (affine) v = bn_relu_bf16x8(v, aff.x, aff.y, aff.z);
     *reinterpret_cast<uint4*>(stage + xim * STG + XC + xci * WG_XCH + (xh + 1) * 16) = v;
   };
   auto load_dy = [&](uint4 (&r)[2], int n) {
@@ -1724,7 +1721,7 @@
   const bool eight = p.form == IgForm::Eight;
   auto beside = [&](const ConvGeom* o) { return KS == 3 && o->kh == 1 && o->Cout == g.Cout && o->Cin == g.Cin && o->N == g.N; };
   p.folds_addend = eight || dgrad;
-  p.folds_affine = eight;
+  p.folds_affine = eight || (sw().fuse_bn_conv_narrow && p.form == IgForm::Two64 && KS == 3 && !dgrad);
   p.sibling = sw().conv_sibling && rq.sibling && !dgrad && !rq.addend && p.form != IgForm::Two64 && beside(rq.sibling->g);
   p.second = sw().conv_dgrad_pair && rq.second && dgrad && beside(rq.second->g);
   p.stats = sw().conv_bn_stats && !dgrad && g.N >= 2;
@@ -1823,10 +1820,17 @@
 #define IG_LAUNCH_B(KS_, SIBM_)                                                                                                                \
   do { if (pl.one) IG_LAUNCH_TWO((ig_conv8b_kernel<KS_, 8, SIBM_, 1>), 512); else if (pl.w8) IG_LAUNCH_TWO((ig_conv8b_kernel<KS_, 8, SIBM_, 2>), 512); \
        else IG_LAUNCH_TWO((ig_conv8b_kernel<KS_, 4, SIBM_, 2>), 256); } while (0)
+#define IG_LAUNCH_C(K_)                                                                                                                        \
+  do {                                                                                                                                         \
+    allow_big_lds((const void*)K_);                                                                                                            \
+    hipLaunchKernelGGL(K_, dim3(pl.blocks), dim3(256), pl.lds, st, inp, wpp, bp, outp, N, CI, KP, CO, statp, addp, sib, affp);                 \
+  } while (0)
     if (pl.form == IgForm::Two128) IG_FOR_KS_SIBM(IG_LAUNCH_B);
-    else if (KS == 1) IG_LAUNCH_TWO((ig_conv8c_kernel<1>), 256);
-    else if (sibm == 2) IG_LAUNCH_TWO((ig_conv8c_kernel<3, 2>), 256);
-    else IG_LAUNCH_TWO((ig_conv8c_kernel<3>), 256);
+    else if (KS == 1) IG_LAUNCH_C((ig_conv8c_kernel<1>));
+    else if (sibm == 2) IG_LAUNCH_C((ig_conv8c_kernel<3, 2>));
+    else if (affp) IG_LAUNCH_C((ig_conv8c_kernel<3, 0, true>));
+    else IG_LAUNCH_C((ig_conv8c_kernel<3>));
+#undef IG_LAUNCH_C
 #undef IG_LAUNCH_B
 #undef IG_LAUNCH_TWO
   }
@@ -1865,10 +1869,12 @@
   if (addend_fused) *addend_fused = addend && pl.folds_addend;
   return true;
 }
-static bool ig_fwd_folds_affine(const ConvGeom& g, int dtype) { return ig_qualifies(g, dtype) && ig_plan(g, false, IgRequest{}).folds_affine; }
+bool igemm_conv_fwd_folds_affine(const ConvGeom& g, int dtype) { return ig_qualifies(g, dtype) && ig_plan(g, false, IgRequest{}).folds_affine; }
 static bool wgrad_takes_eight_wave(const ConvGeom& g) { return g.kh == 3 && g.Cin > WG_CI && g.Cout > 64; }
-static bool ig_wgrad_folds_affine(const ConvGeom& g, int dtype) { return ig_qualifies(g, dtype) && wgrad_takes_eight_wave(g); }
-bool igemm_conv_folds_affine(const ConvGeom& g, int dtype) { return ig_fwd_folds_affine(g, dtype) && ig_wgrad_folds_affine(g, dtype); }
+static bool wgrad_v2_takes_table(const ConvGeom& g) { return sw().fuse_bn_conv_narrow && g.kh == 3 && g.Cin <= 16; }
+bool igemm_conv_wgrad_folds_affine(const ConvGeom& g, int dtype) {
+  return ig_qualifies(g, dtype) && (wgrad_takes_eight_wave(g) || wgrad_v2_takes_table(g));
+}
 bool igemm_conv_fwd_affine(const Tensor* x, const Tensor* affine, const Tensor* w, const Tensor* bias, Tensor* y, const ConvGeom& g, hipStream_t st) {
   if (!ig_qualifies(g, x->dtype)) return false;
   IgRequest rq;
@@ -1980,7 +1986,7 @@
   if (!ig_qualifies(g, x->dtype)) return false;
   const int KS = g.kh, RS = KS * KS;
   const float4* affp = affine ? reinterpret_cast<const float4*>(affine->ptr<float>()) : (const float4*)nullptr;
-  if (affine && !ig_wgrad_folds_affine(g, x->dtype)) return false;
+  if (affine && (second || !igemm_conv_wgrad_folds_affine(g, x->dtype))) return false;
   if (wgrad_takes_eight_wave(g)) {
     if (!second && wg8h_group_defer(dy, x, dw, g, st, affine)) return true;
     Wg8hProblem a{dy, x, dw, g, affine};
@@ -2008,7 +2014,8 @@
       const double sec_by = pair ? conv_bytes(*second->g, 2) - (double)g.N * g.Cin * 64 * 2 : 0.0;
       KernelTimer kt("conv_wgrad_igemm", conv_flops(g) + sec_fl, conv_bytes(g, 2) + sec_by, st);
       const bool ci16 = KS == 3 && CIP == 16;
-      const void* kfn = ci16    ? (pair ? (const void*)ig_wgrad8v2_kernel<3, true, 1, true, true> : (const void*)ig_wgrad8v2_kernel<3, true, 1, false, true>)
+      const void* kfn = ci16    ? (pair   ? (const void*)ig_wgrad8v2_kernel<3, true, 1, true, true>
+                                   : affp ? (const void*)ig_wgrad8v2_kernel<3, true, 1, false, true, true> : (const void*)ig_wgrad8v2_kernel<3, true, 1, false, true>)
                       : pair    ? (narrow ? (const void*)ig_wgrad8v2_kernel<3, true, 1, true> : (const void*)ig_wgrad8v2_kernel<3, false, 1, true>)
                       : KS == 3 ? (narrow ? (const void*)ig_wgrad8v2_kernel<3, true, 1> : (const void*)ig_wgrad8v2_kernel<3, false, 1>)
                       : all_ci  ? (narrow ? (const void*)ig_wgrad8v2_kernel<1, true, 4> : (const void*)ig_wgrad8v2_kernel<1, false, 4>)
@@ -2020,7 +2027,7 @@
       int a_N = (int)g.N, a_CO = (int)g.Cout, a_CI = (int)g.Cin, a_CIP = CIP, a_ips = ips, a_COP = COP, a_ntile = ntile;
       int a_CO2 = pair ? (int)second->g->Cout : 0, a_COP2 = COP2;
       void* args[] = {(void*)&dyp, (void*)&xp, (void*)&pp, (void*)&a_N, (void*)&a_CO, (void*)&a_CI, (void*)&a_CIP, (void*)&a_ips, (void*)&a_COP, (void*)&a_ntile,
-                      (void*)&dy2p, (void*)&p2p, (void*)&a_CO2, (void*)&a_COP2};
+                      (void*)&dy2p, (void*)&p2p, (void*)&a_CO2, (void*)&a_COP2, (void*)&affp};
       HIP_CHECK(hipLaunchKernel(kfn, dim3(ntile * nsplit), dim3(256), args, lds, st));
       LAMP_LAUNCH_CHECK();
     }
diff --git a/lamp_amd/csrc/kernels/conv_narrow.hip b/lamp_amd/csrc/kernels/conv_narrow.hip
--- a/lamp_amd/csrc/kernels/conv_narrow.hip
+++ b/lamp_amd/csrc/kernels/conv_narrow.hip
@@ -159,11 +159,11 @@
   r.m2 = a.m2 + b.m2 + d * d * a.n * f;
   return r;
 }
-template <int NK, int SW, int PH0, int NS, bool ADD, bool STATS, bool PAR = false>
-__global__ __launch_bounds__(256, (STATS && NK <= 5) ? 3 : 1) void ncv_fwd2_kernel(const bf16_t* __restrict__ src, const nv_bf8* __restrict__ wpk, const bf16_t* __restrict__ bias,
+template <int NK, int SW, int PH0, int NS, bool ADD, bool STATS, bool PAR = false, bool AFF = false>
+__global__ __launch_bounds__(256, (STATS && NK <= 5 && !(AFF && NS == 1)) ? 3 : 1) void ncv_fwd2_kernel(const bf16_t* __restrict__ src, const nv_bf8* __restrict__ wpk, const bf16_t* __restrict__ bias,
                                                        bf16_t* dst, NcvGeom q, const bf16_t* add, bf16_t* dst2, const bf16_t* __restrict__ bias2, int co_a,
                                                        float* __restrict__ stats, float* __restrict__ stats2, int stats_per_wg,
-                                                       const bf16_t* __restrict__ src2) {
+                                                       const bf16_t* __restrict__ src2, const float4* __restrict__ affine) {
   __shared__ float sst[STATS ? 2 : 1][4][16][3];
   extern __shared__ __attribute__((aligned(16))) char smem[];
   unsigned short* xs = reinterpret_cast<unsigned short*>(smem);
@@ -178,6 +178,14 @@
   NcvPre pre;
   const NcvPlan plan = ncv_stage_plan(q, tid, nthreads);
   if (q.pf && (int)blockIdx.x < q.N) ncv_stage_load(pre, plan, src + blockIdx.x * img_in, src2 + blockIdx.x * img_in2);
+  const float4* afs = reinterpret_cast<const float4*>(smem + (size_t)q.C * q.Hs * q.Ws * 2);
+  int pch[AFF ? NCV_PF : 1];
+  if constexpr (AFF) {
+    if (tid < q.C) reinterpret_cast<float4*>(smem + (size_t)q.C * q.Hs * q.Ws * 2)[tid] = affine[tid];
+    const int hw = q.H * q.W;
+#pragma unroll
+    for (int k = 0; k < NCV_PF; k++) pch[k] = plan.dst[k] >= 0 ? plan.src[k] / hw : 0;
+  }
   nv_bf8 wfr[NK];
   int koff[NK];
 #pragma unroll
@@ -245,6 +253,11 @@
     if (n < 0)
 #endif
     {
+    if constexpr (AFF) {
+#pragma unroll
+      for (int k = 0; k < NCV_PF; k++)
+        if (plan.dst[k] >= 0) { const float4 a = afs[pch[k]]; pre.v[k] = bn_relu_bf16x8(pre.v[k], a.x, a.y, a.z); }
+    }
     if (q.pf) ncv_stage_store(xs, pre, plan, q.dil);
     else ncv_stage(xs, src + n * img_in, q, tid, nthreads);
     }
@@ -494,9 +507,10 @@
 
 constexpr int NCV_OFFA = 8;
 constexpr int NCV_WPF = 6;
-template <int KW, int PW, int SW, int NPT>
+template <int KW, int PW, int SW, int NPT, bool AFF = false>
 __global__ __launch_bounds__(256) void ncv_wgrad2_kernel(const bf16_t* __restrict__ dy, const bf16_t* __restrict__ x, float* __restrict__ partial, NcvWGeom q,
-                                                         int images_per_block, const bf16_t* __restrict__ dy2, float* __restrict__ partial2) {
+                                                         int images_per_block, const bf16_t* __restrict__ dy2, float* __restrict__ partial2,
+                                                         const float4* __restrict__ affine) {
   extern __shared__ __attribute__((aligned(16))) char smem[];
   const int tid = threadIdx.x, lane = tid & 63, wid = tid >> 6;
   const int HoWo = q.Ho * q.Wo;
@@ -505,6 +519,8 @@
   unsigned short* ds = xs + q.IG * ximg;
   constexpr int NCOLT = NPT * KW * 16;
   float* red = reinterpret_cast<float*>(ds + q.IG * 16 * HoWo);
+  float4* afs = reinterpret_cast<float4*>(red + 4 * 16 * NCOLT);
+  if constexpr (AFF) { if (tid < q.Cin) afs[tid] = affine[tid]; }
   {
     const int tot = q.IG * (ximg + 16 * HoWo);
     for (int o = tid * 8; o < tot; o += 256 * 8) *reinterpret_cast<uint4*>(xs + o) = make_uint4(0, 0, 0, 0);
@@ -528,6 +544,7 @@
   const int chunks_per_img = HoWo >> 5;
   const int xpk = (q.Cin * q.H * q.W) >> 3, dpk = (q.Cout * HoWo) >> 3, dpk2 = (q.Cout2 * HoWo) >> 3, per = xpk + dpk + dpk2;
   const int rc = q.W >> 3;
+  auto im_of = [&](int meta) { return AFF ? (meta & 0xffff) : meta; };
   const bool pf = q.IG * per <= NCV_WPF * 256;
   uint4 pre[NCV_WPF];
   int p_src[NCV_WPF], p_dst[NCV_WPF], p_im[NCV_WPF];
@@ -536,6 +553,7 @@
     const int idx = tid + k * 256;
     const int im = idx / per, j = idx - im * per;
     p_im[k] = (pf && im < q.IG) ? im : -1;
+    if constexpr (AFF) { if (p_im[k] >= 0 && j < xpk) p_im[k] |= (j / (rc * q.H)) << 16; }
     if (j < xpk) {
       const int b = j % rc, a = (j / rc) % q.H, c = j / (rc * q.H);
       p_src[k] = im * q.Cin * q.H * q.W + j * 8;
@@ -554,7 +572,7 @@
     const bf16_t* dg2 = dy2 + nb * q.Cout2 * HoWo;
 #pragma unroll
     for (int k = 0; k < NCV_WPF; k++)
-      if (p_im[k] >= 0 && p_im[k] < ig) {
+      if (p_im[k] >= 0 && im_of(p_im[k]) < ig) {
         const bf16_t* sp = p_src[k] >= 0 ? xg + p_src[k] : p_src[k] >= -(1 << 30) ? dg + (-p_src[k] - 1) : dg2 + (-p_src[k] - 1 - (1 << 30));
         pre[k] = *reinterpret_cast<const uint4*>(sp);
       }
@@ -573,8 +591,11 @@
   auto pre_store = [&](int ig) {
 #pragma unroll
     for (int k = 0; k < NCV_WPF; k++) {
-      if (p_im[k] < 0 || p_im[k] >= ig) continue;
-      const uint4 v = pre[k];
+      if (p_im[k] < 0 || im_of(p_im[k]) >= ig) continue;
+      uint4 v = pre[k];
+      if constexpr (AFF) {
+        if (p_src[k] >= 0) { const float4 a = afs[p_im[k] >> 16]; v = bn_relu_bf16x8(v, a.x, a.y, a.z); }
+      }
       if (SW == 1 || p_src[k] < 0) *reinterpret_cast<uint4*>(xs + p_dst[k]) = v;
       else stage_x(xs + p_dst[k], v);
     }
@@ -595,7 +616,11 @@
     else for (int im = 0; im < ig; im++) {
       const bf16_t* xp = x + (nb + im) * q.Cin * q.H * q.W;
       unsigned short* xi = xs + im * ximg;
-      for (int i = tid; i < xpk; i += 256) stage_x(x_dst(xi, i), *reinterpret_cast<const uint4*>(xp + i * 8));
+      for (int i = tid; i < xpk; i += 256) {
+        uint4 v = *reinterpret_cast<const uint4*>(xp + i * 8);
+        if constexpr (AFF) { const float4 a = afs[i / (rc * q.H)]; v = bn_relu_bf16x8(v, a.x, a.y, a.z); }
+        stage_x(x_dst(xi, i), v);
+      }
       const bf16_t* dp = dy + (nb + im) * q.Cout * HoWo;
       unsigned short* di = ds + im * 16 * HoWo;
       for (int i = tid; i < dpk; i += 256) *reinterpret_cast<uint4*>(di + i * 8) = *reinterpret_cast<const uint4*>(dp + i * 8);
@@ -822,11 +847,14 @@
 
 struct NcvSibling { const Tensor* w; const Tensor* bias; Tensor* out; };
 struct NcvSecondGrad { const Tensor* dy; const Tensor* w; };
+struct NcvAffine { const Tensor* table; bool plan_only; };
 static bool ncv_run(const Tensor* in, const Tensor* w, const Tensor* bias, Tensor* out, const ConvGeom& g, bool dgrad, hipStream_t st,
                     const Tensor* addend = nullptr, bool* addend_fused = nullptr, const NcvSibling* sib = nullptr,
-                    const NcvSecondGrad* second = nullptr) {
+                    const NcvSecondGrad* second = nullptr, const NcvAffine* aff = nullptr) {
   if (addend_fused) *addend_fused = false;
-  if (!ncv_common(g, in->dtype)) return false;
+  const bool plan_only = aff && aff->plan_only;
+  if (!plan_only && !ncv_common(g, in->dtype)) return false;
+  if (aff && (dgrad || sib || second || addend || g.kh != 3 || g.kw != 3 || g.ph != 1 || g.pw != 1 || g.sh != 1)) return false;
   const int cout2 = sib ? (int)sib->w->sizes[0] : second ? (int)second->w->sizes[0] : 0;
   if (sib && (dgrad || g.Cout + cout2 > 16)) return false;
   if (second && (!dgrad || sib || cout2 > 16)) return false;
@@ -855,7 +883,7 @@
   if (aligned && !(ncg == 2 || ncg == 4 || ncg == 8 || ncg == 16)) aligned = false;
   if (aligned && q.Ho % (16 / ncg) != 0) aligned = false;
   if (aligned) q.Ws = round_up(std::max(q.Ws, q.Wo * q.sw + (q.wx - ph0) + 16), 8);
-  if ((sib || second) && !aligned) return false;
+  if ((sib || second || aff) && !aligned) return false;
   const int pairs = q.C1 * q.kh + (q.C - q.C1);
   const int nk_real = (pairs + 3) / 4;
   static const int nk_opts[] = {1, 2, 4, 5, 6, 8, 12, 16};
@@ -877,10 +905,15 @@
       if (step % ncg == 0 && ((step / ncg) & 1) == 1 && (size_t)q.C * q.Hs * (q.Ws + 8 * k) * 2 <= 64 * 1024) { q.Ws += 8 * k; break; }
     }
   }
-  const size_t lds = (size_t)q.C * q.Hs * q.Ws * 2;
+  const size_t lds = (size_t)q.C * q.Hs * q.Ws * 2 + (aff ? 256 : 0);
   if (lds > 64 * 1024) return false;
   const bool two_shift_on = sw().ncv_two_shift;
   const int NS = (two_shift_on && aligned && q.CO <= 8 && g.kw + q.sw <= 8) ? 2 : 1;
+  if (aff) {
+    const int threads = 64 * std::min(4, q.Ho / (16 / ncg));
+    if (NK < 5 || NK > 12 || (int64_t)q.C * q.H * q.W > (int64_t)NCV_PF * threads * 8) return false;
+    if (plan_only) return true;
+  }
   const Tensor* wsecond = sib ? sib->w : second ? second->w : nullptr;
   const NcvW wq{w->ptr<bf16_t>(), (int)g.Cout, (int)g.Cin, g.kh, g.kw, dgrad ? 1 : 0, NS, q.sw, wsecond ? wsecond->ptr<bf16_t>() : (const bf16_t*)nullptr, cout2, nke};
   Hold wpk_h(ncv_packed_weights(w, wq, st, wsecond));
@@ -917,6 +950,12 @@
       case 16: NCV_F2_PAIR(16); break;
       default: NCV_F2_SW(12); break;
     }
+    if (aff) {
+#define NCV_F2A(NKv, STv) kfn = NS == 2 ? (const void*)ncv_fwd2_kernel<NKv, 1, 7, 2, false, STv, false, true> : (const void*)ncv_fwd2_kernel<NKv, 1, 7, 1, false, STv, false, true>
+      if (NK2 == 5) { if (with_stats) NCV_F2A(5, true); else NCV_F2A(5, false); }
+      else { if (with_stats) NCV_F2A(12, true); else NCV_F2A(12, false); }
+#undef NCV_F2A
+    }
 #undef NCV_F2_PAIR
 #undef NCV_F2P_PH
 #undef NCV_F2P
@@ -953,8 +992,9 @@
         stat2p = statt2->ptr<float>();
       }
     }
+    const float4* affp = aff ? reinterpret_cast<const float4*>(aff->table->ptr<float>()) : (const float4*)nullptr;
     void* args[] = {(void*)&srcp, (void*)&wpk, (void*)&bp, (void*)&dstp, (void*)&q, (void*)&addp, (void*)&dst2p, (void*)&bias2p, (void*)&co_a,
-                    (void*)&statp, (void*)&stat2p, (void*)&stats_per_wg, (void*)&src2p};
+                    (void*)&statp, (void*)&stat2p, (void*)&stats_per_wg, (void*)&src2p, (void*)&affp};
     HIP_CHECK(hipLaunchKernel(kfn, dim3(blocks), dim3(threads), args, lds, st));
     LAMP_LAUNCH_CHECK();
     if (statt.get()) conv_stats_publish(out, statt.get(), parts, sib ? 0 : w->st->uid);
@@ -979,6 +1019,14 @@
 bool narrow_conv_fwd(const Tensor* x, const Tensor* w, const Tensor* bias, Tensor* y, const ConvGeom& g, hipStream_t st) {
   return ncv_run(x, w, bias, y, g, false, st);
 }
+bool narrow_conv_fwd_affine(const Tensor* x, const Tensor* affine, const Tensor* w, const Tensor* bias, Tensor* y, const ConvGeom& g, hipStream_t st) {
+  const NcvAffine a{affine, false};
+  return ncv_run(x, w, bias, y, g, false, st, nullptr, nullptr, nullptr, nullptr, &a);
+}
+bool narrow_conv_fwd_folds_affine(const ConvGeom& g, int dtype) {
+  const NcvAffine a{nullptr, true};
+  return ncv_common(g, dtype) && ncv_run(nullptr, nullptr, nullptr, nullptr, g, false, nullptr, nullptr, nullptr, nullptr, nullptr, &a);
+}
 bool narrow_conv_fwd_pair(const Tensor* x, const Tensor* w, const Tensor* bias, Tensor* y, const ConvGeom& g, const Tensor* w1, const Tensor* bias1,
                           Tensor* y1, const ConvGeom& g1, hipStream_t st) {
   const bool on = sw().conv_sibling;
@@ -1012,8 +1060,11 @@
 }
 
 struct NcvSecondWgrad { const Tensor* dy; Tensor* dw; };
-static bool ncv_wgrad_run(const Tensor* dy, const Tensor* x, Tensor* dw, const ConvGeom& g, hipStream_t st, const NcvSecondWgrad* second) {
-  if (!ncv_common(g, x->dtype)) return false;
+static bool ncv_wgrad_run(const Tensor* dy, const Tensor* x, Tensor* dw, const ConvGeom& g, hipStream_t st, const NcvSecondWgrad* second,
+                          const NcvAffine* aff = nullptr) {
+  const bool plan_only = aff && aff->plan_only;
+  if (!plan_only && !ncv_common(g, x->dtype)) return false;
+  if (aff && (second || g.kh != 3 || g.kw != 3 || g.ph != 1 || g.pw != 1 || g.sh != 1)) return false;
   if (g.W % 8 != 0 || g.Wo % 8 != 0 || (g.Ho * g.Wo) % 32 != 0) return false;
   const int cout2 = second ? (int)second->dy->sizes[1] : 0;
   if (second && (g.Cout + cout2 > 16 || g.kh != 3 || g.kw != 3 || g.ph != 1 || g.pw != 1)) return false;
@@ -1038,8 +1089,9 @@
     else q.Ws = round_up(NCV_OFFA + std::max((int)g.W / 2, (int)g.Wo) + 8, 8);
     const int ximg2 = q.Cin * q.Hs * q.Ws * (SW == 2 ? 2 : 1);
     const int ncolt = npt * g.kw * 16;
-    const size_t lds2 = (size_t)q.IG * (ximg2 + 16 * HoWo) * 2 + (size_t)4 * 16 * ncolt * 4;
+    const size_t lds2 = (size_t)q.IG * (ximg2 + 16 * HoWo) * 2 + (size_t)4 * 16 * ncolt * 4 + (aff ? 256 : 0);
     if (lds2 <= 150 * 1024) {
+      if (plan_only) return true;
       const int O = q.Cout * q.ncol;
       const void* kfn = nullptr;
 #define NCV_WG2(KWv, PWv, SWv, NPTv) kfn = (const void*)ncv_wgrad2_kernel<KWv, PWv, SWv, NPTv>
@@ -1051,6 +1103,8 @@
       else NCV_WG2_NPT(1, 0, 2);
 #undef NCV_WG2_NPT
 #undef NCV_WG2
+      if (aff) kfn = npt == 1 ? (const void*)ncv_wgrad2_kernel<3, 1, 1, 1, true> : npt == 2 ? (const void*)ncv_wgrad2_kernel<3, 1, 1, 2, true>
+                                                                                           : (const void*)ncv_wgrad2_kernel<3, 1, 1, 3, true>;
       allow_big_lds(kfn);
       const int per_cu = std::min((int)std::max<size_t>(1, std::min<size_t>(4, (size_t)(150 * 1024) / lds2)), kernel_occupancy(kfn, 256, lds2));
       const int64_t rounds = (g.N + q.IG - 1) / q.IG;
@@ -1070,7 +1124,8 @@
         const bf16_t* dp2 = second ? second->dy->ptr<bf16_t>() : (const bf16_t*)nullptr;
         float* pp2 = second ? partial2->ptr<float>() : (float*)nullptr;
         int ipb_arg = ipb;
-        void* args[] = {(void*)&dp, (void*)&xp, (void*)&pp, (void*)&q, (void*)&ipb_arg, (void*)&dp2, (void*)&pp2};
+        const float4* affp = aff ? reinterpret_cast<const float4*>(aff->table->ptr<float>()) : (const float4*)nullptr;
+        void* args[] = {(void*)&dp, (void*)&xp, (void*)&pp, (void*)&q, (void*)&ipb_arg, (void*)&dp2, (void*)&pp2, (void*)&affp};
         HIP_CHECK(hipLaunchKernel(kfn, dim3(nblocks), dim3(256), args, lds2, st));
         LAMP_LAUNCH_CHECK();
       }
@@ -1084,11 +1139,11 @@
       }
       return true;
     }
-    if (second) return false;
+    if (second || aff) return false;
     if (SW == 1) q.Ws = round_up(std::max(NCV_LEFT + (int)g.W, (int)g.Wo - 1 + g.kw - 1 - g.pw + NCV_LEFT + 1), 8);
     else { const int half_max = (g.kw - 1 - g.pw) >> 1; q.Ws = round_up(std::max((int)g.W / 2, (int)g.Wo + half_max) + NCV_OFF2 + 1, 8); }
   }
-  if (second) return false;
+  if (second || aff) return false;
   const int nt_real = (q.ncol + 15) / 16;
   static const int nt_opts[] = {1, 2, 4, 5, 9};
   int NT = 0;
@@ -1130,7 +1185,14 @@
   return true;
 }
 
-bool narrow_conv_wgrad(const Tensor* dy, const Tensor* x, Tensor* dw, const ConvGeom& g, hipStream_t st) { return ncv_wgrad_run(dy, x, dw, g, st, nullptr); }
+bool narrow_conv_wgrad(const Tensor* dy, const Tensor* x, Tensor* dw, const ConvGeom& g, hipStream_t st, const Tensor* affine) {
+  const NcvAffine a{affine, false};
+  return ncv_wgrad_run(dy, x, dw, g, st, nullptr, affine ? &a : nullptr);
+}
+bool narrow_conv_wgrad_folds_affine(const ConvGeom& g, int dtype) {
+  const NcvAffine a{nullptr, true};
+  return ncv_common(g, dtype) && ncv_wgrad_run(nullptr, nullptr, nullptr, g, nullptr, nullptr, &a);
+}
 bool narrow_conv_wgrad_pair(const Tensor* dy, const Tensor* dy1, const Tensor* x, Tensor* dw, Tensor* dw1, const ConvGeom& g, const ConvGeom& g1, hipStream_t st) {
   const bool on = sw().conv_wgrad_pair;
   if (!on || x->dtype != kBF16 || dy->dtype != kBF16 || dy1->dtype != kBF16) return false;
diff --git a/lamp_amd/csrc/kernels/device_utils.h b/lamp_amd/csrc/kernels/device_utils.h
--- a/lamp_amd/csrc/kernels/device_utils.h
+++ b/lamp_amd/csrc/kernels/device_utils.h
@@ -39,6 +39,19 @@
 }
 __device__ __forceinline__ uint4 add_bf16x8(const uint4& a, const uint4& b) {
   return make_uint4(add_bf16x2(a.x, b.x), add_bf16x2(a.y, b.y), add_bf16x2(a.z, b.z), add_bf16x2(a.w, b.w));
+}
+
+__device__ __forceinline__ uint4 bn_relu_bf16x8(uint4 v, float mu, float scale, float bb) {
+  unsigned* w = &v.x;
+#pragma unroll
+  for (int q = 0; q < 4; q++) {
+    const float x0 = __uint_as_float(w[q] << 16), x1 = __uint_as_float(w[q] & 0xffff0000u);
+    bf16_t o0(__builtin_fmaf(x0 - mu, scale, bb)), o1(__builtin_fmaf(x1 - mu, scale, bb));
+    if ((float)o0 < 0.f) o0 = bf16_t(0.f);
+    if ((float)o1 < 0.f) o1 = bf16_t(0.f);
+    w[q] = (unsigned)o0.bits | ((unsigned)o1.bits << 16);
+  }
+  return v;
 }
 
 __device__ __forceinline__ uint4 nt_load16(const uint4* p) {
```

Result: no change. 2.209 million samples/s (-0.4%).
